# markomih/SplatFields

Hardware: AMD Instinct MI355X
Metric: splats*px rasterized/sec (fwd+bwd) (higher is better)
Workload: dtype f32

## Files before the change

include/splatraster.h:

```cpp
#ifndef SPLATRASTER_H
#define SPLATRASTER_H

#include <stddef.h>

#ifdef __cplusplus
extern "C" {
#endif

#define SR_VERSION 4
#define SR_TILE 16

typedef struct SrView {
    int image_height;
    int image_width;
    float tanfovx;
    float tanfovy;
    float scale_modifier;
    int sh_degree;
    int sh_coeffs;
    int prefiltered;
    int debug;
    const float* viewmatrix;
    const float* projmatrix;
    const float* campos;
    const float* bg;
} SrView;

typedef struct SrSplats {
    int count;
    const float* means3D;
    const float* opacities;
    const float* scales;
    const float* rotations;
    const float* cov3D_precomp;
    const float* shs;
    const float* colors_precomp;
    int raw_params;
    const float* shs_rest;
} SrSplats;

#define SR_RAW_SCALES 1
#define SR_RAW_OPACITY 2
#define SR_RAW_ROTATIONS 4
#define SR_FORWARD_ONLY 8

typedef struct SrGrads {
    float* dL_dmeans3D;
    float* dL_dmeans2D;
    float* dL_dopacity;
    float* dL_dscales;
    float* dL_drotations;
    float* dL_dcov3D;
    float* dL_dshs;
    float* dL_dcolors;
    float* dL_dshs_rest;
} SrGrads;

int sr_version(void);
const char* sr_last_error(void);

size_t sr_geom_bytes(int n_splats, int height, int width);
size_t sr_binning_bytes(long long instances, int height, int width);
size_t sr_image_bytes(int height, int width);
size_t sr_backward_scratch_bytes(long long instances);

int sr_forward_prepare(const SrView* view, const SrSplats* splats, void* geom, int* radii,
                       long long* instances_out, void* hip_stream);

int sr_forward_render(const SrView* view, const SrSplats* splats, void* geom, void* binning,
                      long long instances, void* image, float* out_color, float* out_depth,
                      float* out_alpha, void* hip_stream);

#define SR_NEED_CAPACITY 2
int sr_forward(const SrView* view, const SrSplats* splats, void* geom, int* radii, void* binning,
               long long binning_capacity, void* image, float* out_color, float* out_depth, float* out_alpha,
               long long* instances_out, void* hip_stream);

int sr_forward_async(const SrView* view, const SrSplats* splats, void* geom, int* radii, void* binning,
                     long long binning_capacity, long long longest_list_hint, long long longest_list_expected, void* image,
                     float* out_color, float* out_depth, float* out_alpha, void** ticket_out, void* hip_stream);
int sr_ticket_wait(void* ticket, long long* instances_out, long long* longest_list_out);
long long sr_last_longest_list(void);
int sr_ticket_release(void* ticket);

#define SR_BWD_SLOT_SPEC_BELOW 6
int sr_backward(const SrView* view, const SrSplats* splats, const void* geom, void* binning,
                long long instances, long long instances_rendered, const void* image, const int* radii,
                const float* dL_dcolor, const float* dL_ddepth, const float* dL_dalpha, void* scratch,
                const SrGrads* grads, void* hip_stream);

int sr_backward_blend(const SrView* view, const SrSplats* splats, const void* geom, void* binning,
                      long long instances, long long instances_rendered, const void* image,
                      const float* dL_dcolor, const float* dL_ddepth, const float* dL_dalpha, void* scratch, void* hip_stream);
int sr_backward_splats(const SrView* view, const SrSplats* splats, const void* geom, void* binning,
                       long long instances, long long instances_rendered, const void* image, const int* radii, void* scratch,
                       const SrGrads* grads, int first_splat, int n_splats, void* hip_stream);

int sr_set_backward_kernel(int which);

int sr_mark_visible(int n_splats, const float* means3D, const float* viewmatrix,
                    const float* projmatrix, unsigned char* present, void* hip_stream);

int sr_densification_stats(int n_splats, const float* dL_dmeans2D, const int* radii, float* grad_accum, float* denom,
                           float* max_radii2D, void* hip_stream);

size_t sr_loss_workspace_bytes(int planes, int height, int width);
size_t sr_loss_maps_bytes(int planes, int height, int width);
int sr_photometric_forward(int batch, int channels, int height, int width, const float* image, const float* gt,
                           const float* alpha, const float* gt_mask, float lambda_dssim, float lambda_mask, void* workspace,
                           float* maps, float* loss, float* l1, float* ssim, float* mask_l1, void* hip_stream);
int sr_photometric_backward(int batch, int channels, int height, int width, const float* image, const float* gt,
                            const float* alpha, const float* gt_mask, const float* maps, float w_l1, float w_ssim, float w_mask,
                            const float* upstream, int upstream_per_item, float* dL_dimage, float* dL_dalpha, void* hip_stream);

#define SR_QUANT_NONE 0
#define SR_QUANT_PNG 1
#define SR_QUANT_TO8B 2
size_t sr_metrics_workspace_bytes(int batch, int height, int width);
int sr_image_metrics(int batch, int height, int width, const float* pred, const long long* pred_strides4, const float* gt,
                     const long long* gt_strides4, const float* mask, long long mask_item_stride, int quantize, void* workspace,
                     float* psnr, float* ssim, float* psnr_channels, unsigned char* frames, void* hip_stream);

int sr_sh_forward(int n_splats, int sh_coeffs, int sh_degree, const float* means3D, const float* shs, const float* campos,
                  float* colors, unsigned char* clamped, void* hip_stream);

int sr_sh_forward_views(int n_splats, int sh_coeffs, int sh_degree, int n_views, const float* means3D, const float* shs,
                        const float* campos, float* colors, float* keep, void* hip_stream);

int sr_sh_backward(int n_splats, int sh_coeffs, int sh_degree, int n_views, const float* means3D, const float* shs,
                   const float* campos, const float* dL_dcolors, float scale, float* dL_dshs, float* dL_dmeans3D,
                   int accumulate_means, void* hip_stream);

size_t sr_knn_workspace_bytes(int n_points);
int sr_knn3_mean_dist2(int n_points, const float* points, float* mean_dist2, void* workspace, void* hip_stream);

#define SR_KNN_MAX_K 8
size_t sr_knn_graph_workspace_bytes(int n_points, int k);
int sr_knn_graph(int n_points, int k, const float* points, int* nn_ix, unsigned* order, unsigned* rev_start, unsigned* rev_edges,
                 void* workspace, void* hip_stream);

#define SR_MORAN_MAX_TENSORS 8
size_t sr_moran_workspace_bytes(int n_items, int n_tensors);
size_t sr_moran_edges_bytes(int n_items, int k, int channels);
int sr_moran_forward(int n_items, int k, float eps, const float* points, const float* weight, const int* nn_ix,
                     const unsigned* order, int n_tensors, const float* const* features, const int* widths, void* workspace,
                     float* out, void* hip_stream);
int sr_moran_backward(int n_items, int k, float eps, const float* points, const float* weight, const int* nn_ix,
                      const unsigned* order, const unsigned* rev_start, const unsigned* rev_edges, int n_tensors,
                      const float* const* features, const int* widths, const float* out, const float* upstream, void* edges,
                      float* const* dL_dfeatures, float* dL_dpoints, float* dL_dweight, void* hip_stream);
int sr_moran_weights(int n_points, int k, float eps, const float* points, const int* nn_ix, float* weights, void* hip_stream);
int sr_moran_weights_backward(int n_points, int k, float eps, const float* points, const int* nn_ix, const unsigned* rev_start,
                              const unsigned* rev_edges, const float* dL_dweights, void* edges, float* dL_dpoints,
                              void* hip_stream);

size_t sr_splat_reg_workspace_bytes(int n_splats);
int sr_splat_reg_forward(int n_splats, const float* means3D, const float* opacity, double lambda_norm, double lambda_norm_mean,
                         double lambda_opacity, void* workspace, float* out, void* hip_stream);
int sr_splat_reg_backward(int n_splats, const float* means3D, const float* opacity, double lambda_norm, double lambda_norm_mean,
                          double lambda_opacity, const float* out, const float* upstream, float* dL_dmeans3D, float* dL_dopacity,
                          void* hip_stream);

size_t sr_depth_l1_workspace_bytes(int batch, int height, int width);
int sr_depth_l1_forward(int batch, int height, int width, const float* depth, const float* gt_depth, void* workspace, float* out,
                        void* hip_stream);
int sr_depth_l1_backward(int batch, int height, int width, const float* depth, const float* gt_depth, const float* upstream,
                         int upstream_per_item, float* dL_ddepth, void* hip_stream);

size_t sr_densify_workspace_bytes(int n_splats);
int sr_densify_plan(int n_splats, const float* log_scales, int scale_cols, const float* opacity_logits, const float* grad_accum,
                    const float* denom, const float* max_radii2D, float grad_threshold, float min_opacity, float extent,
                    float percent_dense, float max_screen_size, void* workspace, int* dest, long long* counts5, void* hip_stream);
int sr_densify_gather(int n_splats, int row_floats, const float* src, float* dst, const int* dest, int mode,
                      const float* log_scales, int scale_cols, const float* rotations, const float* unit_normals,
                      void* hip_stream);

#define SR_ADAM_MAX_TENSORS 32
typedef struct SrAdamJob {
    float* param;
    const float* grad;
    float* exp_avg;
    float* exp_avg_sq;
    long long count;
    int row;
    float step_size, bias_correction2_sqrt, one_minus_beta1, one_minus_beta2, eps;
} SrAdamJob;
int sr_adam_step(int n_jobs, const SrAdamJob* jobs, const unsigned char* visible_or_null, long long rows, void* hip_stream);

#define SR_MLP_MAX_OPS 24
#define SR_MLP_NONE 0
#define SR_MLP_LEAKY 1
#define SR_MLP_MASK 2
typedef struct SrMlpOp {
    const float* w_packed;
    const float* bias;
    const float* src;
    const float* mask;
    float* store;
    unsigned int* sign_store;
    const unsigned int* mask_bits;
    int out_tiles;
    int mem_tiles;
    int reg_tiles;
    int src_row;
    int epilogue;
    int mask_row;
    int store_row;
    int store_channels;
    int store_accumulate;
    int keep_state;
} SrMlpOp;
int sr_mlp_chain(int n_points, int hidden_tiles, int n_ops, const SrMlpOp* ops, float negative_slope, void* hip_stream);

#define SR_MLP_MAX_PACK_JOBS 32
typedef struct SrMlpPackJob {
    const float* w;
    const float* bias_src;
    float* dst;
    float* bias_dst;
    int ld;
    int transposed;
    int row0, n_rows;
    int n_mem, mem_pad, mem_col0;
    int n_reg, reg_width, reg_col0;
    int out_tiles;
    int n_bias;
} SrMlpPackJob;
int sr_mlp_pack(int n_jobs, const SrMlpPackJob* jobs, void* hip_stream);

int sr_mlp_pack_bf16(int n_jobs, const SrMlpPackJob* jobs, void* hip_stream);
int sr_mlp_chain_bf16(int n_points, int hidden_tiles, int n_ops, const SrMlpOp* ops, float negative_slope, void* hip_stream);

int sr_mlp_pack_bf16x3(int n_jobs, const SrMlpPackJob* jobs, void* hip_stream);
int sr_mlp_chain_bf16x3(int n_points, int hidden_tiles, int n_ops, const SrMlpOp* ops, float negative_slope, void* hip_stream);

#define SR_MLP_GROUP_MAX_NETS 8
#define SR_MLP_GROUP_MAX_OPS 40
typedef struct SrMlpNet {
    const SrMlpOp* ops;
    int n_ops;
} SrMlpNet;
int sr_mlp_chain_group(int n_points, int hidden_tiles, int n_nets, const SrMlpNet* nets, float negative_slope, void* hip_stream);
int sr_mlp_chain_group_bf16(int n_points, int hidden_tiles, int n_nets, const SrMlpNet* nets, float negative_slope, void* hip_stream);
int sr_mlp_chain_group_bf16x3(int n_points, int hidden_tiles, int n_nets, const SrMlpNet* nets, float negative_slope, void* hip_stream);

#define SR_MLP_MAX_GRAD_JOBS 16
#define SR_MLP_MAX_GRAD_TASKS 128
typedef struct SrMlpGradJob {
    const float* dz;
    const float* x;
    float* dw;
// ... 50 lines not shown
size_t sr_resfield_backward_workspace(int n_jobs, const SrResFieldJob* jobs);
int sr_resfield_backward(int n_jobs, const SrResFieldJob* jobs, const long long* frame, void* workspace, size_t workspace_bytes,
                         void* hip_stream);

size_t sr_triplane_backward_workspace(int n_points, int channels, int height, int width);
int sr_triplane_forward(int n_points, int channels, int height, int width, const float* planes, float* planes_texel_major,
                        const float* points, float* out, void* hip_stream);
int sr_triplane_backward(int n_points, int channels, int height, int width, const float* planes_texel_major, const float* points,
                         const float* dL_dout, float* dL_dplanes, float* dL_dpoints, void* workspace, void* hip_stream);

#define SR_PLANE_MAX_JOBS 8
#define SR_CONV_PROLOGUE 1
#define SR_CONV_UPSAMPLE 2
#define SR_CONV_RESIDUAL 4
#define SR_CONV_SILU_OUT 8
typedef struct SrPlaneJob {
    const float* x;
    const float* weight;
    const float* bias;
    const float* gamma;
    const float* beta;
    float* stats;
    const float* residual;
    float* out;
    float* pre;
    const float* dy;
    float* dx;
    float* dweight;
    float* dbias;
    float* dgamma;
    float* dbeta;
    float* d_residual;
    const float* add;
    float* dx_out;
} SrPlaneJob;

size_t sr_groupnorm_stats_workspace(int n_planes, int channels, int groups, int height, int width);
int sr_groupnorm_stats(int n_planes, const SrPlaneJob* jobs, int channels, int groups, int height, int width, float eps,
                       void* workspace, void* hip_stream);

int sr_conv3x3_forward(int n_planes, const SrPlaneJob* jobs, int cin, int cout, int h_in, int w_in, int groups, int flags,
                       void* hip_stream);

int sr_conv3x3_backward_data(int n_planes, const SrPlaneJob* jobs, int cin, int cout, int h_in, int w_in, int flags, void* hip_stream);

size_t sr_groupnorm_silu_backward_workspace(int n_planes, int channels, int height, int width);
int sr_groupnorm_silu_backward(int n_planes, const SrPlaneJob* jobs, int channels, int groups, int height, int width, float eps,
                               void* workspace, void* hip_stream);

size_t sr_conv3x3_weight_grad_workspace(int n_planes, int cin, int cout, int h_in, int w_in, int flags);
int sr_conv3x3_weight_grad(int n_planes, const SrPlaneJob* jobs, int cin, int cout, int h_in, int w_in, int groups, int flags,
                           void* workspace, void* hip_stream);

typedef struct SrAttentionJob {
    const float* x;
    const float* gamma;
    const float* beta;
    float* stats;
    const float* wq;
    const float* bq;
    const float* wk;
    const float* bk;
    const float* wv;
    const float* bv;
    const float* wo;
    const float* bo;
    float* out;
    void* saved;
    const float* dy;
    float* dx;
    float* dgamma;
    float* dbeta;
    float* dwq;
    float* dbq;
    float* dwk;
    float* dbk;
    float* dwv;
    float* dbv;
    float* dwo;
    float* dbo;
} SrAttentionJob;

size_t sr_attention_saved_bytes(int n_planes, int channels, int groups, int height, int width);
size_t sr_attention_backward_workspace(int n_planes, int channels, int groups, int height, int width);

int sr_attention_forward(int n_planes, const SrAttentionJob* jobs, int channels, int groups, int height, int width, float eps,
                         void* hip_stream);

int sr_attention_backward(int n_planes, const SrAttentionJob* jobs, int channels, int groups, int height, int width, float eps,
                          void* workspace, void* hip_stream);

#define SR_HULL_KRT 0
#define SR_HULL_NDC 1
#define SR_HULL_OUTSIDE_CARVE 0
#define SR_HULL_OUTSIDE_KEEP 1
#define SR_HULL_MAX_VIEWS 1024
typedef struct SrHullView {
    double m[12];
    long long mask_offset;
    int height, width;
    int convention;
    int outside;
} SrHullView;
size_t sr_hull_workspace_bytes(long long n_items);
int sr_hull_carve(int n_views, const SrHullView* views, const unsigned char* masks, long long mask_bytes, const double* grid, int G,
                  const void* points, long long n_points, int point_is_double, void* workspace, int* count_out, void* hip_stream);
int sr_hull_gather(const double* grid, int G, const void* points, long long n_points, int point_is_double, const void* workspace,
                   long long capacity, int* indices_out, float* points_out, void* hip_stream);

#define SR_FLOW_OFFSET 0
#define SR_FLOW_SE3 1
#define SR_FLOW_SE3_AFFINE 2
#define SR_FLOW_SE3_SCALED 3
#define SR_FLOW_AFFINE 4
#define SR_FLOW_DCT 5
#define SR_FLOW_MAX_BRANCHES 4
#define SR_FLOW_MAX_WIDTH 256
#define SR_FLOW_MAX_OUT 32
#define SR_FLOW_MAX_BASIS 10
typedef struct SrFlowBranch {
    const float* weight;
    const float* bias;
    int rows;
} SrFlowBranch;
size_t sr_flow_head_saved_bytes(int model, long long n_points, int width, int n_basis);
size_t sr_flow_head_workspace_bytes(int model, long long n_points, int width, int n_basis);
int sr_flow_head_dz_row(int model, int n_basis);
int sr_flow_head_forward(int model, long long n_points, int width, int n_basis, int n_branches, const SrFlowBranch* branches,
                         const float* hidden, const float* pts, const float* bases, float* means3D, float* flow, void* saved,
                         void* hip_stream);
int sr_flow_head_backward(int model, long long n_points, int width, int n_basis, int n_branches, const SrFlowBranch* branches,
                          const float* pts, const float* bases, const void* saved, const float* dL_dmeans3D, const float* dL_dflow,
                          float* dL_dpts, float* dL_dz, float* dL_dhidden, void* workspace, void* hip_stream);

#define SR_VIEW_FROM_CAMERAS 0
#define SR_VIEW_DIRS_GIVEN 1
#define SR_VIEW_MAX_WIDTH 256
#define SR_VIEW_MAX_VIEWS 16
size_t sr_view_color_saved_bytes(long long n_points, int width, int n_views);
size_t sr_view_color_workspace_bytes(long long n_points, int width, int n_views);
int sr_view_color_forward(int mode, long long n_points, int width, int n_views, const float* feature, const float* means3D,
                          const float* campos_or_dirs, const float* weight, const float* bias, float* colours, void* saved,
                          void* hip_stream);
int sr_view_color_backward(int mode, long long n_points, int width, int n_views, const float* means3D, const float* campos_or_dirs,
                           const float* weight, const void* saved, const float* dL_dcolours, float* dL_dfeature, float* dL_dpos,
                           float* dL_dzsum, void* workspace, void* hip_stream);

int sr_debug_layout(int n_splats, int height, int width, long long instances, size_t* out4);

int sr_debug_backward_stats(unsigned long long* out16, int reset);

int sr_debug_counters(long long* out4, int reset);

int sr_debug_snapshot(const SrView* view, const SrSplats* splats, const float* dL_dcolor, const float* dL_ddepth,
                      const float* dL_dalpha, int backward);

#define SR_PROFILE_STAGES 7
int sr_profile_enable(int on);
int sr_profile_collect(double* ms_sum, long long* launches);
const char* sr_profile_stage_name(int stage);

#ifdef __cplusplus
}
#endif
#endif
```

splatfields_amd/_lib.py:

```python
from __future__ import annotations

import ctypes as C
from pathlib import Path

import os

import torch

LIB_PATH = Path(os.environ.get("SPLATRASTER_LIB") or (Path(__file__).resolve().parent / "libsplatraster.so"))

c_float_p = C.c_void_p


class SrView(C.Structure):
    _fields_ = [("image_height", C.c_int), ("image_width", C.c_int), ("tanfovx", C.c_float), ("tanfovy", C.c_float),
                ("scale_modifier", C.c_float), ("sh_degree", C.c_int), ("sh_coeffs", C.c_int), ("prefiltered", C.c_int),
                ("debug", C.c_int), ("viewmatrix", C.c_void_p), ("projmatrix", C.c_void_p), ("campos", C.c_void_p),
                ("bg", C.c_void_p)]


class SrSplats(C.Structure):
    _fields_ = [("count", C.c_int), ("means3D", C.c_void_p), ("opacities", C.c_void_p), ("scales", C.c_void_p),
                ("rotations", C.c_void_p), ("cov3D_precomp", C.c_void_p), ("shs", C.c_void_p),
                ("colors_precomp", C.c_void_p), ("raw_params", C.c_int), ("shs_rest", C.c_void_p)]


class SrGrads(C.Structure):
    _fields_ = [("dL_dmeans3D", C.c_void_p), ("dL_dmeans2D", C.c_void_p), ("dL_dopacity", C.c_void_p),
                ("dL_dscales", C.c_void_p), ("dL_drotations", C.c_void_p), ("dL_dcov3D", C.c_void_p),
                ("dL_dshs", C.c_void_p), ("dL_dcolors", C.c_void_p), ("dL_dshs_rest", C.c_void_p)]


class SrMlpOp(C.Structure):
    _fields_ = [("w_packed", C.c_void_p), ("bias", C.c_void_p), ("src", C.c_void_p), ("mask", C.c_void_p), ("store", C.c_void_p),
                ("sign_store", C.c_void_p), ("mask_bits", C.c_void_p),
                ("out_tiles", C.c_int), ("mem_tiles", C.c_int), ("reg_tiles", C.c_int), ("src_row", C.c_int), ("epilogue", C.c_int),
                ("mask_row", C.c_int), ("store_row", C.c_int), ("store_channels", C.c_int), ("store_accumulate", C.c_int),
                ("keep_state", C.c_int)]


class SrMlpNet(C.Structure):
    _fields_ = [("ops", C.POINTER(SrMlpOp)), ("n_ops", C.c_int)]


class SrMlpHeadInput(C.Structure):
    _fields_ = [("x0", C.c_void_p), ("dL_dx0", C.c_void_p), ("multires", C.c_int), ("row", C.c_int)]


class SrMlpHeadOutput(C.Structure):
    _fields_ = [("y", C.c_void_p), ("out", C.c_void_p), ("dL_dout", C.c_void_p), ("g", C.c_void_p), ("out_features", C.c_int),
                ("row", C.c_int), ("activation", C.c_int), ("reserved", C.c_int)]


class SrMlpPackJob(C.Structure):
    _fields_ = [("w", C.c_void_p), ("bias_src", C.c_void_p), ("dst", C.c_void_p), ("bias_dst", C.c_void_p), ("ld", C.c_int),
                ("transposed", C.c_int), ("row0", C.c_int), ("n_rows", C.c_int), ("n_mem", C.c_int), ("mem_pad", C.c_int),
                ("mem_col0", C.c_int), ("n_reg", C.c_int), ("reg_width", C.c_int), ("reg_col0", C.c_int), ("out_tiles", C.c_int),
                ("n_bias", C.c_int)]


class SrMlpGradJob(C.Structure):
    _fields_ = [("dz", C.c_void_p), ("x", C.c_void_p), ("dw", C.c_void_p), ("db", C.c_void_p), ("dz_row", C.c_int), ("m", C.c_int),
                ("x_row", C.c_int), ("k", C.c_int), ("dw_row", C.c_int), ("dw_col0", C.c_int)]


class SrResFieldJob(C.Structure):
    _fields_ = [("w", C.c_void_p), ("weights_t", C.c_void_p), ("matrix_t", C.c_void_p), ("out", C.c_void_p), ("d_out", C.c_void_p),
                ("d_matrix_t", C.c_void_p), ("d_weights_t", C.c_void_p), ("count", C.c_int), ("rank", C.c_int), ("capacity", C.c_int)]


class SrAdamJob(C.Structure):
    _fields_ = [("param", C.c_void_p), ("grad", C.c_void_p), ("exp_avg", C.c_void_p), ("exp_avg_sq", C.c_void_p),
                ("count", C.c_longlong), ("row", C.c_int), ("step_size", C.c_float), ("bias_correction2_sqrt", C.c_float),
                ("one_minus_beta1", C.c_float), ("one_minus_beta2", C.c_float), ("eps", C.c_float)]


class SrPlaneJob(C.Structure):
    _fields_ = [(name, C.c_void_p) for name in (
        "x", "weight", "bias", "gamma", "beta", "stats", "residual", "out", "pre", "dy", "dx", "dweight", "dbias", "dgamma", "dbeta",
        "d_residual", "add", "dx_out")]


class SrAttentionJob(C.Structure):
    _fields_ = [(name, C.c_void_p) for name in (
        "x", "gamma", "beta", "stats", "wq", "bq", "wk", "bk", "wv", "bv", "wo", "bo", "out", "saved", "dy", "dx", "dgamma", "dbeta",
        "dwq", "dbq", "dwk", "dbk", "dwv", "dbv", "dwo", "dbo")]


class SrHullView(C.Structure):
    _fields_ = [("m", C.c_double * 12), ("mask_offset", C.c_longlong), ("height", C.c_int), ("width", C.c_int),
                ("convention", C.c_int), ("outside", C.c_int)]


class SrFlowBranch(C.Structure):
    _fields_ = [("weight", C.c_void_p), ("bias", C.c_void_p), ("rows", C.c_int)]


FLOW_OFFSET, FLOW_SE3, FLOW_SE3_AFFINE, FLOW_SE3_SCALED, FLOW_AFFINE, FLOW_DCT = 0, 1, 2, 3, 4, 5
FLOW_MAX_BRANCHES, FLOW_MAX_WIDTH, FLOW_MAX_OUT, FLOW_MAX_BASIS = 4, 256, 32, 10
VIEW_FROM_CAMERAS, VIEW_DIRS_GIVEN, VIEW_MAX_WIDTH, VIEW_MAX_VIEWS = 0, 1, 256, 16
HULL_KRT, HULL_NDC, HULL_OUTSIDE_CARVE, HULL_OUTSIDE_KEEP, HULL_MAX_VIEWS = 0, 1, 0, 1, 1024
RESFIELD_MAX_JOBS, RESFIELD_MAX_RANK = 16, 64
PLANE_MAX_JOBS = 8
CONV_PROLOGUE, CONV_UPSAMPLE, CONV_RESIDUAL, CONV_SILU_OUT = 1, 2, 4, 8
MLP_MAX_GRAD_JOBS, MLP_MAX_GRAD_TASKS = 16, 128
MLP_MAX_PACK_JOBS = 32
MORAN_MAX_TENSORS, KNN_MAX_K = 8, 8
ADAM_MAX_TENSORS = 32
QUANT_NONE, QUANT_PNG, QUANT_TO8B = 0, 1, 2
MLP_MAX_OPS, MLP_NONE, MLP_LEAKY, MLP_MASK = 24, 0, 1, 2
MLP_GROUP_MAX_NETS, MLP_GROUP_MAX_OPS, MLP_GROUP_MAX_HEADS = 8, 40, 8
MLP_OUT_NONE, MLP_OUT_SIGMOID, MLP_OUT_NORMALIZE = 0, 1, 2


SYMBOLS = {
    "sr_version": (C.c_int, []),
    "sr_last_error": (C.c_char_p, []),
    "sr_geom_bytes": (C.c_size_t, [C.c_int, C.c_int, C.c_int]),
    "sr_binning_bytes": (C.c_size_t, [C.c_longlong, C.c_int, C.c_int]),
    "sr_image_bytes": (C.c_size_t, [C.c_int, C.c_int]),
    "sr_backward_scratch_bytes": (C.c_size_t, [C.c_longlong]),
    "sr_forward_prepare": (C.c_int, [C.POINTER(SrView), C.POINTER(SrSplats), C.c_void_p, C.c_void_p,
                                     C.POINTER(C.c_longlong), C.c_void_p]),
    "sr_forward_render": (C.c_int, [C.POINTER(SrView), C.POINTER(SrSplats), C.c_void_p, C.c_void_p, C.c_longlong,
                                    C.c_void_p, C.c_void_p, C.c_void_p, C.c_void_p, C.c_void_p]),
    "sr_forward": (C.c_int, [C.POINTER(SrView), C.POINTER(SrSplats), C.c_void_p, C.c_void_p, C.c_void_p, C.c_longlong,
                             C.c_void_p, C.c_void_p, C.c_void_p, C.c_void_p, C.POINTER(C.c_longlong), C.c_void_p]),
    "sr_forward_async": (C.c_int, [C.POINTER(SrView), C.POINTER(SrSplats), C.c_void_p, C.c_void_p, C.c_void_p, C.c_longlong,
                                   C.c_longlong, C.c_longlong, C.c_void_p, C.c_void_p, C.c_void_p, C.c_void_p, C.POINTER(C.c_void_p),
                                   C.c_void_p]),
    "sr_ticket_wait": (C.c_int, [C.c_void_p, C.POINTER(C.c_longlong), C.POINTER(C.c_longlong)]),
    "sr_ticket_release": (C.c_int, [C.c_void_p]),
    "sr_last_longest_list": (C.c_longlong, []),
    "sr_debug_counters": (C.c_int, [C.POINTER(C.c_longlong), C.c_int]),
    "sr_backward": (C.c_int, [C.POINTER(SrView), C.POINTER(SrSplats), C.c_void_p, C.c_void_p, C.c_longlong, C.c_longlong, C.c_void_p,
                              C.c_void_p, C.c_void_p, C.c_void_p, C.c_void_p, C.c_void_p, C.POINTER(SrGrads),
                              C.c_void_p]),
    "sr_backward_blend": (C.c_int, [C.POINTER(SrView), C.POINTER(SrSplats), C.c_void_p, C.c_void_p, C.c_longlong, C.c_longlong, C.c_void_p,
                                    C.c_void_p, C.c_void_p, C.c_void_p, C.c_void_p, C.c_void_p]),
    "sr_backward_splats": (C.c_int, [C.POINTER(SrView), C.POINTER(SrSplats), C.c_void_p, C.c_void_p, C.c_longlong, C.c_longlong, C.c_void_p, C.c_void_p,
                                     C.c_void_p, C.POINTER(SrGrads), C.c_int, C.c_int, C.c_void_p]),
    "sr_debug_snapshot": (C.c_int, [C.POINTER(SrView), C.POINTER(SrSplats), C.c_void_p, C.c_void_p, C.c_void_p, C.c_int]),
    "sr_set_backward_kernel": (C.c_int, [C.c_int]),
    "sr_sh_forward": (C.c_int, [C.c_int, C.c_int, C.c_int, C.c_void_p, C.c_void_p, C.c_void_p, C.c_void_p, C.c_void_p, C.c_void_p]),
    "sr_sh_forward_views": (C.c_int, [C.c_int, C.c_int, C.c_int, C.c_int, C.c_void_p, C.c_void_p, C.c_void_p, C.c_void_p, C.c_void_p, C.c_void_p]),
    "sr_sh_backward": (C.c_int, [C.c_int, C.c_int, C.c_int, C.c_int, C.c_void_p, C.c_void_p, C.c_void_p, C.c_void_p, C.c_float,
                                 C.c_void_p, C.c_void_p, C.c_int, C.c_void_p]),
    "sr_knn_workspace_bytes": (C.c_size_t, [C.c_int]),
    "sr_knn3_mean_dist2": (C.c_int, [C.c_int, C.c_void_p, C.c_void_p, C.c_void_p, C.c_void_p]),
    "sr_knn_graph_workspace_bytes": (C.c_size_t, [C.c_int, C.c_int]),
    "sr_knn_graph": (C.c_int, [C.c_int, C.c_int, C.c_void_p, C.c_void_p, C.c_void_p, C.c_void_p, C.c_void_p, C.c_void_p, C.c_void_p]),
    "sr_moran_workspace_bytes": (C.c_size_t, [C.c_int, C.c_int]),
    "sr_moran_edges_bytes": (C.c_size_t, [C.c_int, C.c_int, C.c_int]),
    "sr_moran_forward": (C.c_int, [C.c_int, C.c_int, C.c_float, C.c_void_p, C.c_void_p, C.c_void_p, C.c_void_p, C.c_int,
                                   C.POINTER(C.c_void_p), C.POINTER(C.c_int), C.c_void_p, C.c_void_p, C.c_void_p]),
    "sr_moran_backward": (C.c_int, [C.c_int, C.c_int, C.c_float, C.c_void_p, C.c_void_p, C.c_void_p, C.c_void_p, C.c_void_p, C.c_void_p,
                                    C.c_int, C.POINTER(C.c_void_p), C.POINTER(C.c_int), C.c_void_p, C.c_void_p, C.c_void_p,
                                    C.POINTER(C.c_void_p), C.c_void_p, C.c_void_p, C.c_void_p]),
    "sr_moran_weights": (C.c_int, [C.c_int, C.c_int, C.c_float, C.c_void_p, C.c_void_p, C.c_void_p, C.c_void_p]),
    "sr_moran_weights_backward": (C.c_int, [C.c_int, C.c_int, C.c_float, C.c_void_p, C.c_void_p, C.c_void_p, C.c_void_p, C.c_void_p,
                                            C.c_void_p, C.c_void_p, C.c_void_p]),
    "sr_loss_workspace_bytes": (C.c_size_t, [C.c_int, C.c_int, C.c_int]),
    "sr_loss_maps_bytes": (C.c_size_t, [C.c_int, C.c_int, C.c_int]),
    "sr_photometric_forward": (C.c_int, [C.c_int, C.c_int, C.c_int, C.c_int, C.c_void_p, C.c_void_p, C.c_void_p, C.c_void_p, C.c_float,
                                         C.c_float, C.c_void_p, C.c_void_p, C.c_void_p, C.c_void_p, C.c_void_p, C.c_void_p, C.c_void_p]),
    "sr_photometric_backward": (C.c_int, [C.c_int, C.c_int, C.c_int, C.c_int, C.c_void_p, C.c_void_p, C.c_void_p, C.c_void_p, C.c_void_p,
                                          C.c_float, C.c_float, C.c_float, C.c_void_p, C.c_int, C.c_void_p, C.c_void_p, C.c_void_p]),
    "sr_metrics_workspace_bytes": (C.c_size_t, [C.c_int, C.c_int, C.c_int]),
    "sr_image_metrics": (C.c_int, [C.c_int, C.c_int, C.c_int, C.c_void_p, C.POINTER(C.c_longlong), C.c_void_p, C.POINTER(C.c_longlong),
                                   C.c_void_p, C.c_longlong, C.c_int, C.c_void_p, C.c_void_p, C.c_void_p, C.c_void_p, C.c_void_p,
                                   C.c_void_p]),
    "sr_adam_step": (C.c_int, [C.c_int, C.POINTER(SrAdamJob), C.c_void_p, C.c_longlong, C.c_void_p]),
    "sr_splat_reg_workspace_bytes": (C.c_size_t, [C.c_int]),
    "sr_splat_reg_forward": (C.c_int, [C.c_int, C.c_void_p, C.c_void_p, C.c_double, C.c_double, C.c_double, C.c_void_p, C.c_void_p, C.c_void_p]),
    "sr_splat_reg_backward": (C.c_int, [C.c_int, C.c_void_p, C.c_void_p, C.c_double, C.c_double, C.c_double, C.c_void_p, C.c_void_p, C.c_void_p,
                                        C.c_void_p, C.c_void_p]),
    "sr_depth_l1_workspace_bytes": (C.c_size_t, [C.c_int, C.c_int, C.c_int]),
    "sr_depth_l1_forward": (C.c_int, [C.c_int, C.c_int, C.c_int, C.c_void_p, C.c_void_p, C.c_void_p, C.c_void_p, C.c_void_p]),
    "sr_depth_l1_backward": (C.c_int, [C.c_int, C.c_int, C.c_int, C.c_void_p, C.c_void_p, C.c_void_p, C.c_int, C.c_void_p, C.c_void_p]),
    "sr_densify_workspace_bytes": (C.c_size_t, [C.c_int]),
    "sr_densify_plan": (C.c_int, [C.c_int, C.c_void_p, C.c_int, C.c_void_p, C.c_void_p, C.c_void_p, C.c_void_p, C.c_float, C.c_float,
                                  C.c_float, C.c_float, C.c_float, C.c_void_p, C.c_void_p, C.POINTER(C.c_longlong), C.c_void_p]),
    "sr_densify_gather": (C.c_int, [C.c_int, C.c_int, C.c_void_p, C.c_void_p, C.c_void_p, C.c_int, C.c_void_p, C.c_int, C.c_void_p,
                                    C.c_void_p, C.c_void_p]),
    "sr_hull_workspace_bytes": (C.c_size_t, [C.c_longlong]),
    "sr_hull_carve": (C.c_int, [C.c_int, C.POINTER(SrHullView), C.c_void_p, C.c_longlong, C.c_void_p, C.c_int, C.c_void_p, C.c_longlong,
                                C.c_int, C.c_void_p, C.c_void_p, C.c_void_p]),
    "sr_hull_gather": (C.c_int, [C.c_void_p, C.c_int, C.c_void_p, C.c_longlong, C.c_int, C.c_void_p, C.c_longlong, C.c_void_p, C.c_void_p,
                                 C.c_void_p]),
    "sr_mlp_pack": (C.c_int, [C.c_int, C.POINTER(SrMlpPackJob), C.c_void_p]),
    "sr_mlp_weight_grad_workspace": (C.c_size_t, [C.c_int, C.c_int, C.POINTER(SrMlpGradJob)]),
    "sr_mlp_weight_grad": (C.c_int, [C.c_int, C.c_int, C.POINTER(SrMlpGradJob), C.c_void_p, C.c_size_t, C.c_void_p]),
    "sr_mlp_chain": (C.c_int, [C.c_int, C.c_int, C.c_int, C.POINTER(SrMlpOp), C.c_float, C.c_void_p]),
    "sr_mlp_pack_bf16": (C.c_int, [C.c_int, C.POINTER(SrMlpPackJob), C.c_void_p]),
    "sr_mlp_chain_bf16": (C.c_int, [C.c_int, C.c_int, C.c_int, C.POINTER(SrMlpOp), C.c_float, C.c_void_p]),
    "sr_mlp_pack_bf16x3": (C.c_int, [C.c_int, C.POINTER(SrMlpPackJob), C.c_void_p]),
    "sr_mlp_chain_bf16x3": (C.c_int, [C.c_int, C.c_int, C.c_int, C.POINTER(SrMlpOp), C.c_float, C.c_void_p]),
    "sr_mlp_chain_group": (C.c_int, [C.c_int, C.c_int, C.c_int, C.POINTER(SrMlpNet), C.c_float, C.c_void_p]),
    "sr_mlp_chain_group_bf16": (C.c_int, [C.c_int, C.c_int, C.c_int, C.POINTER(SrMlpNet), C.c_float, C.c_void_p]),
    "sr_mlp_chain_group_bf16x3": (C.c_int, [C.c_int, C.c_int, C.c_int, C.POINTER(SrMlpNet), C.c_float, C.c_void_p]),
    "sr_mlp_group_input_forward": (C.c_int, [C.c_int, C.c_int, C.POINTER(SrMlpHeadInput), C.c_int, C.c_int, C.c_void_p, C.c_void_p, C.c_void_p,
                                             C.c_void_p]),
    "sr_mlp_group_input_backward": (C.c_int, [C.c_int, C.c_int, C.POINTER(SrMlpHeadInput), C.c_int, C.c_void_p, C.c_void_p, C.c_void_p, C.c_void_p]),
    "sr_mlp_group_output": (C.c_int, [C.c_int, C.c_int, C.POINTER(SrMlpHeadOutput), C.c_void_p]),
    "sr_mlp_group_top_gradient": (C.c_int, [C.c_int, C.c_int, C.POINTER(SrMlpHeadOutput), C.c_float, C.c_void_p]),
    "sr_mlp_input_forward": (C.c_int, [C.c_int, C.c_int, C.c_int, C.c_int, C.c_int, C.c_void_p, C.c_void_p, C.c_void_p, C.c_void_p, C.c_void_p]),
    "sr_mlp_top_gradient": (C.c_int, [C.c_int, C.c_int, C.c_int, C.c_void_p, C.c_void_p, C.c_float, C.c_void_p, C.c_void_p]),
    "sr_mlp_input_backward": (C.c_int, [C.c_int, C.c_int, C.c_int, C.c_int, C.c_void_p, C.c_void_p, C.c_void_p, C.c_void_p, C.c_void_p]),
    "sr_resfield_compose": (C.c_int, [C.c_int, C.POINTER(SrResFieldJob), C.c_void_p, C.c_void_p]),
    "sr_resfield_backward_workspace": (C.c_size_t, [C.c_int, C.POINTER(SrResFieldJob)]),
    "sr_resfield_backward": (C.c_int, [C.c_int, C.POINTER(SrResFieldJob), C.c_void_p, C.c_void_p, C.c_size_t, C.c_void_p]),
    "sr_triplane_backward_workspace": (C.c_size_t, [C.c_int, C.c_int, C.c_int, C.c_int]),
    "sr_triplane_forward": (C.c_int, [C.c_int, C.c_int, C.c_int, C.c_int, C.c_void_p, C.c_void_p, C.c_void_p, C.c_void_p, C.c_void_p]),
    "sr_triplane_backward": (C.c_int, [C.c_int, C.c_int, C.c_int, C.c_int, C.c_void_p, C.c_void_p, C.c_void_p, C.c_void_p, C.c_void_p,
                                       C.c_void_p, C.c_void_p]),
    "sr_groupnorm_stats_workspace": (C.c_size_t, [C.c_int, C.c_int, C.c_int, C.c_int, C.c_int]),
    "sr_groupnorm_stats": (C.c_int, [C.c_int, C.POINTER(SrPlaneJob), C.c_int, C.c_int, C.c_int, C.c_int, C.c_float, C.c_void_p, C.c_void_p]),
    "sr_conv3x3_forward": (C.c_int, [C.c_int, C.POINTER(SrPlaneJob), C.c_int, C.c_int, C.c_int, C.c_int, C.c_int, C.c_int, C.c_void_p]),
    "sr_conv3x3_backward_data": (C.c_int, [C.c_int, C.POINTER(SrPlaneJob), C.c_int, C.c_int, C.c_int, C.c_int, C.c_int, C.c_void_p]),
    "sr_groupnorm_silu_backward_workspace": (C.c_size_t, [C.c_int, C.c_int, C.c_int, C.c_int]),
    "sr_groupnorm_silu_backward": (C.c_int, [C.c_int, C.POINTER(SrPlaneJob), C.c_int, C.c_int, C.c_int, C.c_int, C.c_float, C.c_void_p,
                                             C.c_void_p]),
    "sr_conv3x3_weight_grad_workspace": (C.c_size_t, [C.c_int, C.c_int, C.c_int, C.c_int, C.c_int, C.c_int]),
    "sr_conv3x3_weight_grad": (C.c_int, [C.c_int, C.POINTER(SrPlaneJob), C.c_int, C.c_int, C.c_int, C.c_int, C.c_int, C.c_int, C.c_void_p,
                                         C.c_void_p]),
    "sr_attention_saved_bytes": (C.c_size_t, [C.c_int, C.c_int, C.c_int, C.c_int, C.c_int]),
    "sr_attention_backward_workspace": (C.c_size_t, [C.c_int, C.c_int, C.c_int, C.c_int, C.c_int]),
    "sr_attention_forward": (C.c_int, [C.c_int, C.POINTER(SrAttentionJob), C.c_int, C.c_int, C.c_int, C.c_int, C.c_float, C.c_void_p]),
    "sr_attention_backward": (C.c_int, [C.c_int, C.POINTER(SrAttentionJob), C.c_int, C.c_int, C.c_int, C.c_int, C.c_float, C.c_void_p,
                                        C.c_void_p]),
    "sr_flow_head_saved_bytes": (C.c_size_t, [C.c_int, C.c_longlong, C.c_int, C.c_int]),
    "sr_flow_head_workspace_bytes": (C.c_size_t, [C.c_int, C.c_longlong, C.c_int, C.c_int]),
    "sr_flow_head_dz_row": (C.c_int, [C.c_int, C.c_int]),
    "sr_flow_head_forward": (C.c_int, [C.c_int, C.c_longlong, C.c_int, C.c_int, C.c_int, C.POINTER(SrFlowBranch), C.c_void_p, C.c_void_p,
                                       C.c_void_p, C.c_void_p, C.c_void_p, C.c_void_p, C.c_void_p]),
    "sr_flow_head_backward": (C.c_int, [C.c_int, C.c_longlong, C.c_int, C.c_int, C.c_int, C.POINTER(SrFlowBranch), C.c_void_p, C.c_void_p,
                                        C.c_void_p, C.c_void_p, C.c_void_p, C.c_void_p, C.c_void_p, C.c_void_p, C.c_void_p, C.c_void_p]),
    "sr_view_color_saved_bytes": (C.c_size_t, [C.c_longlong, C.c_int, C.c_int]),
    "sr_view_color_workspace_bytes": (C.c_size_t, [C.c_longlong, C.c_int, C.c_int]),
    "sr_view_color_forward": (C.c_int, [C.c_int, C.c_longlong, C.c_int, C.c_int, C.c_void_p, C.c_void_p, C.c_void_p, C.c_void_p, C.c_void_p,
                                        C.c_void_p, C.c_void_p, C.c_void_p]),
    "sr_view_color_backward": (C.c_int, [C.c_int, C.c_longlong, C.c_int, C.c_int, C.c_void_p, C.c_void_p, C.c_void_p, C.c_void_p, C.c_void_p,
                                         C.c_void_p, C.c_void_p, C.c_void_p, C.c_void_p, C.c_void_p]),
    "sr_debug_layout": (C.c_int, [C.c_int, C.c_int, C.c_int, C.c_longlong, C.POINTER(C.c_size_t)]),
    "sr_debug_backward_stats": (C.c_int, [C.POINTER(C.c_ulonglong), C.c_int]),
    "sr_profile_enable": (C.c_int, [C.c_int]),
    "sr_profile_collect": (C.c_int, [C.POINTER(C.c_double), C.POINTER(C.c_longlong)]),
    "sr_profile_stage_name": (C.c_char_p, [C.c_int]),
    "sr_mark_visible": (C.c_int, [C.c_int, C.c_void_p, C.c_void_p, C.c_void_p, C.c_void_p, C.c_void_p]),
    "sr_densification_stats": (C.c_int, [C.c_int, C.c_void_p, C.c_void_p, C.c_void_p, C.c_void_p, C.c_void_p, C.c_void_p]),
}

PROFILE_STAGES = 7
SR_VERSION = 4
SR_NEED_CAPACITY = 2
SR_RAW_SCALES, SR_RAW_OPACITY, SR_RAW_ROTATIONS, SR_FORWARD_ONLY = 1, 2, 4, 8
_lib = None


def bind(path) -> C.CDLL:
    lib = C.CDLL(str(path))
    for name, (res, args) in SYMBOLS.items():
        fn = getattr(lib, name)
        fn.restype = res
        fn.argtypes = args
    got = lib.sr_version()
    if got != SR_VERSION:
        raise RuntimeError(f"{path} implements version {got} of the splatraster ABI, this binding expects {SR_VERSION}: "
                           "rebuild it with `python -m splatfields_amd.build`")
    return lib


def load() -> C.CDLL:
    global _lib
    if _lib is None:
        if not LIB_PATH.exists():
            raise RuntimeError(
                f"{LIB_PATH} is missing: build it with `python -m splatfields_amd.build` "
                "(hipcc --offload-arch=gfx950). There is no CPU fallback.")
        _lib = bind(LIB_PATH)
    return _lib


class use_library:

    def __init__(self, path):
        self.handle = bind(path)

    def __enter__(self):
        global _lib
        self.prev, _lib = _lib, self.handle
        return self.handle

    def __exit__(self, *exc):
        global _lib
        _lib = self.prev
# ... 31 lines not shown
```

splatfields_amd/build.py:

```python
from __future__ import annotations

import os
import shutil
import subprocess
from pathlib import Path

PKG_DIR = Path(__file__).resolve().parent
CSRC = PKG_DIR / "csrc"
LIB_PATH = PKG_DIR / "libsplatraster.so"
STATS_LIB_PATH = PKG_DIR / "libsplatraster_stats.so"
SOURCES = ["api.hip", "preprocess.hip", "binning.hip", "render.hip", "blend_bwd.hip", "knn.hip", "sh.hip", "densify.hip", "mlp.hip", "triplane.hip", "loss.hip", "moran.hip", "adam.hip", "metrics.hip", "objective.hip", "planegen.hip", "attention.hip", "hull.hip", "flow_head.hip", "view_color.hip"]
HEADERS = ["common.h", "kernels.h", "host_api.h", "expand.h", "sh_stage.h", "quadmask.h", "reduce.h", "window11.h", "point_tile.h", "mlp_bf16x3.h", "../../include/splatraster.h"]


def _hipcc() -> str:
    exe = shutil.which("hipcc") or "/opt/rocm/bin/hipcc"
    if not os.path.exists(exe):
        raise RuntimeError("hipcc not found; libsplatraster.so cannot be built")
    return exe


def is_stale() -> bool:
    if not LIB_PATH.exists():
        return True
    t = LIB_PATH.stat().st_mtime
    return any((CSRC / f).stat().st_mtime > t for f in SOURCES + HEADERS)


def strip_comments(text: str) -> str:
    out, i, n = [], 0, len(text)
    while i < n:
        c = text[i]
        if c in "\"'":
            j = i + 1
            while j < n and text[j] != c:
                j += 2 if text[j] == "\\" else 1
            out.append(text[i:j + 1])
            i = j + 1
        elif text.startswith("//", i):
            j = text.find("\n", i)
            i = n if j < 0 else j
        elif text.startswith("/*", i):
            j = text.find("*/", i + 2)
            out.append(" ")
            i = n if j < 0 else j + 2
        else:
            out.append(c)
            i += 1
    lines = (" ".join(line.split()) for line in "".join(out).splitlines())
    return "\n".join(line for line in lines if line)


def source_hash() -> str:
    import hashlib
    h = hashlib.sha256()
    for f in sorted(SOURCES + HEADERS):
        h.update(f.encode())
        h.update(strip_comments((CSRC / f).read_text()).encode())
    return h.hexdigest()[:16]


def build_library(force: bool = False, verbose: bool = False, out: Path = None, defines=()) -> Path:
    if out is None and not force and not is_stale():
        return LIB_PATH
    target = Path(out) if out is not None else LIB_PATH
    cmd = [_hipcc(), "--offload-arch=gfx950", "-O3", "-std=c++17", "-shared", "-fPIC", "-Wno-unused-value",
           "-fno-slp-vectorize"] + [f"-D{d}" for d in defines] + [
           "-o", str(target)] + [str(CSRC / f) for f in SOURCES]
    if verbose:
        print(" ".join(cmd))
    subprocess.run(cmd, check=True, cwd=str(CSRC))
    return target


def build_stats_library(force: bool = False, verbose: bool = False) -> Path:
    if not force and STATS_LIB_PATH.exists() and not any(
            (CSRC / f).stat().st_mtime > STATS_LIB_PATH.stat().st_mtime for f in SOURCES + HEADERS):
        return STATS_LIB_PATH
    return build_library(force=True, verbose=verbose, out=STATS_LIB_PATH, defines=["SR_BWD_STATS", "SR_BWD_WAVES_PER_SIMD=3"])


if __name__ == "__main__":
    import sys
    if len(sys.argv) > 1:
        print(build_library(force=True, verbose=True, out=Path(sys.argv[1]).resolve(), defines=sys.argv[2:]))
    else:
        print(build_library(force=True, verbose=True))
```

splatfields_amd/csrc/api.hip:

```cpp
#include <cstdint>
#include <cstdio>
#include <cstdlib>
#include <cstring>
#include <atomic>
#include <chrono>
#include <thread>
#include <mutex>
#include <string>
#include <vector>
#include "host_api.h"
#include "kernels.h"

namespace {

thread_local std::string g_last_error;
thread_local long long g_last_longest = -1;

struct ProfRec { int stage; hipEvent_t a, b; bool ended; unsigned long long serial; };
unsigned long long g_prof_serial = 0;
bool g_prof_on = false;
std::vector<ProfRec> g_prof;
std::mutex g_prof_mutex;
const char* kStageNames[SR_PROFILE_STAGES] = {"preprocess", "scan", "emit", "sort_tiles", "render_forward",
                                              "render_backward", "preprocess_backward"};

}

namespace sr {

int fail(const std::string& msg) { g_last_error = msg; return 1; }

int check_hip(hipError_t e, const char* what) {
    if (e == hipSuccess) return 0;
    return fail(std::string(what) + ": " + hipGetErrorString(e));
}

StageTimer::StageTimer(int stage, hipStream_t s) : st(s) {
    if (!g_prof_on) return;
    ProfRec r; r.stage = stage; r.ended = false;
    if (hipEventCreate(&r.a) != hipSuccess || hipEventCreate(&r.b) != hipSuccess) return;
    hipEventRecord(r.a, st);
    std::lock_guard<std::mutex> lock(g_prof_mutex);
    serial = ++g_prof_serial;
    r.serial = serial;
    g_prof.push_back(r); idx = 0;
    end = r.b;
}
StageTimer::~StageTimer() {
    if (idx < 0) return;
    std::lock_guard<std::mutex> lock(g_prof_mutex);
    for (auto& r : g_prof)
        if (r.serial == serial) { hipEventRecord(end, st); r.ended = true; break; }
}

}

using sr::fail; using sr::check_hip; using sr::StageTimer;

namespace {

struct StatusBlock { uint32_t* pinned = nullptr; uint32_t* pinned_dev = nullptr; uint32_t seq = 0; hipStream_t stream = nullptr; int dev = 0; };
thread_local StatusBlock g_sync[64];
std::mutex g_ticket_mutex;
std::vector<StatusBlock*> g_ticket_free[64];
std::atomic<long long> g_counters[4];

int status_block_init(StatusBlock& b, int dev) {
    if (hipHostMalloc(reinterpret_cast<void**>(&b.pinned), 64, hipHostMallocCoherent) != hipSuccess &&
        hipHostMalloc(reinterpret_cast<void**>(&b.pinned), 64, hipHostMallocDefault) != hipSuccess) return fail("hipHostMalloc failed");
    void* dp = nullptr;
    if (hipHostGetDevicePointer(&dp, b.pinned, 0) != hipSuccess) { hipHostFree(b.pinned); b.pinned = nullptr; return fail("hipHostGetDevicePointer failed"); }
    b.pinned_dev = static_cast<uint32_t*>(dp);
    for (int i = 0; i < 16; ++i) b.pinned[i] = 0u;
    b.dev = dev; b.seq = 0;
    return 0;
}
uint32_t status_block_arm(StatusBlock& b, hipStream_t st) {
    b.seq = b.seq + 1u == 0u ? 1u : b.seq + 1u;
    b.stream = st;
    return b.seq;
}
int status_block_wait(StatusBlock& b, bool* waited) {
    volatile uint32_t* p = b.pinned;
    auto ready = [&] { return p[2] == b.seq && p[3] == b.seq; };
    if (waited) *waited = false;
    if (!ready()) {
        if (waited) *waited = true;
        const auto t0 = std::chrono::steady_clock::now();
        for (unsigned spins = 0; !ready(); ++spins) {
            if (spins > 4096u) std::this_thread::yield();
            if ((spins & 0xfffu) == 0xfffu && std::chrono::steady_clock::now() - t0 > std::chrono::seconds(2)) {
                SR_TRY(check_hip(hipStreamSynchronize(b.stream), "wait for the instance count"));
                if (!ready()) return fail("the instance count of the forward never reached the host (k_scan_small did not run?)");
            }
        }
    }
    std::atomic_thread_fence(std::memory_order_acquire);
    return 0;
}

int current_device(int* dev) {
    if (hipGetDevice(dev) != hipSuccess || *dev < 0 || *dev >= 64) return fail("hipGetDevice failed");
    return 0;
}

int thread_block(StatusBlock** out) {
    int dev = 0;
    SR_TRY(current_device(&dev));
    *out = &g_sync[dev];
    return (*out)->pinned ? 0 : status_block_init(**out, dev);
}

int ticket_acquire(StatusBlock** out) {
    int dev = 0;
    SR_TRY(current_device(&dev));
    {
        std::lock_guard<std::mutex> lock(g_ticket_mutex);
        if (!g_ticket_free[dev].empty()) { *out = g_ticket_free[dev].back(); g_ticket_free[dev].pop_back(); return 0; }
    }
    StatusBlock* t = new StatusBlock;
    if (int rc = status_block_init(*t, dev)) { delete t; return rc; }
    g_counters[3].fetch_add(1, std::memory_order_relaxed);
    *out = t;
    return 0;
}
void ticket_recycle(StatusBlock* t) {
    std::lock_guard<std::mutex> lock(g_ticket_mutex);
    g_ticket_free[t->dev].push_back(t);
}

std::atomic<int> g_bwd_kernel{[] {
    const char* sel = getenv("SPLATRASTER_BWD");
    return !sel ? 0 : (std::string(sel) == "wave" ? 1 : (std::string(sel) == "quads" ? 2 : 0));
}()};


struct CallContext { const SrView* view = nullptr; const SrSplats* splats = nullptr; const char* file = nullptr;
                     const float* dL_dcolor = nullptr; const float* dL_ddepth = nullptr; const float* dL_dalpha = nullptr; };
thread_local CallContext g_call;

void dump_record(FILE* f, const char* name, const void* dev, size_t bytes, bool on_device) {
    char tag[16] = {0};
    std::strncpy(tag, name, 15);
    std::vector<char> host;
    uint64_t n = 0;
    if (dev && bytes) {
        host.resize(bytes);
        if (!on_device) { std::memcpy(host.data(), dev, bytes); n = bytes; }
        else if (hipMemcpy(host.data(), dev, bytes, hipMemcpyDeviceToHost) == hipSuccess) n = bytes;
        else (void)hipGetLastError();
    }
    std::fwrite(tag, 1, 16, f); std::fwrite(&n, 8, 1, f);
    if (n) std::fwrite(host.data(), 1, (size_t)n, f);
}

void dump_snapshot(const char* stage) {
    const CallContext& c = g_call;
    if (!c.view || !c.splats || !c.file) return;
    FILE* f = std::fopen(c.file, "wb");
    if (!f) return;
    char head[8] = {'S', 'R', 'S', 'N', 'A', 'P', '1', 0}, st[32] = {0};
    std::strncpy(st, stage, 31);
    std::fwrite(head, 1, 8, f); std::fwrite(st, 1, 32, f);
    const SrView* v = c.view; const SrSplats* s = c.splats;
    const int32_t vi[4] = {v->image_height, v->image_width, v->sh_degree, v->sh_coeffs};
    const float vf[3] = {v->tanfovx, v->tanfovy, v->scale_modifier};
    char vb[32]; std::memcpy(vb, vi, 16); std::memcpy(vb + 16, vf, 12); const int32_t pf = v->prefiltered; std::memcpy(vb + 28, &pf, 4);
    dump_record(f, "view", vb, 32, false);
    const int32_t n = s->count;
    dump_record(f, "count", &n, 4, false);
    dump_record(f, "viewmatrix", v->viewmatrix, 64, true); dump_record(f, "projmatrix", v->projmatrix, 64, true);
    dump_record(f, "campos", v->campos, 12, true); dump_record(f, "bg", v->bg, 12, true);
    const size_t N = (size_t)(n > 0 ? n : 0);
    dump_record(f, "means3D", s->means3D, N * 12, true); dump_record(f, "opacities", s->opacities, N * 4, true);
    dump_record(f, "scales", s->scales, N * 12, true); dump_record(f, "rotations", s->rotations, N * 16, true);
    dump_record(f, "cov3D_precomp", s->cov3D_precomp, N * 24, true);
    dump_record(f, "shs", s->shs, s->shs ? N * 12 * (size_t)(s->shs_rest ? 1 : v->sh_coeffs) : 0, true);
    dump_record(f, "shs_rest", s->shs_rest, N * 12 * 15, true);
    dump_record(f, "colors_precomp", s->colors_precomp, N * 12, true);
    const size_t px = (size_t)v->image_height * v->image_width;
    dump_record(f, "dL_dcolor", c.dL_dcolor, px * 12, true); dump_record(f, "dL_ddepth", c.dL_ddepth, px * 4, true);
    dump_record(f, "dL_dalpha", c.dL_dalpha, px * 4, true);
    std::fclose(f);
}

int after_launch(const SrView* view, hipStream_t st, const char* what) {
    int rc = check_hip(hipGetLastError(), what);
    if (!rc && view && view->debug) rc = check_hip(hipStreamSynchronize(st), what);
    if (rc && view && view->debug) {
        const std::string keep = g_last_error;
        dump_snapshot(what);
        g_last_error = keep + (g_call.file ? std::string(" (inputs written to ") + g_call.file + ")" : std::string());
    }
    return rc;
}

int validate(const SrView* view, const SrSplats* s) {
    if (!view || !s) return fail("null view/splats");
    if (s->count < 0) return fail("negative splat count");
    if (view->image_height <= 0 || view->image_width <= 0) return fail("image size must be positive");
    if (!view->viewmatrix || !view->projmatrix || !view->campos || !view->bg) return fail("viewmatrix/projmatrix/campos/bg must be device pointers");
    if (s->count > 0) {
        if (!s->means3D || !s->opacities) return fail("means3D/opacities missing");
        const bool has_sr = s->scales && s->rotations;
        if (has_sr == (s->cov3D_precomp != nullptr)) return fail("Please provide exactly one of either scale/rotation pair or precomputed 3D covariance!");
        if ((s->shs != nullptr) == (s->colors_precomp != nullptr)) return fail("Please provide excatly one of either SHs or precomputed colors!");
        if (s->shs) {
            if (view->sh_degree < 0 || view->sh_degree > 3) return fail("sh_degree must be 0..3");
            if (view->sh_coeffs < (view->sh_degree + 1) * (view->sh_degree + 1)) return fail("shs holds fewer coefficients than sh_degree needs");
            if (s->shs_rest) {
                if (view->sh_coeffs != 16) return fail("shs_rest (dc + rest SH tensors) needs sh_coeffs == 16");
                if ((reinterpret_cast<uintptr_t>(s->shs) | reinterpret_cast<uintptr_t>(s->shs_rest)) & 15u) return fail("shs / shs_rest must be 16-byte aligned");
            }
        } else if (s->shs_rest) return fail("shs_rest without shs");
        if (s->raw_params & ~(SR_RAW_SCALES | SR_RAW_OPACITY | SR_RAW_ROTATIONS | SR_FORWARD_ONLY)) return fail("unknown bits in raw_params");
        if (s->cov3D_precomp && (s->raw_params & (SR_RAW_SCALES | SR_RAW_ROTATIONS))) return fail("raw scales/rotations with cov3D_precomp");
    }
    if ((sr::tiles_x(view->image_width) > sr::kMaxTilesPerSide) || (sr::tiles_y(view->image_height) > sr::kMaxTilesPerSide)) return fail("image too large (more than 65520 pixels a side)");
    return 0;
}

sr::ViewK make_view(const SrView* v) {
    sr::ViewK k;
    k.H = v->image_height; k.W = v->image_width;
    k.gx = sr::tiles_x(k.W); k.gy = sr::tiles_y(k.H);
    k.tanfovx = v->tanfovx; k.tanfovy = v->tanfovy;
    k.focal_x = k.W / (2.0f * v->tanfovx); k.focal_y = k.H / (2.0f * v->tanfovy);
    k.scale_modifier = v->scale_modifier;
    k.sh_degree = v->sh_degree; k.sh_coeffs = v->sh_coeffs;
    k.viewmatrix = v->viewmatrix; k.projmatrix = v->projmatrix; k.campos = v->campos; k.bg = v->bg;
    return k;
}

sr::SplatsK make_splats(const SrSplats* s) {
    sr::SplatsK k;
    k.N = s->count; k.means3D = s->means3D; k.opacities = s->opacities; k.scales = s->scales;
    k.rotations = s->rotations; k.cov3D = s->cov3D_precomp; k.shs = s->shs; k.colors = s->colors_precomp;
    k.raw = s->raw_params; k.shs_rest = s->shs_rest;
    return k;
}

long long covered_by_hint(long long hint) { return hint <= 2048 ? 2048 : hint <= 4096 ? 4096 : hint <= 8192 ? 8192 : -1; }

struct Call {
    hipStream_t st = nullptr;
    sr::ViewK v; sr::SplatsK s;
    sr::Geom g; sr::Binning b; sr::Image im;
    void carve(const void* geom, void* binning, long long capacity, const void* image) {
        sr::carve_geom(const_cast<void*>(geom), s.N, v.H, v.W, &g);
        if (binning) sr::carve_binning(binning, capacity, &b);
        if (image) sr::carve_image(const_cast<void*>(image), v.H, v.W, &im);
    }
};

int open_call(Call& c, const CallContext& ctx, void* hip_stream) {
    SR_TRY(validate(ctx.view, ctx.splats));
    g_call = ctx;
    c.st = static_cast<hipStream_t>(hip_stream);
    c.v = make_view(ctx.view);
    c.s = make_splats(ctx.splats);
    return 0;
}

bool capacity_in_range(long long r) { return r >= 0 && r < (1ll << 32); }

}

extern "C" {

int sr_version(void) { return SR_VERSION; }
const char* sr_last_error(void) { return g_last_error.c_str(); }

size_t sr_geom_bytes(int n, int h, int w) { return sr::carve_geom(nullptr, n, h, w, nullptr); }
size_t sr_binning_bytes(long long r, int, int) { return sr::carve_binning(nullptr, r, nullptr); }
size_t sr_image_bytes(int h, int w) { return sr::carve_image(nullptr, h, w, nullptr); }
size_t sr_backward_scratch_bytes(long long r) {
    const size_t n = (size_t)(r > 0 ? r : 1);
    return sr::align_up(n * sr::kSlotFloats * sizeof(float), 256);
}

}

namespace {

int launch_stage1(const SrView* view, const sr::ViewK& v, const sr::SplatsK& s, const sr::Geom& g, int* radii, uint32_t* host_out,
                  uint32_t host_seq, hipStream_t st) {
    { StageTimer t_(0, st); sr::launch_preprocess(v, s, g, radii, st); }
    SR_TRY(after_launch(view, st, "preprocess"));
    { StageTimer t_(1, st); sr::launch_count_tiles(v, s.N, g, st); sr::launch_scan_small(v, s.N, g, host_out, host_seq, st); }
    SR_TRY(after_launch(view, st, "scan"));
    return 0;
}

int launch_stage2(const SrView* view, const sr::ViewK& v, const sr::SplatsK& s, const sr::Geom& g, const sr::Binning& b,
                  const sr::Image& im, float* out_color, float* out_depth, float* out_alpha, StatusBlock* hs, long long max_len,
                  long long expected_len, hipStream_t st) {
    { StageTimer t_(2, st); sr::launch_emit(v, s.N, g, b, st); }
    SR_TRY(after_launch(view, st, "emit"));
    if (hs) {
        g_counters[0].fetch_add(1, std::memory_order_relaxed);
        SR_TRY(status_block_wait(*hs, nullptr));
        max_len = (long long)hs->pinned[1];
        if ((long long)hs->pinned[0] > (long long)b.capacity) return 0;
    }
    { StageTimer t_(3, st); sr::launch_sort_tiles(v, g, b, max_len, expected_len, st); }
    SR_TRY(after_launch(view, st, "sort_tiles"));
    { StageTimer t_(4, st); sr::launch_render_forward(v, g, b, im, out_color, out_depth, out_alpha, st); }
    SR_TRY(after_launch(view, st, "render_forward"));
    return 0;
}

}

extern "C" {

int sr_forward_prepare(const SrView* view, const SrSplats* splats, void* geom, int* radii,
                       long long* instances_out, void* hip_stream) {
    Call c;
    SR_TRY(open_call(c, CallContext{view, splats, "snapshot_fw.dump"}, hip_stream));
    if (!geom || !instances_out || (splats->count > 0 && !radii)) return fail("null geom/radii/instances_out");
    c.carve(geom, nullptr, 0, nullptr);
    StatusBlock* hs = nullptr;
    SR_TRY(thread_block(&hs));
    SR_TRY(launch_stage1(view, c.v, c.s, c.g, radii, hs->pinned_dev, status_block_arm(*hs, c.st), c.st));
    SR_TRY(check_hip(hipStreamSynchronize(c.st), "sync after prepare"));
    *instances_out = (long long)hs->pinned[0];
    return 0;
}

int sr_forward(const SrView* view, const SrSplats* splats, void* geom, int* radii, void* binning,
               long long binning_capacity, void* image, float* out_color, float* out_depth, float* out_alpha,
               long long* instances_out, void* hip_stream) {
    Call c;
    SR_TRY(open_call(c, CallContext{view, splats, "snapshot_fw.dump"}, hip_stream));
    if (!geom || !binning || !image || !out_color || !out_depth || !instances_out || (splats->count > 0 && !radii)) return fail("null buffer");
    if (!capacity_in_range(binning_capacity)) return fail("binning capacity out of range");
    c.carve(geom, binning, binning_capacity, image);
    StatusBlock* hs = nullptr;
    SR_TRY(thread_block(&hs));
    SR_TRY(launch_stage1(view, c.v, c.s, c.g, radii, hs->pinned_dev, status_block_arm(*hs, c.st), c.st));
    SR_TRY(launch_stage2(view, c.v, c.s, c.g, c.b, c.im, out_color, out_depth, out_alpha, hs, -1, -1, c.st));
    const long long total = (long long)hs->pinned[0];
    *instances_out = total;
    g_last_longest = (long long)hs->pinned[1];
    return total > binning_capacity ? SR_NEED_CAPACITY : 0;
}

int sr_forward_render(const SrView* view, const SrSplats* splats, void* geom, void* binning,
                      long long instances, void* image, float* out_color, float* out_depth,
                      float* out_alpha, void* hip_stream) {
    Call c;
    SR_TRY(open_call(c, CallContext{view, splats, "snapshot_fw.dump"}, hip_stream));
    if (!geom || !binning || !image || !out_color || !out_depth) return fail("null buffer");
    if (!capacity_in_range(instances)) return fail("instance count out of range");
    c.carve(geom, binning, instances, image);
    return launch_stage2(view, c.v, c.s, c.g, c.b, c.im, out_color, out_depth, out_alpha, nullptr, -1, -1, c.st);
}

int sr_forward_async(const SrView* view, const SrSplats* splats, void* geom, int* radii, void* binning,
                     long long binning_capacity, long long longest_list_hint, long long longest_list_expected, void* image,
                     float* out_color, float* out_depth, float* out_alpha, void** ticket_out, void* hip_stream) {
    Call c;
    SR_TRY(open_call(c, CallContext{view, splats, "snapshot_fw.dump"}, hip_stream));
    if (!geom || !binning || !image || !out_color || !out_depth || !ticket_out || (splats->count > 0 && !radii)) return fail("null buffer");
    if (!capacity_in_range(binning_capacity)) return fail("binning capacity out of range");
    if (longest_list_hint < 0) return fail("longest_list_hint must be >= 0");
    c.carve(geom, binning, binning_capacity, image);
    const long long covered = covered_by_hint(longest_list_hint);
    c.b.sorted_up_to = covered < 0 ? 0xffffffffu : (uint32_t)covered;
    StatusBlock* t = nullptr;
    SR_TRY(ticket_acquire(&t));
    int rc = launch_stage1(view, c.v, c.s, c.g, radii, t->pinned_dev, status_block_arm(*t, c.st), c.st);
    if (!rc) rc = launch_stage2(view, c.v, c.s, c.g, c.b, c.im, out_color, out_depth, out_alpha, nullptr, covered,
                                longest_list_expected >= 0 && longest_list_expected <= longest_list_hint ? longest_list_expected : -1, c.st);
    if (rc) {
        (void)hipStreamSynchronize(c.st);
        ticket_recycle(t);
        return rc;
    }
    g_counters[1].fetch_add(1, std::memory_order_relaxed);
    *ticket_out = t;
    return 0;
}

int sr_ticket_wait(void* ticket, long long* instances_out, long long* longest_list_out) {
    if (!ticket) return fail("null ticket");
    StatusBlock* t = static_cast<StatusBlock*>(ticket);
    bool waited = false;
    const int rc = status_block_wait(*t, &waited);
    if (waited) g_counters[2].fetch_add(1, std::memory_order_relaxed);
    if (rc) {
        return rc;
    }
    if (instances_out) *instances_out = (long long)t->pinned[0];
    if (longest_list_out) *longest_list_out = (long long)t->pinned[1];
    ticket_recycle(t);
    return 0;
}

long long sr_last_longest_list(void) { return g_last_longest; }

int sr_ticket_release(void* ticket) { return sr_ticket_wait(ticket, nullptr, nullptr); }

int sr_debug_counters(long long* out4, int reset) {
    if (!out4) return fail("null pointer in sr_debug_counters");
    for (int i = 0; i < 4; ++i) out4[i] = reset ? g_counters[i].exchange(0, std::memory_order_relaxed) : g_counters[i].load(std::memory_order_relaxed);
    return 0;
}

namespace {
int backward_impl(int what, const SrView* view, const SrSplats* splats, const void* geom, void* binning,
                  long long instances, long long instances_rendered, const void* image, const int* radii,
                  const float* dL_dcolor, const float* dL_ddepth, const float* dL_dalpha, void* scratch,
                  const SrGrads* grads, int first, int count, void* hip_stream) {
    Call c;
    SR_TRY(open_call(c, CallContext{view, splats, "snapshot_bw.dump", dL_dcolor, dL_ddepth, dL_dalpha}, hip_stream));
    if (!geom || !binning || !image || !scratch) return fail("null buffer");
    if ((what & 1) && !dL_dcolor) return fail("null buffer");
    if ((what & 2) && !grads) return fail("null buffer");
    if (what & 2) {
        if (splats->count > 0 && (!radii || !grads->dL_dmeans3D || !grads->dL_dmeans2D || !grads->dL_dopacity)) return fail("null gradient output");
        if (splats->count > 0 && splats->shs && !grads->dL_dshs && !grads->dL_dcolors) return fail("dL_dshs (or dL_dcolors for the colour-gradient mode) missing");
        if (splats->count > 0 && splats->shs_rest && grads->dL_dshs && !grads->dL_dshs_rest) return fail("dL_dshs_rest missing");
        if (splats->count > 0 && splats->colors_precomp && !grads->dL_dcolors) return fail("dL_dcolors missing");
        if (splats->count > 0 && splats->cov3D_precomp && !grads->dL_dcov3D) return fail("dL_dcov3D missing");
        if (splats->count > 0 && !splats->cov3D_precomp && (!grads->dL_dscales || !grads->dL_drotations)) return fail("dL_dscales/dL_drotations missing");
        if (first < 0 || count < 0 || (first % sr::kBlock) != 0) return fail("splat range must start at a multiple of 256");
    }
    if (splats->raw_params & SR_FORWARD_ONLY) return fail("the forward of these buffers was run with SR_FORWARD_ONLY");
    c.carve(geom, binning, instances, image);
    const hipStream_t st = c.st;
    const sr::SplatsK& s = c.s;
    float* slots = static_cast<float*>(scratch);
    if (what & 1) {
        StageTimer t_(5, st);
        const int pinned = g_bwd_kernel.load(std::memory_order_relaxed);
        const bool wave_kernel = pinned == 1;
        if (wave_kernel) sr::launch_render_backward(c.v, c.g, c.b, c.im, dL_dcolor, dL_ddepth, dL_dalpha, slots, st);
        else sr::launch_render_backward_quads(c.v, c.g, c.b, c.im, dL_dcolor, dL_ddepth, dL_dalpha, slots, st);
    }
    if (what & 1) SR_TRY(after_launch(view, st, "render_backward"));
    if (what & 2) {
        sr::GradsK gr;
        gr.means3D = grads->dL_dmeans3D; gr.means2D = grads->dL_dmeans2D; gr.opacity = grads->dL_dopacity;
        gr.scales = s.cov3D ? nullptr : grads->dL_dscales; gr.rotations = s.cov3D ? nullptr : grads->dL_drotations;
        gr.cov3D = s.cov3D ? grads->dL_dcov3D : nullptr;
        gr.shs = s.shs ? grads->dL_dshs : nullptr;
        gr.shs_rest = (s.shs_rest && gr.shs) ? grads->dL_dshs_rest : nullptr;
        gr.colors = (s.colors || (s.shs && !grads->dL_dshs)) ? grads->dL_dcolors : nullptr;
        const bool small_fp = !(instances_rendered >= 0 && instances_rendered > (long long)SR_BWD_SLOT_SPEC_BELOW * (long long)s.N);
        { StageTimer t_(6, st); sr::launch_preprocess_backward(c.v, s, c.g, radii, slots, c.b.reached, gr, first, count, small_fp, st); }
        SR_TRY(after_launch(view, st, "preprocess_backward"));
    }
    return 0;
}
}

int sr_backward(const SrView* view, const SrSplats* splats, const void* geom, void* binning,
                long long instances, long long instances_rendered, const void* image, const int* radii,
                const float* dL_dcolor, const float* dL_ddepth, const float* dL_dalpha, void* scratch,
                const SrGrads* grads, void* hip_stream) {
    return backward_impl(3, view, splats, geom, binning, instances, instances_rendered, image, radii, dL_dcolor, dL_ddepth, dL_dalpha,
                         scratch, grads, 0, splats ? splats->count : 0, hip_stream);
}

int sr_backward_blend(const SrView* view, const SrSplats* splats, const void* geom, void* binning,
                      long long instances, long long instances_rendered, const void* image,
                      const float* dL_dcolor, const float* dL_ddepth, const float* dL_dalpha, void* scratch, void* hip_stream) {
    return backward_impl(1, view, splats, geom, binning, instances, instances_rendered, image, nullptr, dL_dcolor, dL_ddepth, dL_dalpha,
                         scratch, nullptr, 0, 0, hip_stream);
}

int sr_backward_splats(const SrView* view, const SrSplats* splats, const void* geom, void* binning,
                       long long instances, long long instances_rendered, const void* image, const int* radii, void* scratch,
                       const SrGrads* grads, int first_splat, int n_splats, void* hip_stream) {
    return backward_impl(2, view, splats, geom, binning, instances, instances_rendered, image, radii, nullptr, nullptr, nullptr, scratch,
                         grads, first_splat, n_splats, hip_stream);
}

int sr_set_backward_kernel(int which) {
    if (which < 0 || which > 2) return -1;
    return g_bwd_kernel.exchange(which, std::memory_order_relaxed);
}

int sr_mark_visible(int n, const float* means3D, const float* viewmatrix, const float*, unsigned char* present, void* hip_stream) {
    if (n < 0 || (n > 0 && (!means3D || !viewmatrix || !present))) return fail("bad arguments to sr_mark_visible");
    hipStream_t st = static_cast<hipStream_t>(hip_stream);
    sr::launch_mark_visible(n, means3D, viewmatrix, present, st);
    return check_hip(hipGetLastError(), "mark_visible");
}

int sr_densification_stats(int n, const float* dL_dmeans2D, const int* radii, float* grad_accum, float* denom, float* max_radii2D,
                           void* hip_stream) {
    if (n < 0) return fail("bad arguments to sr_densification_stats");
    if (n > 0 && (!dL_dmeans2D || !radii)) return fail("null pointer in sr_densification_stats");
    sr::launch_densification_stats(n, dL_dmeans2D, radii, grad_accum, denom, max_radii2D, static_cast<hipStream_t>(hip_stream));
    return check_hip(hipGetLastError(), "densification_stats");
}

int sr_debug_layout(int n, int h, int w, long long instances, size_t* out4) {
    if (!out4 || n < 0 || h <= 0 || w <= 0 || instances < 0) return fail("bad arguments to sr_debug_layout");
    sr::Geom g; sr::Binning b;
    char* const origin = reinterpret_cast<char*>(4096);
    sr::carve_geom(origin, n, h, w, &g);
    sr::carve_binning(origin, instances, &b);
    out4[0] = (size_t)(reinterpret_cast<char*>(g.tile_start) - origin);
    out4[1] = (size_t)(reinterpret_cast<char*>(b.sorted_id) - origin);
    out4[2] = (size_t)(reinterpret_cast<char*>(g.total) - origin);
    out4[3] = (size_t)(reinterpret_cast<char*>(g.offsets) - origin);
    return 0;
}

int sr_debug_backward_stats(unsigned long long* out8, int reset) {
    if (!out8) return fail("null pointer in sr_debug_backward_stats");
    if (hipDeviceSynchronize() != hipSuccess) return fail("sr_debug_backward_stats: device synchronisation failed");
    return sr::backward_stats(out8, reset) ? fail("sr_debug_backward_stats: counter copy failed") : 0;
}

int sr_debug_snapshot(const SrView* view, const SrSplats* splats, const float* dL_dcolor, const float* dL_ddepth, const float* dL_dalpha,
                      int backward) {
    if (!view || !splats) return fail("null view/splats");
    g_call = CallContext{view, splats, backward ? "snapshot_bw.dump" : "snapshot_fw.dump", dL_dcolor, dL_ddepth, dL_dalpha};
    dump_snapshot(backward ? "render_backward (test hook)" : "preprocess (test hook)");
    return 0;
}

int sr_profile_enable(int on) { g_prof_on = on != 0; return 0; }

int sr_profile_collect(double* ms_sum, long long* launches) {
    std::lock_guard<std::mutex> lock(g_prof_mutex);
    std::vector<ProfRec> open;
    for (auto& r : g_prof) {
        if (!r.ended) { open.push_back(r); continue; }
        float ms = 0.f;
        if (hipEventSynchronize(r.b) == hipSuccess && hipEventElapsedTime(&ms, r.a, r.b) == hipSuccess) {
            if (ms_sum) ms_sum[r.stage] += ms;
            if (launches) launches[r.stage] += 1;
        }
        hipEventDestroy(r.a); hipEventDestroy(r.b);
    }
    g_prof.swap(open);
    return 0;
}

const char* sr_profile_stage_name(int stage) { return (stage >= 0 && stage < SR_PROFILE_STAGES) ? kStageNames[stage] : ""; }

}
```

splatfields_amd/csrc/binning.hip:

```cpp
#include <atomic>
#include "kernels.h"
#include "expand.h"

namespace sr {

static void allow_dynamic_lds(const void* kernel, int slot, int bytes) {
    static std::atomic<bool> done[8][64];
    int dev = 0;
    if (hipGetDevice(&dev) != hipSuccess) return;
    if (dev >= 0 && dev < 64 && done[slot][dev].load(std::memory_order_acquire)) return;
    if (hipFuncSetAttribute(kernel, hipFuncAttributeMaxDynamicSharedMemorySize, bytes) != hipSuccess) { (void)hipGetLastError(); return; }
    if (dev >= 0 && dev < 64) done[slot][dev].store(true, std::memory_order_release);
}

__global__ void __launch_bounds__(kBlock) k_count_tiles(const ViewK v, int N, const Geom g, const Chunking ch) {
    extern __shared__ __attribute__((aligned(16))) uint32_t s_hist[];
    __shared__ uint32_t s_off[kBlock + 1];
    __shared__ ushort4 s_rect[kBlock];
    __shared__ float4 s_r0[kBlock], s_r1[kBlock];
    __shared__ uint32_t s_scan[8];
    for (int t = 4 * threadIdx.x; t < ch.tiles_padded; t += 4 * kBlock) *reinterpret_cast<uint4*>(&s_hist[t]) = make_uint4(0u, 0u, 0u, 0u);
    __syncthreads();
    const int base_chunk = (int)blockIdx.x / ch.slices, slice = (int)blockIdx.x % ch.slices;
    const int sb0 = base_chunk * ch.sub_per_chunk, sb1 = min(sb0 + ch.sub_per_chunk, ch.n_sub);
    for (int sb = sb0; sb < sb1; ++sb) {
        const int idx = sb * kBlock + threadIdx.x;
        uint32_t touched = 0;
        ushort4 rect = make_ushort4(0, 0, 0, 0);
        float4 r0 = make_float4(0.f, 0.f, -1.f, 0.f), r1 = r0;
        if (idx < N) {
            touched = g.touched[idx]; rect = g.rect[idx];
            if (touched > kMaskTiles) { r0 = g.rec[4 * (size_t)idx]; r1 = g.rec[4 * (size_t)idx + 1]; }
        }
        const uint32_t mask = rect_mask16(rect);
        const ushort4 packed = rect;
        rect = rect_clean(rect);
        const bool direct = ch.slices == 1 && touched <= kDirectTiles;
        if (direct && touched > 0u) {
            uint32_t k = 0;
            for (uint32_t ty = rect.y; ty < rect.w; ++ty)
                for (uint32_t tx = rect.x; tx < rect.z; ++tx, ++k)
                    if ((mask >> k) & 1u) atomicAdd(&s_hist[ty * (uint32_t)v.gx + tx], 1u);
        }
        const uint32_t coop = direct ? 0u : touched;
        if (!__syncthreads_or(coop != 0u)) continue;
        uint32_t total;
        const uint32_t excl = block_exclusive_scan(coop, s_scan, total);
        s_off[threadIdx.x] = excl;
        s_rect[threadIdx.x] = packed;
        tile_test_prepare(r0, r1, s_r0[threadIdx.x], s_r1[threadIdx.x]);
        if (threadIdx.x == 0) s_off[kBlock] = total;
        __syncthreads();
        for_each_block_instance(s_off, s_rect, v.gx, [&](int e, uint32_t k, uint32_t tile, uint32_t, uint32_t tile_x, uint32_t tile_y, uint32_t w) {
            if ((w & kRectMasked) ? (w >> k) & 1u : tile_reached(s_r0[e], s_r1[e], tile_x, tile_y)) atomicAdd(&s_hist[tile], 1u);
        }, (uint32_t)slice, (uint32_t)ch.slices);
    }
    __syncthreads();
    uint32_t* row = g.cnt + (size_t)blockIdx.x * ch.tiles_padded;
    for (int t = 4 * threadIdx.x; t < ch.tiles_padded; t += 4 * kBlock) *reinterpret_cast<uint4*>(&row[t]) = *reinterpret_cast<const uint4*>(&s_hist[t]);
}

#ifndef SR_STRIP_COLS
#define SR_STRIP_COLS 32
#endif
constexpr int kStripCols = SR_STRIP_COLS, kStripGroups = 1024 / kStripCols, kStripRows = (kMaxChunks + kStripGroups - 1) / kStripGroups;
__global__ void __launch_bounds__(1024) k_colscan(const Geom g, const Chunking ch) {
    __shared__ uint32_t s_tot[kStripGroups][kStripCols + 1];
    const int c = threadIdx.x % kStripCols, rg = threadIdx.x / kStripCols;
    const int col = blockIdx.x * kStripCols + c, row0 = rg * kStripRows;
    uint32_t* p = g.cnt + (size_t)row0 * ch.tiles_padded + col;
    uint32_t x[kStripRows];
#pragma unroll
    for (int r = 0; r < kStripRows; ++r) x[r] = row0 + r < ch.chunks ? p[(size_t)r * ch.tiles_padded] : 0u;
    uint32_t run = 0;
#pragma unroll
    for (int r = 0; r < kStripRows; ++r) { const uint32_t t = x[r]; x[r] = run; run += t; }
    s_tot[rg][c] = run;
    __syncthreads();
    uint32_t base = 0, all = 0;
#pragma unroll 8
    for (int k = 0; k < kStripGroups; ++k) { const uint32_t t = s_tot[k][c]; base += k < rg ? t : 0u; all += t; }
    if (rg == 0) g.segtot[col] = all;
#pragma unroll
    for (int r = 0; r < kStripRows; ++r) if (row0 + r < ch.chunks) p[(size_t)r * ch.tiles_padded] = x[r] + base;
}

void launch_count_tiles(const ViewK& v, int N, const Geom& g, hipStream_t st) {
    if (!use_count_matrix(v) || N <= 0) return;
    const Chunking ch = make_chunking(N, v.gx * v.gy);
    allow_dynamic_lds(reinterpret_cast<const void*>(&k_count_tiles), 0, (int)(sizeof(uint32_t) * kMaxMatrixTiles));
    hipLaunchKernelGGL(k_count_tiles, dim3(ch.chunks), dim3(kBlock), sizeof(uint32_t) * ch.tiles_padded, st, v, N, g, ch);
    hipLaunchKernelGGL(k_colscan, dim3(ch.tiles_padded / kStripCols), dim3(1024), 0, st, g, ch);
}

__global__ void __launch_bounds__(1024) k_scan_small(const Geom g, int n_sub, int n_tiles, const Chunking ch, int use_matrix,
                                                      uint32_t* __restrict__ host_out, uint32_t host_seq) {
    __shared__ uint32_t s_wave[16];
    const bool tiles = blockIdx.x == 1;
    uint32_t* dst = tiles ? g.tile_start : g.block_offsets;
    const int n = tiles ? n_tiles : n_sub;
    const int tid = threadIdx.x, lane = tid & 63, w = tid >> 6;
    constexpr int kPer = 4;
    uint32_t carry = 0, vmax = 0;
    uint32_t v[kPer];
    for (int base = 0; base < n; base += 1024 * kPer) {
        const int i0 = base + tid * kPer;
        uint32_t sum = 0;
#pragma unroll
        for (int k = 0; k < kPer; ++k) {
            const int i = i0 + k;
            v[k] = 0;
            if (i < n) {
                if (!tiles) v[k] = g.block_sums[i];
                else if (!use_matrix) v[k] = g.tile_count[i];
                else v[k] = g.segtot[i];
            }
            vmax = max(vmax, v[k]);
            sum += v[k];
        }
        const uint32_t inc = wave_inclusive_scan(sum);
        if (lane == 63) s_wave[w] = inc;
        __syncthreads();
        uint32_t wave_base = 0, all = 0;
#pragma unroll
        for (int k = 0; k < 16; ++k) { const uint32_t t = s_wave[k]; if (k < w) wave_base += t; all += t; }
        uint32_t run = carry + wave_base + inc - sum;
#pragma unroll
        for (int k = 0; k < kPer; ++k) {
            const int i = i0 + k;
            if (i < n) { dst[i] = run; if (tiles) g.tile_cursor[i] = 0u; }
            run += v[k];
        }
        carry += all;
        __syncthreads();
    }
    const bool in_regs = n <= 1024 * kPer;
    if (tid == 0) {
        if (tiles) dst[n] = carry;
        else {
            g.total[0] = carry;
            if (host_out) { host_out[0] = carry; __hip_atomic_store(host_out + 2, host_seq, __ATOMIC_RELEASE, __HIP_MEMORY_SCOPE_SYSTEM); }
        }
    }
    if (tiles) {
#pragma unroll
        for (int d = 32; d > 0; d >>= 1) vmax = max(vmax, (uint32_t)__shfl_xor((int)vmax, d, 64));
        __syncthreads();
        if (lane == 0) s_wave[w] = vmax;
        __syncthreads();
        if (tid == 0) {
            uint32_t m = 0;
            for (int k = 0; k < 16; ++k) m = max(m, s_wave[k]);
            g.total[1] = m; s_wave[0] = m;
            if (host_out) { host_out[1] = m; __hip_atomic_store(host_out + 3, host_seq, __ATOMIC_RELEASE, __HIP_MEMORY_SCOPE_SYSTEM); }
        }
        __syncthreads();
        __shared__ uint32_t s_hist[256];
        const uint32_t longest = max(s_wave[0], 1u);
        const float to_class = 255.0f / (float)longest;
        if (tid < 256) s_hist[tid] = 0u;
        __syncthreads();
        if (in_regs) {
#pragma unroll
            for (int k = 0; k < kPer; ++k)
                if (tid * kPer + k < n) atomicAdd(&s_hist[255u - min(255u, (uint32_t)((float)v[k] * to_class))], 1u);
        } else {
            for (int i = tid; i < n; i += 1024) {
                const uint32_t len = dst[i + 1] - dst[i];
                atomicAdd(&s_hist[255u - min(255u, (uint32_t)((float)len * to_class))], 1u);
            }
        }
        __syncthreads();
        if (w == 0) {
            uint32_t c0 = s_hist[4 * lane], c1 = s_hist[4 * lane + 1], c2 = s_hist[4 * lane + 2], c3 = s_hist[4 * lane + 3];
            const uint32_t sum = c0 + c1 + c2 + c3;
            const uint32_t excl = wave_inclusive_scan(sum) - sum;
            s_hist[4 * lane] = excl; s_hist[4 * lane + 1] = excl + c0; s_hist[4 * lane + 2] = excl + c0 + c1;
            s_hist[4 * lane + 3] = excl + c0 + c1 + c2;
        }
        __syncthreads();
        if (tid < 3) {
            const uint32_t lo = 2048u << tid;
            uint32_t cand = 0u;
            if (longest > lo) {
                const uint32_t cls = 255u - min(255u, (uint32_t)((float)(lo + 1u) * to_class));
                cand = cls >= 255u ? (uint32_t)n : s_hist[cls + 1u];
            }
            g.total[4 + tid] = cand;
        }
        __syncthreads();
        if (in_regs) {
#pragma unroll
            for (int k = 0; k < kPer; ++k)
                if (tid * kPer + k < n)
                    g.tile_order[atomicAdd(&s_hist[255u - min(255u, (uint32_t)((float)v[k] * to_class))], 1u)] = (uint32_t)(tid * kPer + k);
        } else {
            for (int i = tid; i < n; i += 1024) {
                const uint32_t len = dst[i + 1] - dst[i];
                g.tile_order[atomicAdd(&s_hist[255u - min(255u, (uint32_t)((float)len * to_class))], 1u)] = (uint32_t)i;
            }
        }
    }
}

void launch_scan_small(const ViewK& v, int N, const Geom& g, uint32_t* host_out, uint32_t host_seq, hipStream_t st) {
    const Chunking ch = make_chunking(N, v.gx * v.gy);
    hipLaunchKernelGGL(k_scan_small, dim3(2), dim3(1024), 0, st, g, (N + kBlock - 1) / kBlock, v.gx * v.gy, ch,
                       use_count_matrix(v) ? 1 : 0, host_out, host_seq);
}

template <bool MATRIX>
__global__ void __launch_bounds__(kBlock) k_emit(const ViewK v, int N, const Geom g, const Binning b, const Chunking ch) {
    extern __shared__ __attribute__((aligned(16))) uint32_t s_cur[];
    __shared__ uint32_t s_off[kBlock + 1];
    __shared__ ushort4 s_rect[kBlock];
    __shared__ uint32_t s_depth[kBlock];
    __shared__ float4 s_r0[kBlock], s_r1[kBlock];
    __shared__ uint32_t s_scan[8];
    if (g.total[0] > b.capacity) return;
    int sb0 = blockIdx.x, sb1 = blockIdx.x + 1;
    uint32_t slice = 0, slices = 1;
    if constexpr (MATRIX) {
        const int per = (ch.chunks + 7) >> 3;
        const int chunk = (int)(blockIdx.x & 7u) * per + (int)(blockIdx.x >> 3);
        if ((int)(blockIdx.x >> 3) >= per || chunk >= ch.chunks) return;
        slice = (uint32_t)(chunk % ch.slices); slices = (uint32_t)ch.slices;
        sb0 = (chunk / ch.slices) * ch.sub_per_chunk; sb1 = min(sb0 + ch.sub_per_chunk, ch.n_sub);
        const uint32_t* row = g.cnt + (size_t)chunk * ch.tiles_padded;
        const int n_tiles = v.gx * v.gy;
        for (int t = 4 * threadIdx.x; t < n_tiles; t += 4 * kBlock) {
            const uint4 a = *reinterpret_cast<const uint4*>(&g.tile_start[t]), r = *reinterpret_cast<const uint4*>(&row[t]);
            *reinterpret_cast<uint4*>(&s_cur[t]) = make_uint4(a.x + r.x, a.y + r.y, a.z + r.z, a.w + r.w);
        }
    }
    constexpr int kAhead = 4;
    for (int sbg = sb0; sbg < sb1; sbg += kAhead) {
        uint32_t touched_a[kAhead], word_a[kAhead], dbits_a[kAhead], base_a[kAhead];
        ushort4 rect_a[kAhead];
        float4 r0_a[kAhead], r1_a[kAhead];
#pragma unroll
        for (int u = 0; u < kAhead; ++u) {
            const int idx = (sbg + u) * kBlock + threadIdx.x;
            touched_a[u] = 0; dbits_a[u] = 0; base_a[u] = 0; rect_a[u] = make_ushort4(0, 0, 0, 0);
            if (sbg + u < sb1) {
                base_a[u] = g.block_offsets[sbg + u];
                if (idx < N) {
                    touched_a[u] = g.touched[idx];
                    rect_a[u] = g.rect[idx];
                    dbits_a[u] = g.depth_bits[idx];
                }
            }
        }
#pragma unroll
        for (int u = 0; u < kAhead; ++u) {
            const int idx = (sbg + u) * kBlock + threadIdx.x;
            r0_a[u] = make_float4(0.f, 0.f, -1.f, 0.f); r1_a[u] = r0_a[u];
            if (touched_a[u] > kMaskTiles) { r0_a[u] = g.rec[4 * (size_t)idx]; r1_a[u] = g.rec[4 * (size_t)idx + 1]; }
            word_a[u] = rect_mask16(rect_a[u]);
        }
#pragma unroll
        for (int u = 0; u < kAhead; ++u) {
            const int sb = sbg + u;
            if (sb >= sb1) break;
            const int idx = sb * kBlock + threadIdx.x;
            const uint32_t touched = touched_a[u], mask = word_a[u];
            const bool direct = slices == 1u && touched <= kDirectTiles;
            const uint32_t coop = direct ? 0u : touched;
            uint32_t total, coop_total;
            uint32_t coop_excl;
            const uint32_t excl = block_exclusive_scan2(touched, coop, s_scan, total, coop_excl, coop_total);
            const uint32_t base = base_a[u];
            if (idx < N) g.offsets[idx] = base + excl;
            if (slice == 0u)
                for (uint32_t i = threadIdx.x; i < total; i += kBlock) b.reached[base + i] = 0;
            const uint32_t first_splat = (uint32_t)sb * kBlock;
            if (direct && touched > 0u) {
                const uint64_t entry = ((uint64_t)dbits_a[u] << 32) | (uint64_t)(first_splat + threadIdx.x);
                uint32_t k = 0;
                const ushort4 rc = rect_clean(rect_a[u]);
                for (uint32_t ty = rc.y; ty < rc.w; ++ty)
                    for (uint32_t tx = rc.x; tx < rc.z; ++tx, ++k) {
                        if (!((mask >> k) & 1u)) continue;
                        const uint32_t tile = ty * (uint32_t)v.gx + tx;
                        uint32_t slot;
                        if constexpr (MATRIX) slot = atomicAdd(&s_cur[tile], 1u);
                        else slot = g.tile_start[tile] + atomicAdd(&g.tile_cursor[tile], 1u);
                        b.ent[slot] = entry;
                    }
            }
            if (coop_total == 0u) continue;
            s_off[threadIdx.x] = coop_excl;
            s_rect[threadIdx.x] = rect_a[u];
            s_depth[threadIdx.x] = dbits_a[u];
            tile_test_prepare(r0_a[u], r1_a[u], s_r0[threadIdx.x], s_r1[threadIdx.x]);
            if (threadIdx.x == 0) s_off[kBlock] = coop_total;
            __syncthreads();
            for_each_block_instance(s_off, s_rect, v.gx, [&](int e, uint32_t k, uint32_t tile, uint32_t, uint32_t tile_x, uint32_t tile_y, uint32_t w) {
                if (!((w & kRectMasked) ? (w >> k) & 1u : tile_reached(s_r0[e], s_r1[e], tile_x, tile_y))) return;
                uint32_t slot;
                if constexpr (MATRIX) slot = atomicAdd(&s_cur[tile], 1u);
                else slot = g.tile_start[tile] + atomicAdd(&g.tile_cursor[tile], 1u);
                b.ent[slot] = ((uint64_t)s_depth[e] << 32) | (uint64_t)(first_splat + (uint32_t)e);
            }, slice, slices);
        }
    }
}

void launch_emit(const ViewK& v, int N, const Geom& g, const Binning& b, hipStream_t st) {
    if (N <= 0) return;
    const Chunking ch = make_chunking(N, v.gx * v.gy);
    allow_dynamic_lds(reinterpret_cast<const void*>(&k_emit<true>), 1, (int)(sizeof(uint32_t) * kMaxMatrixTiles));
    if (use_count_matrix(v))
        hipLaunchKernelGGL(k_emit<true>, dim3((ch.chunks + 7) / 8 * 8), dim3(kBlock), sizeof(uint32_t) * ch.tiles_padded, st, v, N, g, b, ch);
    else
        hipLaunchKernelGGL(k_emit<false>, dim3(ch.n_sub), dim3(kBlock), 0, st, v, N, g, b, ch);
}

template <int D>
__device__ __forceinline__ uint32_t lane_xor(uint32_t x) {
    if constexpr (D == 1) return (uint32_t)__builtin_amdgcn_update_dpp(0, (int)x, 0xB1, 0xf, 0xf, false);
    else if constexpr (D == 2) return (uint32_t)__builtin_amdgcn_update_dpp(0, (int)x, 0x4E, 0xf, 0xf, false);
    else if constexpr (D == 8) return (uint32_t)__builtin_amdgcn_update_dpp(0, (int)x, 0x128, 0xf, 0xf, false);
    else if constexpr (D == 4) {
        const uint32_t a = (uint32_t)__builtin_amdgcn_update_dpp(0, (int)x, 0x124, 0xf, 0xf, false);
        const uint32_t b = (uint32_t)__builtin_amdgcn_update_dpp(0, (int)x, 0x12C, 0xf, 0xf, false);
        return (threadIdx.x & 4u) ? a : b;
    } else if constexpr (D == 16) {
        typedef unsigned int u2 __attribute__((ext_vector_type(2)));
        const u2 r = __builtin_amdgcn_permlane16_swap(x, x, false, false);
        return (threadIdx.x & 16u) ? r.x : r.y;
    } else {
        typedef unsigned int u2 __attribute__((ext_vector_type(2)));
        const u2 r = __builtin_amdgcn_permlane32_swap(x, x, false, false);
        return (threadIdx.x & 32u) ? r.x : r.y;
    }
}

__device__ __forceinline__ uint32_t lane_xor_d(uint32_t x, int d) {
    switch (d) {
        case 1: return lane_xor<1>(x);
        case 2: return lane_xor<2>(x);
        case 4: return lane_xor<4>(x);
        case 8: return lane_xor<8>(x);
        case 16: return lane_xor<16>(x);
        default: return lane_xor<32>(x);
    }
}

__device__ __forceinline__ void exchange_select(uint64_t& k, uint64_t pk, bool keep_min) {
    const bool take = (pk < k) == keep_min;
    k = take ? pk : k;
}

template <int N, int E>
__device__ __forceinline__ void bitonic_regs(uint64_t (&k)[E], uint64_t* skey, uint32_t tid) {
#pragma unroll
    for (int kk = 2; kk <= N; kk <<= 1) {
#pragma unroll
        for (int j = kk >> 1; j > 0; j >>= 1) {
            if (j < E) {
#pragma unroll
                for (int e = 0; e < E; ++e) {
                    if ((e & j) == 0) {
                        const uint32_t i = tid * E + e;
                        const bool asc = (i & kk) == 0;
                        const bool swap = (k[e] > k[e | j]) == asc;
                        const uint64_t ka = k[e], kb = k[e | j];
                        k[e] = swap ? kb : ka; k[e | j] = swap ? ka : kb;
                    }
                }
            } else if (j < 64 * E) {
                const int d = j / E;
                const bool lower = (tid & d) == 0;
                const bool keep_min = lower == (((tid * E) & kk) == 0);
                uint32_t plo[E], phi[E];
#pragma unroll
                for (int e = 0; e < E; ++e) {
                    plo[e] = lane_xor_d((uint32_t)k[e], d);
                    phi[e] = lane_xor_d((uint32_t)(k[e] >> 32), d);
                }
#pragma unroll
                for (int e = 0; e < E; ++e) exchange_select(k[e], ((uint64_t)phi[e] << 32) | plo[e], keep_min);
            } else {
                __syncthreads();
#pragma unroll
                for (int e = 0; e < E; ++e) skey[tid * E + e] = k[e];
                __syncthreads();
#pragma unroll
                for (int e = 0; e < E; ++e) {
                    const uint32_t i = tid * E + e;
                    const bool asc = (i & kk) == 0;
                    const bool lower = (i & j) == 0;
                    exchange_select(k[e], skey[i ^ j], lower == asc);
                }
            }
        }
    }
}

template <int N, int E>
__device__ __forceinline__ void load_sort_chunk(const Binning& b, uint32_t first, uint32_t m, uint64_t (&k)[E], uint64_t* scratch_key, uint32_t tid) {
#pragma unroll
    for (int e = 0; e < E; ++e) {
        const uint32_t i = tid * E + e;
        k[e] = i < m ? b.ent[first + i] : ~0ull;
    }
    bitonic_regs<N, E>(k, scratch_key, tid);
}

template <int N, int E>
__device__ __forceinline__ void sort_tile_regs(const Binning& b, uint32_t start, uint32_t n, uint64_t* skey) {
    uint64_t k[E];
    load_sort_chunk<N, E>(b, start, n, k, skey, threadIdx.x);
#pragma unroll
    for (int e = 0; e < E; ++e) {
        const uint32_t i = threadIdx.x * E + e;
        if (i < n) b.sorted_id[start + i] = (uint32_t)k[e];
    }
}

template <int CAP, int THREADS, typename Emit>
__device__ __forceinline__ void sort_block_lds(const Binning& b, uint32_t first, uint32_t n, uint64_t* run_key, Emit&& emit);

__global__ void __launch_bounds__(256) k_sort_tiles_regs(const Geom g, const Binning b) {
    __shared__ uint64_t skey[2048];
    const uint32_t total_instances = g.total[0];
    const uint32_t tile = g.tile_order[blockIdx.x];
    asm volatile("" :: "s"(tile));
    if (total_instances > b.capacity) return;
    const uint32_t start = g.tile_start[tile];
    const uint32_t n = g.tile_start[tile + 1] - start;
    if (n == 0u || n > 2048u) return;
    if (n <= 256u) sort_tile_regs<256, 1>(b, start, n, skey);
    else if (n <= 512u) sort_tile_regs<512, 2>(b, start, n, skey);
    else if (n <= 1024u) sort_tile_regs<1024, 4>(b, start, n, skey);
    else sort_block_lds<2048, 256>(b, start, n, skey, [&](uint32_t rank, uint64_t key) { b.sorted_id[start + rank] = (uint32_t)key; });
}

template <int E, typename Out>
__device__ __forceinline__ void merge_run_pairs(const uint64_t* src, uint32_t n, uint32_t width, Out&& out) {
    const uint32_t o = threadIdx.x * (uint32_t)E;
    if (o >= n) return;
    const uint32_t base = o & ~(2u * width - 1u);
    const uint64_t* A = src + base;
    const uint32_t a = min(width, n - base);
    const uint32_t b = n - base - a < width ? n - base - a : width;
    const uint32_t d = o - base;
    uint32_t lo = d > b ? d - b : 0u, hi = min(d, a);
    while (lo < hi) {
        const uint32_t mid = (lo + hi) >> 1;
        if (A[mid] < A[width + d - 1u - mid]) lo = mid + 1u; else hi = mid;
    }
    uint32_t ai = lo, bi = d - lo;
    constexpr uint64_t kInf = ~0ull;
    uint64_t ka = ai < a ? A[ai] : kInf;
    uint64_t kb = bi < b ? A[width + bi] : kInf;
#pragma unroll
    for (int e = 0; e < E; ++e) {
        const bool take_a = ka < kb;
        const uint64_t key = take_a ? ka : kb;
        if (d + (uint32_t)e < a + b) out(o + (uint32_t)e, key);
        ai += take_a ? 1u : 0u;
        bi += take_a ? 0u : 1u;
        const bool more = take_a ? ai < a : bi < b;
        const uint64_t nxt = A[take_a ? min(ai, a - 1u) : width + min(bi, max(b, 1u) - 1u)];
        if (take_a) ka = more ? nxt : kInf; else kb = more ? nxt : kInf;
    }
}

template <int CAP, int THREADS, typename Emit>
__device__ __forceinline__ void sort_block_lds(const Binning& b, uint32_t first, uint32_t n, uint64_t* run_key, Emit&& emit) {
    constexpr int GROUPS = THREADS / 256;
    const uint32_t group = threadIdx.x >> 8, tid = threadIdx.x & 255u;
    const uint32_t n_runs = (n + 1023u) / 1024u;
    for (uint32_t r0 = 0; r0 < n_runs; r0 += GROUPS) {
        const uint32_t r = r0 + group;
        const uint32_t m = r < n_runs ? min(1024u, n - r * 1024u) : 0u;
        __syncthreads();
        uint64_t* rk = run_key + r * 1024u;
        uint64_t k[4];
        if (m <= 256u) {
            uint64_t k1[1];
            load_sort_chunk<256, 1>(b, first + r * 1024u, m, k1, rk, tid);
            k[0] = k1[0];
        } else if (m <= 512u) {
            uint64_t k2[2];
            load_sort_chunk<512, 2>(b, first + r * 1024u, m, k2, rk, tid);
            k[0] = k2[0]; k[1] = k2[1];
        } else {
            load_sort_chunk<1024, 4>(b, first + r * 1024u, m, k, rk, tid);
        }
        __syncthreads();
        const uint32_t per = m <= 256u ? 1u : (m <= 512u ? 2u : 4u);
#pragma unroll
        for (int e = 0; e < 4; ++e) {
            const uint32_t i = tid * per + e;
            if ((uint32_t)e < per && i < m) rk[i] = k[e];
        }
    }
    __syncthreads();
    uint64_t* src = run_key;
    uint64_t* dst = run_key + CAP;
    for (uint32_t width = 1024u;; width <<= 1) {
        if (2u * width >= n) {
            merge_run_pairs<CAP / THREADS>(src, n, width, emit);
            break;
        }
        merge_run_pairs<CAP / THREADS>(src, n, width, [&](uint32_t pos, uint64_t key) { dst[pos] = key; });
        __syncthreads();
        uint64_t* t = src; src = dst; dst = t;
    }
    __syncthreads();
}

template <int LO, int CAP, int THREADS>
__global__ void __launch_bounds__(THREADS) k_sort_tiles_merge(const Geom g, const Binning b, int n_tiles) {
    extern __shared__ __attribute__((aligned(16))) unsigned char s_dyn[];
    uint64_t* run_key = reinterpret_cast<uint64_t*>(s_dyn);
    if (g.total[0] > b.capacity) return;
    const uint32_t limit = min((uint32_t)n_tiles, g.total[LO == 2048 ? 4 : 5]);
    for (uint32_t slot = blockIdx.x; slot < limit; slot += gridDim.x) {
        const uint32_t tile = g.tile_order[slot];
        const uint32_t start = g.tile_start[tile];
        const uint32_t n = g.tile_start[tile + 1] - start;
        if (n <= (uint32_t)LO || n > (uint32_t)CAP) continue;
        sort_block_lds<CAP, THREADS>(b, start, n, run_key, [&](uint32_t rank, uint64_t key) { b.sorted_id[start + rank] = (uint32_t)key; });
    }
}

template <typename T>
__device__ __forceinline__ T ld_agent(const T* p) { return __hip_atomic_load(p, __ATOMIC_RELAXED, __HIP_MEMORY_SCOPE_AGENT); }

template <int CAP, int THREADS>
__global__ void __launch_bounds__(THREADS) k_sort_tiles_long(const Geom g, const Binning b, int n_tiles) {
    extern __shared__ __attribute__((aligned(16))) unsigned char s_dyn[];
    uint64_t* run_key = reinterpret_cast<uint64_t*>(s_dyn);
    if (g.total[0] > b.capacity) return;
    const uint32_t limit = min((uint32_t)n_tiles, g.total[6]);
    for (uint32_t slot = blockIdx.x; slot < limit; slot += gridDim.x) {
        const uint32_t tile = g.tile_order[slot];
        const uint32_t start = g.tile_start[tile];
        const uint32_t n = g.tile_start[tile + 1] - start;
        if (n <= (uint32_t)CAP) continue;
        uint64_t* k0 = b.keys + start;
        uint64_t* k1 = b.keys_tmp + start;
        for (uint32_t c0 = 0; c0 < n; c0 += CAP) {
            const uint32_t m = min((uint32_t)CAP, n - c0);
            sort_block_lds<CAP, THREADS>(b, start + c0, m, run_key, [&](uint32_t rank, uint64_t key) { k0[c0 + rank] = key; });
        }
        for (uint32_t width = CAP; width < n; width <<= 1) {
            __threadfence();
            __syncthreads();
            for (uint32_t i = threadIdx.x; i < n; i += THREADS) {
                const uint32_t pair_base = (i / (2 * width)) * (2 * width);
                const uint32_t mid = min(pair_base + width, n), end = min(pair_base + 2 * width, n);
                const bool left = i < mid;
                const uint64_t key = ld_agent(k0 + i);
                uint32_t lo = left ? mid : pair_base, hi = left ? end : mid;
                while (lo < hi) {
                    const uint32_t mm = (lo + hi) >> 1;
                    if (ld_agent(k0 + mm) < key) lo = mm + 1; else hi = mm;
                }
                const uint32_t rank = lo - (left ? mid : pair_base);
                const uint32_t pos = pair_base + (i - (left ? pair_base : mid)) + rank;
                k1[pos] = key;
            }
            uint64_t* tk = k0; k0 = k1; k1 = tk;
        }
        __threadfence();
        __syncthreads();
        for (uint32_t i = threadIdx.x; i < n; i += THREADS) b.sorted_id[start + i] = (uint32_t)ld_agent(k0 + i);
        __syncthreads();
    }
}

void launch_sort_tiles(const ViewK& v, const Geom& g, const Binning& b, long long max_len, long long expected_len, hipStream_t st) {
    const int tiles = v.gx * v.gy;
    if (tiles <= 0) return;
    auto lds = [](int cap, int) { return (size_t)cap * 16; };
    hipLaunchKernelGGL(k_sort_tiles_regs, dim3(tiles), dim3(256), 0, st, g, b);
    if (max_len >= 0 && max_len <= 2048) return;
    allow_dynamic_lds(reinterpret_cast<const void*>(&k_sort_tiles_merge<2048, 4096, 1024>), 2, (int)lds(4096, 1024));
    allow_dynamic_lds(reinterpret_cast<const void*>(&k_sort_tiles_merge<4096, 8192, 1024>), 3, (int)lds(8192, 1024));
    allow_dynamic_lds(reinterpret_cast<const void*>(&k_sort_tiles_long<8192, 1024>), 4, (int)lds(8192, 1024));
    const int long_grid = tiles < 512 ? tiles : 512;
    auto grid_for = [&](long long lo) { return (expected_len >= 0 && expected_len <= lo) ? (long_grid < 8 ? long_grid : 8) : long_grid; };
    hipLaunchKernelGGL((k_sort_tiles_merge<2048, 4096, 1024>), dim3(grid_for(2048)), dim3(1024), lds(4096, 1024), st, g, b, tiles);
    if (max_len >= 0 && max_len <= 4096) return;
    hipLaunchKernelGGL((k_sort_tiles_merge<4096, 8192, 1024>), dim3(grid_for(4096)), dim3(1024), lds(8192, 1024), st, g, b, tiles);
    if (max_len >= 0 && max_len <= 8192) return;
    hipLaunchKernelGGL((k_sort_tiles_long<8192, 1024>), dim3(grid_for(8192)), dim3(1024), lds(8192, 1024), st, g, b, tiles);
}

}
```

splatfields_amd/csrc/common.h:

```cpp
#pragma once
#include <hip/hip_runtime.h>
#include <stdint.h>
#include "../../include/splatraster.h"

namespace sr {

constexpr int kTile = SR_TILE;
constexpr int kSub = 8;
constexpr float kNearCullZ = 0.2f;
constexpr float kDilation = 0.3f;
constexpr float kClampFov = 1.3f;
constexpr float kAlphaMax = 0.99f;
constexpr float kAlphaMin = 1.0f / 255.0f;
constexpr float kTStop = 0.0001f;
constexpr float kWEps = 0.0000001f;

constexpr float SH_C0 = 0.28209479177387814f;
constexpr float SH_C1 = 0.4886025119029199f;
constexpr float SH_C2_0 = 1.0925484305920792f, SH_C2_1 = -1.0925484305920792f, SH_C2_2 = 0.31539156525252005f,
                SH_C2_3 = -1.0925484305920792f, SH_C2_4 = 0.5462742152960396f;
constexpr float SH_C3_0 = -0.5900435899266435f, SH_C3_1 = 2.890611442640554f, SH_C3_2 = -0.4570457994644658f,
                SH_C3_3 = 0.3731763325901154f, SH_C3_4 = -0.4570457994644658f, SH_C3_5 = 1.445305721320277f,
                SH_C3_6 = -0.5900435899266435f;

constexpr int kBlock = 256;
constexpr int kWave = 64;

constexpr uint8_t kFlagClampR = 1, kFlagClampG = 2, kFlagClampB = 4, kFlagClampTx = 8, kFlagClampTy = 16;

struct Geom {
    float4* rec;
    ushort4* rect;
    uint32_t* touched;
    uint32_t* offsets;
    float* dcol_ddir;
    uint32_t* depth_bits;
    uint8_t* flags;
    uint32_t* block_sums;
    uint32_t* block_offsets;
    uint32_t* tile_count;
    uint32_t* tile_start;
    uint32_t* tile_cursor;
    uint32_t* tile_order;
    uint32_t* total;
    uint32_t* tile_qlast;
    uint32_t* cnt;
    uint32_t* segtot;
    uint32_t* segbase;
};

constexpr int kMaxChunks = 1024;
constexpr int kSegRows = 128;
constexpr int kMaxMatrixTiles = 16384;

struct Chunking { int n_sub, chunks, sub_per_chunk, slices, segments, tiles_padded; };
inline Chunking make_chunking(int N, int tiles) {
    Chunking c;
    c.n_sub = (N + 255) / 256; if (c.n_sub < 1) c.n_sub = 1;
    const int b = c.n_sub < kMaxChunks ? c.n_sub : kMaxChunks;
    c.sub_per_chunk = (c.n_sub + b - 1) / b;
    c.chunks = (c.n_sub + c.sub_per_chunk - 1) / c.sub_per_chunk;
    c.slices = 1;
    if (c.sub_per_chunk == 1) { c.slices = kMaxChunks / c.chunks; if (c.slices > 8) c.slices = 8; if (c.slices < 1) c.slices = 1; }
    c.chunks *= c.slices;
    c.segments = (c.chunks + kSegRows - 1) / kSegRows;
    c.tiles_padded = (tiles + 63) / 64 * 64;
    return c;
}

struct Binning {
    uint64_t* ent;
    uint64_t* keys;
    uint64_t* keys_tmp;
    uint32_t* sorted_id;
    uint32_t* qmask;
    uint8_t* reached;
    uint32_t capacity;
    uint32_t sorted_up_to;
};

struct Image {
    float* final_T;
    uint32_t* n_contrib;
};

__host__ __device__ inline size_t align_up(size_t x, size_t a) { return (x + a - 1) / a * a; }
inline bool aligned16(const void* p) { return (reinterpret_cast<uintptr_t>(p) & 15u) == 0; }

struct Carver {
    char* base; size_t off;
    template <typename T> __host__ T* take(size_t n) {
        off = align_up(off, 256);
        T* p = base ? reinterpret_cast<T*>(base + off) : nullptr;
        off += n * sizeof(T);
        return p;
    }
};

inline int tiles_x(int W) { return (W + kTile - 1) / kTile; }
inline int tiles_y(int H) { return (H + kTile - 1) / kTile; }

inline size_t carve_geom(void* base, int N, int H, int W, Geom* g) {
    Carver c{static_cast<char*>(base), 0};
    const size_t n = (size_t)(N > 0 ? N : 1);
    const size_t nb = (n + kBlock - 1) / kBlock;
    const size_t tiles = (size_t)tiles_x(W) * tiles_y(H);
    Geom t;
    t.rec = c.take<float4>(4 * n);
    t.rect = c.take<ushort4>(n);
    t.touched = c.take<uint32_t>(n); t.offsets = c.take<uint32_t>(n); t.depth_bits = c.take<uint32_t>(n);
    t.dcol_ddir = c.take<float>(9 * n);
    t.flags = c.take<uint8_t>(n);
    t.block_sums = c.take<uint32_t>(nb); t.block_offsets = c.take<uint32_t>(nb);
    t.tile_count = c.take<uint32_t>(tiles); t.tile_start = c.take<uint32_t>(tiles + 1);
    t.tile_cursor = c.take<uint32_t>(tiles); t.tile_order = c.take<uint32_t>(tiles); t.total = c.take<uint32_t>(8);
    t.tile_qlast = c.take<uint32_t>(16 * tiles);
    t.cnt = t.segtot = t.segbase = nullptr;
    if (tiles <= (size_t)kMaxMatrixTiles) {
        const Chunking ch = make_chunking(N, (int)tiles);
        t.cnt = c.take<uint32_t>((size_t)ch.chunks * ch.tiles_padded);
        t.segtot = c.take<uint32_t>((size_t)ch.segments * ch.tiles_padded);
        t.segbase = c.take<uint32_t>((size_t)ch.segments * ch.tiles_padded);
    }
    if (g) *g = t;
    return align_up(c.off, 256);
}

inline size_t carve_binning(void* base, long long R, Binning* b) {
    Carver c{static_cast<char*>(base), 0};
    const size_t r = (size_t)(R > 0 ? R : 1);
    Binning t;
    t.ent = c.take<uint64_t>(r);
    t.keys = c.take<uint64_t>(r);
    t.keys_tmp = c.take<uint64_t>(r);
    t.sorted_id = c.take<uint32_t>(r);
    t.qmask = c.take<uint32_t>(r);
    t.reached = c.take<uint8_t>(r);
    t.capacity = (uint32_t)(R > 0 ? R : 0);
    t.sorted_up_to = 0xffffffffu;
    if (b) *b = t;
    return align_up(c.off, 256);
}

inline size_t carve_image(void* base, int H, int W, Image* im) {
    Carver c{static_cast<char*>(base), 0};
    const size_t px = (size_t)H * W;
    Image t;
    t.final_T = c.take<float>(px); t.n_contrib = c.take<uint32_t>(px);
    if (im) *im = t;
    return align_up(c.off, 256);
}

constexpr int kSlotF4 = 3;
constexpr int kSlotFloats = 4 * kSlotF4;


struct ViewK {
    int H, W, gx, gy;
    float tanfovx, tanfovy, focal_x, focal_y, scale_modifier;
    int sh_degree, sh_coeffs;
    const float* viewmatrix; const float* projmatrix; const float* campos; const float* bg;
};

#ifdef __HIPCC__

__device__ __forceinline__ int lane_id() { return threadIdx.x & 63; }
__device__ __forceinline__ int wave_id() { return threadIdx.x >> 6; }

__device__ __forceinline__ float4 load_stream(const float4* p) {
    typedef float v4f_nt __attribute__((ext_vector_type(4)));
    const v4f_nt x = __builtin_nontemporal_load(reinterpret_cast<const v4f_nt*>(p));
    return make_float4(x.x, x.y, x.z, x.w);
}

__device__ __forceinline__ void store_stream(float4* p, const float4 v) {
    typedef float v4f_nt __attribute__((ext_vector_type(4)));
    const v4f_nt x = {v.x, v.y, v.z, v.w};
    __builtin_nontemporal_store(x, reinterpret_cast<v4f_nt*>(p));
}

__device__ __forceinline__ void lds_copy16_async(const void* src, uint32_t lds_base) {
    unsigned keep;
    asm volatile("s_mov_b32 %0, m0\n\ts_mov_b32 m0, %2\n\ts_nop 0\n\tglobal_load_lds_dwordx4 %1, off\n\ts_mov_b32 m0, %0"
                 : "=&s"(keep) : "v"(src), "s"(lds_base) : "memory");
}
__device__ __forceinline__ void lds_copy4_async(const void* src, uint32_t lds_base) {
    unsigned keep;
    asm volatile("s_mov_b32 %0, m0\n\ts_mov_b32 m0, %2\n\ts_nop 0\n\tglobal_load_lds_dword %1, off\n\ts_mov_b32 m0, %0"
                 : "=&s"(keep) : "v"(src), "s"(lds_base) : "memory");
}
__device__ __forceinline__ void lds_copy_wait() { asm volatile("s_waitcnt vmcnt(0)" ::: "memory"); }
__device__ __forceinline__ void lds_barrier() { asm volatile("s_waitcnt lgkmcnt(0)\n\ts_barrier" ::: "memory"); }
__device__ __forceinline__ uint32_t lds_address(const void* p) { return (uint32_t)(uintptr_t)p; }

template <int CTRL, int ROW_MASK = 0xf>
__device__ __forceinline__ float dpp_add(float v) {
    const int moved = __builtin_amdgcn_update_dpp(0, __float_as_int(v), CTRL, ROW_MASK, 0xf, false);
    return v + __int_as_float(moved);
}

__device__ __forceinline__ float wave_sum_to_lane63(float v) {
    v = dpp_add<0xB1>(v);
    v = dpp_add<0x4E>(v);
    v = dpp_add<0x124>(v);
    v = dpp_add<0x128>(v);
    v = dpp_add<0x142, 0xA>(v);
    v = dpp_add<0x143, 0xC>(v);
    return v;
}

__device__ __forceinline__ uint32_t wave_inclusive_scan(uint32_t v) {
    const int lane = lane_id();
#pragma unroll
    for (int d = 1; d < 64; d <<= 1) {
        const uint32_t n = __shfl_up(v, d, 64);
        if (lane >= d) v += n;
    }
    return v;
}

__device__ __forceinline__ uint32_t block_exclusive_scan(uint32_t v, uint32_t* scratch, uint32_t& total) {
    const uint32_t inc = wave_inclusive_scan(v);
    const int w = wave_id();
    __syncthreads();
    if (lane_id() == 63) scratch[w] = inc;
    __syncthreads();
    const uint32_t s0 = scratch[0], s1 = scratch[1], s2 = scratch[2], s3 = scratch[3];
    total = s0 + s1 + s2 + s3;
    const uint32_t wave_base = (w > 0 ? s0 : 0) + (w > 1 ? s1 : 0) + (w > 2 ? s2 : 0);
    return wave_base + inc - v;
}


__device__ __forceinline__ uint32_t block_exclusive_scan2(uint32_t a, uint32_t b, uint32_t* scratch, uint32_t& a_total, uint32_t& b_excl, uint32_t& b_total) {
    const uint32_t ia = wave_inclusive_scan(a), ib = wave_inclusive_scan(b);
    const int w = wave_id();
    __syncthreads();
    if (lane_id() == 63) { scratch[w] = ia; scratch[4 + w] = ib; }
    __syncthreads();
    const uint32_t s0 = scratch[0], s1 = scratch[1], s2 = scratch[2], s3 = scratch[3];
    const uint32_t t0 = scratch[4], t1 = scratch[5], t2 = scratch[6], t3 = scratch[7];
    a_total = s0 + s1 + s2 + s3;
    b_total = t0 + t1 + t2 + t3;
    b_excl = (w > 0 ? t0 : 0) + (w > 1 ? t1 : 0) + (w > 2 ? t2 : 0) + ib - b;
    return (w > 0 ? s0 : 0) + (w > 1 ? s1 : 0) + (w > 2 ? s2 : 0) + ia - a;
}

constexpr float kLog2e = 1.4426950408889634f;
__device__ __forceinline__ float pair_alpha_unclamped(float dx, float dy, const float4 f) {
    const float t = f.x * fmaf(f.y, dy, dx), u = f.z * dy;
    const float w = fmaf(u, u, fmaf(t, t, f.w));
    return __builtin_amdgcn_exp2f(-w);
}
__device__ __forceinline__ void exponent_terms(float cx, float cy, const float4 f, float tx0f, float ty0f, float& E0, float& F0, float& ps) {
    const float cxr = cx - tx0f, cyr = cy - ty0f;
    E0 = f.x * fmaf(f.y, cyr, cxr);
    F0 = f.z * cyr;
    ps = f.x * f.y;
}
__device__ __forceinline__ void pair_alpha_row(float Y, float E0, float F0, float ps, float q, float nlo, float& G0, float& K) {
    G0 = fmaf(-ps, Y, E0);
    const float L2 = fmaf(-q, Y, F0);
    K = fmaf(L2, L2, nlo);
}
__device__ __forceinline__ float pair_alpha_px(float X, float p, float G0, float K) {
    const float L1 = fmaf(-p, X, G0);
    return __builtin_amdgcn_exp2f(-fmaf(L1, L1, K));
}
__device__ __forceinline__ void conic_from_factors(const float4 f, float& A, float& B, float& C) {
#pragma clang fp contract(off)
    A = 2.0f * f.x * f.x;
    B = f.y * A;
    C = fmaf(2.0f * f.z, f.z, f.y * B);
}

__device__ __forceinline__ float edge_min(float a, float b2, float c, float inv_c, float fixed, float lo, float hi) {
#pragma clang fp contract(off)
    const float t = fminf(hi, fmaxf(lo, -0.5f * b2 * fixed * inv_c));
    return a * fixed * fixed + (b2 * fixed + c * t) * t;
}
__device__ __forceinline__ bool box_overlap(const float4 r0, const float4 r1, float sx, float sy, float extent) {
    const float tau = r0.z;
    if (!(tau > 0.0f)) return false;
    const float x0 = sx - r0.x, x1 = x0 + extent, y0 = sy - r0.y, y1 = y0 + extent;
    const bool in_x = x0 <= 0.0f && x1 >= 0.0f, in_y = y0 <= 0.0f && y1 >= 0.0f;
    if (in_x && in_y) return true;
    float A, B, C;
    conic_from_factors(r1, A, B, C);
    const float B2 = 2.0f * B;
    const float inv_a = __builtin_amdgcn_rcpf(A), inv_c = __builtin_amdgcn_rcpf(C);
    float fmin_ = edge_min(A, B2, C, inv_c, x0, y0, y1);
    fmin_ = fminf(fmin_, edge_min(A, B2, C, inv_c, x1, y0, y1));
// ... 49 lines not shown
```

splatfields_amd/csrc/kernels.h:

```cpp
#pragma once
#include "common.h"

namespace sr {

struct SplatsK {
    int N;
    const float* means3D; const float* opacities; const float* scales; const float* rotations;
    const float* cov3D; const float* shs; const float* colors;
    int raw;
    const float* shs_rest;
};

struct GradsK {
    float* means3D; float* means2D; float* opacity; float* scales; float* rotations; float* cov3D;
    float* shs; float* colors; float* shs_rest;
};

void launch_preprocess(const ViewK& v, const SplatsK& s, const Geom& g, int* radii, hipStream_t st);
void launch_mark_visible(int N, const float* means3D, const float* viewmatrix, unsigned char* present, hipStream_t st);
void launch_densification_stats(int N, const float* dL_dmeans2D, const int* radii, float* grad_accum, float* denom, float* max_radii2D,
                                hipStream_t st);
void launch_preprocess_backward(const ViewK& v, const SplatsK& s, const Geom& g, const int* radii,
                                const float* slots, const uint8_t* reached, const GradsK& gr, int first, int count, bool small_footprint,
                                hipStream_t st);
inline bool use_count_matrix(const ViewK& v) { return v.gx * v.gy <= kMaxMatrixTiles; }
void launch_count_tiles(const ViewK& v, int N, const Geom& g, hipStream_t st);
void launch_scan_small(const ViewK& v, int N, const Geom& g, uint32_t* host_out, uint32_t host_seq, hipStream_t st);
void launch_emit(const ViewK& v, int N, const Geom& g, const Binning& b, hipStream_t st);
void launch_sort_tiles(const ViewK& v, const Geom& g, const Binning& b, long long max_len, long long expected_len, hipStream_t st);
void launch_render_forward(const ViewK& v, const Geom& g, const Binning& b, const Image& im,
                           float* out_color, float* out_depth, float* out_alpha, hipStream_t st);
void launch_render_backward(const ViewK& v, const Geom& g, const Binning& b, const Image& im,
                            const float* dL_dcolor, const float* dL_ddepth, const float* dL_dalpha,
                            float* slots, hipStream_t st);
void launch_render_backward_quads(const ViewK& v, const Geom& g, const Binning& b, const Image& im,
                                 const float* dL_dcolor, const float* dL_ddepth, const float* dL_dalpha,
                                 float* slots, hipStream_t st);

int backward_stats(unsigned long long* out8, int reset);

}
```

splatfields_amd/csrc/render.hip:

```cpp
#include "kernels.h"
#define SR_QM_DEVICE 1
#include "quadmask.h"

namespace sr {

constexpr int kBwdBatch = 128;

__device__ __forceinline__ void wave_lds_fence() {
    __builtin_amdgcn_fence(__ATOMIC_RELEASE, "wavefront");
    __builtin_amdgcn_wave_barrier();
    __builtin_amdgcn_fence(__ATOMIC_ACQUIRE, "wavefront");
}

typedef unsigned int uint2v __attribute__((ext_vector_type(2)));

__device__ __forceinline__ float mask_select(uint64_t mask, float a, float b) {
    float r;
    asm("v_cndmask_b32_e64 %0, %1, %2, %3" : "=v"(r) : "v"(b), "v"(a), "s"(mask));
    return r;
}
__device__ __forceinline__ uint32_t mask_select(uint64_t mask, uint32_t a, uint32_t b) {
    uint32_t r;
    asm("v_cndmask_b32_e64 %0, %1, %2, %3" : "=v"(r) : "v"(b), "v"(a), "s"(mask));
    return r;
}

__device__ __forceinline__ float swap32_add(float x, float y) {
    const uint2v r = __builtin_amdgcn_permlane32_swap(__float_as_uint(x), __float_as_uint(y), false, false);
    return __uint_as_float(r.x) + __uint_as_float(r.y);
}
__device__ __forceinline__ float swap16_add(float x, float y) {
    const uint2v r = __builtin_amdgcn_permlane16_swap(__float_as_uint(x), __float_as_uint(y), false, false);
    return __uint_as_float(r.x) + __uint_as_float(r.y);
}

__device__ __forceinline__ void publish_tile_reach(const Geom& g, int tile, uint32_t last, int qx, int qy, int D1, int D2, int D3, int D4,
                                                   bool writer) {
    uint32_t ql = last;
    ql = max(ql, (uint32_t)__shfl_xor((int)ql, D1, 64));
    ql = max(ql, (uint32_t)__shfl_xor((int)ql, D2, 64));
    ql = max(ql, (uint32_t)__shfl_xor((int)ql, D3, 64));
    ql = max(ql, (uint32_t)__shfl_xor((int)ql, D4, 64));
    if (writer) g.tile_qlast[16 * (size_t)tile + 4 * qy + qx] = ql;
}

__global__ void __launch_bounds__(kBlock) k_render_forward(const ViewK v, const Geom g, const Binning b, const Image im,
                                                           float* __restrict__ out_color, float* __restrict__ out_depth,
                                                           float* __restrict__ out_alpha) {
    constexpr int kB = 256;
    static_assert(kB == 256 || kB == 128, "a batch is staged by four or by two wavefronts");
    constexpr int kStagers = kB / kWave;
    constexpr uint32_t kStep = 4 / kStagers;
    __shared__ float4 s_r0[1][kB];
    __shared__ float4 s_r1[1][kB];
    __shared__ float4 s_r2[1][kB];
    __shared__ uint16_t s_qm[1][kB];
    __shared__ uint32_t s_live[2][4];
    __shared__ uint8_t s_idx[4][4][kB + 4];
    static_assert(kB == 256, "the pipelined walk indexes the staging area with unmasked bytes: 256 slots");

    const uint32_t total_instances = g.total[0], longest_list = g.total[1];
    const int tile = (int)g.tile_order[blockIdx.x];
    asm volatile("" :: "s"(tile));
    if ((total_instances > b.capacity) | (longest_list > b.sorted_up_to)) {
        const int t = (int)blockIdx.x, lx = (int)threadIdx.x & 15, ly = (int)threadIdx.x >> 4;
        const int qx = (t % v.gx) * kTile + lx, qy = (t / v.gx) * kTile + ly;
        if (qx < v.W && qy < v.H) {
            const size_t hw = (size_t)v.H * v.W, pix = (size_t)qy * v.W + qx;
            const float nan = __builtin_nanf("");
            out_color[pix] = nan; out_color[hw + pix] = nan; out_color[2 * hw + pix] = nan;
            out_depth[pix] = nan;
            if (out_alpha) out_alpha[pix] = nan;
        }
        return;
    }
    const int tx = tile % v.gx, ty = tile / v.gx;
    const int wave = __builtin_amdgcn_readfirstlane(wave_id()), lane = lane_id();
    const int sx = tx * kTile + (wave & 1) * kSub, sy = ty * kTile + (wave >> 1) * kSub;
    const int qrow = lane >> 4;
    const int px = sx + 4 * (qrow & 1) + (lane & 3), py = sy + 4 * (qrow >> 1) + ((lane >> 2) & 3);
    const bool inside = px < v.W && py < v.H;
    const float tx0f = (float)(tx * kTile), ty0f = (float)(ty * kTile);
    const float Xf = (float)(px - tx * kTile), Yf = (float)(py - ty * kTile);
    const uint32_t start = g.tile_start[tile], end = g.tile_start[tile + 1];
    const uint32_t my_quads = 0x33u << (2 * (wave & 1) + 8 * (wave >> 1));

    float T = 1.0f, Cr = 0.f, Cg = 0.f, Cb = 0.f, D = 0.f;
    uint64_t livem = __builtin_amdgcn_ballot_w64(inside);
    uint32_t last = inside ? end - start : 0u;
    if (start == end) {
        goto done;
    }
    {
    auto stages = [&](uint32_t k) { return kStagers == 4 || (uint32_t)(wave >> 1) == (k & 1u); };
    const int slot = kStagers == 4 ? (int)threadIdx.x : (int)(threadIdx.x & 127u);
    const int wslot = kStagers == 4 ? wave : (wave & 1);
    const uint32_t l0 = lds_address(&s_r0[0][wslot * kWave]), l1 = lds_address(&s_r1[0][wslot * kWave]), l2 = lds_address(&s_r2[0][wslot * kWave]);
    constexpr uint32_t kCopyStride = kB * sizeof(float4);
    auto request = [&](int buf, uint32_t id) {
        const float4* rec = g.rec + 4 * (size_t)id;
        lds_copy16_async(rec, l0 + buf * kCopyStride);
        lds_copy16_async(rec + 1, l1 + buf * kCopyStride);
        lds_copy16_async(rec + 2, l2 + buf * kCopyStride);
    };
    auto publish_mask = [&](int buf, uint32_t i) {
        uint32_t qm = 0u;
        if (i < end) {
            const float4 r0 = s_r0[buf][slot], r1 = s_r1[buf][slot];
            qm = sr_quad_mask(r0.x, r0.y, r0.z, r1.x, r1.y, r1.z, tx0f, ty0f);
            b.qmask[i] = qm;
            float E0, F0, ps;
            exponent_terms(r0.x, r0.y, r1, tx0f, ty0f, E0, F0, ps);
            *reinterpret_cast<float2*>(&s_r0[buf][slot]) = make_float2(E0, F0);
            s_r1[buf][slot].y = ps;
        }
        s_qm[buf][slot] = (uint16_t)qm;
    };
    const uint32_t lastpos = end - 1u;
    const uint32_t i0 = start + (uint32_t)slot;
    const uint32_t k_first = kStagers == 4 ? 1u : ((wave >> 1) == 1 ? 1u : 2u);
    uint32_t id_nxt = b.sorted_id[min(i0 + k_first * kB, lastpos)];
    if (stages(0u)) {
        const uint32_t id0 = b.sorted_id[min(i0, lastpos)];
        request(0, id0);
        lds_copy_wait();
        publish_mask(0, i0);
    }
    asm volatile("" :: "v"(id_nxt));
    lds_barrier();

    uint32_t k = 0;
    for (uint32_t base = start; base < end; base += kB, ++k) {
        const bool more = base + kB < end;
        constexpr int buf = 0, nbuf = 0;
        asm volatile("" :: "v"(id_nxt));
        const int cnt = (int)min((uint32_t)kB, end - base);
        if (livem != 0ull) {
            uint32_t qlen[4] = {0u, 0u, 0u, 0u};
            const int qbit0 = 4 * (2 * (wave >> 1)) + 2 * (wave & 1);
            for (int c = 0; c < cnt; c += kWave) {
                const int el = c + lane;
                const uint32_t qm = el < cnt ? (uint32_t)s_qm[buf][el] : 0u;
#pragma unroll
                for (int j = 0; j < 4; ++j) {
                    const bool ok = ((qm >> (qbit0 + (j & 1) + 4 * (j >> 1))) & 1u) != 0u;
                    const uint64_t m = __builtin_amdgcn_ballot_w64(ok);
                    const uint32_t rank = __builtin_amdgcn_mbcnt_hi((uint32_t)(m >> 32), __builtin_amdgcn_mbcnt_lo((uint32_t)m, 0u));
                    if (ok) s_idx[wave][j][qlen[j] + rank] = (uint8_t)el;
                    qlen[j] += (uint32_t)__popcll(m);
                }
            }
            wave_lds_fence();
            const uint32_t my_len = qrow == 0 ? qlen[0] : qrow == 1 ? qlen[1] : qrow == 2 ? qlen[2] : qlen[3];
            const uint32_t n_trip = (uint32_t)__builtin_amdgcn_readfirstlane((int)max(max(qlen[0], qlen[1]), max(qlen[2], qlen[3])));
            const uint8_t* my_idx = &s_idx[wave][qrow][0];
            const uint32_t posb = base - start;
            struct Rec { float2 ef; float4 r1, r2; };
            auto fetch = [&](uint32_t e) { Rec r; r.ef = *reinterpret_cast<const float2*>(&s_r0[buf][e]); r.r1 = s_r1[buf][e]; r.r2 = s_r2[buf][e]; return r; };
            auto trip = [&](uint32_t i, uint32_t e, const Rec& rc) -> bool {
                float G0, K;
                pair_alpha_row(Yf, rc.ef.x, rc.ef.y, rc.r1.y, rc.r1.z, rc.r1.w, G0, K);
                const float alpha = fminf(kAlphaMax, pair_alpha_px(Xf, rc.r1.x, G0, K));
                const float test_T = T * (1.0f - alpha);
                const uint64_t hitm = __builtin_amdgcn_ballot_w64(alpha >= kAlphaMin) & __builtin_amdgcn_ballot_w64(i < my_len) & livem;
                const uint64_t stopm = __builtin_amdgcn_ballot_w64(test_T < kTStop) & hitm;
                const uint64_t blendm = hitm ^ stopm;
                livem &= ~stopm;
                const float w = mask_select(blendm, alpha * T, 0.0f);
                Cr = fmaf(rc.r2.x, w, Cr); Cg = fmaf(rc.r2.y, w, Cg); Cb = fmaf(rc.r2.z, w, Cb); D = fmaf(rc.r2.w, w, D);
                T = mask_select(blendm, test_T, T);
                if (stopm != 0ull) {
                    last = mask_select(stopm, posb + e, last);
                    return livem == 0ull;
                }
                return false;
            };
            if (n_trip != 0u) {
                uint32_t ea = my_idx[0], eb = my_idx[1];
                Rec ra = fetch(ea);
#pragma unroll 1
                for (uint32_t i = 0;;) {
                    const Rec rb = fetch(eb);
                    const uint32_t ea_n = my_idx[i + 2];
                    if (trip(i, ea, ra)) break;
                    if (++i >= n_trip) break;
                    ra = fetch(ea_n);
                    const uint32_t eb_n = my_idx[i + 2];
                    if (trip(i, eb, rb)) break;
                    if (++i >= n_trip) break;
                    ea = ea_n; eb = eb_n;
                }
            }
        }
        if (!more) break;
        if (lane == 0) s_live[k & 1u][wave] = livem != 0ull ? 1u : 0u;
        lds_barrier();
        if ((s_live[k & 1u][0] | s_live[k & 1u][1] | s_live[k & 1u][2] | s_live[k & 1u][3]) == 0u) break;
        if (stages(k + 1u)) request(0, id_nxt);
        if (stages(k + 1u)) {
            lds_copy_wait();
            id_nxt = b.sorted_id[min(base + (1u + kStep) * kB + (uint32_t)slot, lastpos)];
            publish_mask(nbuf, base + kB + (uint32_t)slot);
        }
        lds_barrier();
    }
    }
done:
    if (inside) {
        const size_t hw = (size_t)v.H * v.W, pix = (size_t)py * v.W + px;
        out_color[pix] = Cr + T * v.bg[0];
        out_color[hw + pix] = Cg + T * v.bg[1];
        out_color[2 * hw + pix] = Cb + T * v.bg[2];
        out_depth[pix] = D;
        if (out_alpha) out_alpha[pix] = 1.0f - T;
        im.final_T[pix] = T;
        im.n_contrib[pix] = last;
    }
    publish_tile_reach(g, tile, last,  2 * (wave & 1) + (qrow & 1), 2 * (wave >> 1) + (qrow >> 1),
                        1, 2, 4, 8, (lane & 15) == 0);
}

void launch_render_forward(const ViewK& v, const Geom& g, const Binning& b, const Image& im,
                           float* out_color, float* out_depth, float* out_alpha, hipStream_t st) {
    const int tiles = v.gx * v.gy;
    if (tiles > 0) hipLaunchKernelGGL(k_render_forward, dim3(tiles), dim3(kBlock), 0, st, v, g, b, im, out_color, out_depth, out_alpha);
}

template <bool HAS_D, bool HAS_A>
__global__ void __launch_bounds__(kBlock) k_render_backward(const ViewK v, const Geom g, const Binning b, const Image im,
                                                            const float* __restrict__ dL_dcolor,
                                                            const float* __restrict__ dL_ddepth,
                                                            const float* __restrict__ dL_dalpha,
                                                            float* __restrict__ slots) {
    __shared__ float4 s_r0[kBwdBatch + 1];
    __shared__ float4 s_r1[kBwdBatch + 1];
    __shared__ float4 s_r2[kBwdBatch + 1];
    __shared__ float4 s_acc[4][kBwdBatch][3];
    __shared__ float2 s_ef[kBwdBatch + 1];
    __shared__ uint32_t s_max[4];

    const int tile = (int)g.tile_order[blockIdx.x];
    const int tx = tile % v.gx, ty = tile / v.gx;
    const int wave = wave_id(), lane = lane_id();
    const int sx = tx * kTile + (wave & 1) * kSub, sy = ty * kTile + (wave >> 1) * kSub;
    const int px = sx + (lane & 7), py = sy + (lane >> 3);
    const bool inside = px < v.W && py < v.H;
    const float pxf = (float)px, pyf = (float)py, sxf = (float)sx, syf = (float)sy;
    const float tx0f = (float)(tx * kTile), ty0f = (float)(ty * kTile);
// ... 149 lines not shown
```

splatfields_amd/rasterizer.py:

```python
from __future__ import annotations

import contextlib
import ctypes as C
import math
import os
import threading
import weakref
from typing import NamedTuple, Optional

import torch
from torch import nn

from . import _lib


class GaussianRasterizationSettings(NamedTuple):
    image_height: int
    image_width: int
    tanfovx: float
    tanfovy: float
    bg: torch.Tensor
    scale_modifier: float
    viewmatrix: torch.Tensor
    projmatrix: torch.Tensor
    sh_degree: int
    campos: torch.Tensor
    prefiltered: bool
    debug: bool


def settings_from_camera(cam, bg, sh_degree, scale_modifier=1.0, debug=False) -> GaussianRasterizationSettings:
    return GaussianRasterizationSettings(
        image_height=int(cam.image_height), image_width=int(cam.image_width), tanfovx=math.tan(cam.FoVx * 0.5),
        tanfovy=math.tan(cam.FoVy * 0.5), bg=bg, scale_modifier=scale_modifier, viewmatrix=cam.world_view_transform,
        projmatrix=cam.full_proj_transform, sh_degree=sh_degree, campos=cam.camera_center, prefiltered=False, debug=bool(debug))


LAST_INSTANCES = 0

_DEPTH_GRADIENT = os.environ.get("SPLATRASTER_DEPTH_GRAD", "1") not in ("0", "false", "False", "off")


def set_depth_gradient(enabled: bool) -> bool:
    global _DEPTH_GRADIENT
    prev, _DEPTH_GRADIENT = _DEPTH_GRADIENT, bool(enabled)
    return prev


def depth_gradient_enabled() -> bool:
    return _DEPTH_GRADIENT

_ASYNC = {"1": True, "true": True, "True": True, "on": True, "0": False, "false": False, "False": False, "off": False}.get(
    os.environ.get("SPLATRASTER_ASYNC", ""), None)
_HEADROOM = 1.25


class RasterizerOverflow(RuntimeError):
    """An asynchronously launched forward (sr_forward_async) met more tile-splat instances, or a longer tile list, than the
    last render of that view had promised: it has no result (its outputs are NaN).  The estimates have been corrected; render
    again."""


def set_async_forward(enabled) -> "Optional[bool]":
    global _ASYNC
    prev, _ASYNC = _ASYNC, (None if enabled is None else bool(enabled))
    return prev


class async_forward:

    def __init__(self, enabled: bool = True):
        self.enabled = bool(enabled)

    def __enter__(self):
        self.prev = getattr(_TLS, "async_scope", None)
        _TLS.async_scope = self.enabled
        return self

    def __exit__(self, *exc):
        _TLS.async_scope = self.prev
        return False


def async_forward_enabled() -> bool:
    if _ASYNC is not None:
        return _ASYNC
    return bool(getattr(_TLS, "async_scope", None))


def host_sync_counters(reset: bool = False) -> dict:
    out = (C.c_longlong * 4)()
    _lib.check(_lib.load().sr_debug_counters(out, 1 if reset else 0))
    return {"forward_host_waits": int(out[0]), "async_forwards": int(out[1]), "tickets_waited_for": int(out[2]),
            "tickets_created": int(out[3])}


_BWD_KERNELS = {None: 0, "auto": 0, "wave": 1, "quads": 2}


def set_backward_kernel(which) -> str:
    prev = _lib.load().sr_set_backward_kernel(_BWD_KERNELS[which])
    return {0: "auto", 1: "wave", 2: "quads"}[prev]


def _round_capacity(instances: int) -> int:
    c = max(int(instances * _HEADROOM) + 1024, 1 << 16)
    step = 1 << (c.bit_length() - 4)
    return (c + step - 1) // step * step


def _covered_by_hint(hint: int) -> int:
    return 2048 if hint <= 2048 else 4096 if hint <= 4096 else 8192 if hint <= 8192 else 1 << 62


class _Promise(NamedTuple):
    key: tuple
    capacity: int
    hint: Optional[int] = None
    expected: int = -1
    covered: int = 0


class _Estimates:

    CAPACITY_ROWS = 4096
    SEEN_ROWS = 64

    def __init__(self):
        self.capacity = {}
        self.per_splat = {}
        self.lock = threading.Lock()

    def plan(self, device_index: int, n: int, H: int, W: int, view, may_async: bool) -> _Promise:
        key = (device_index, n, H, W)
        with self.lock:
            ratio = self.per_splat.get((device_index, H, W))
            capacity = self.capacity.get(key) or (max(4 * n, 1 << 16) if ratio is None else _round_capacity(int(ratio * n)))
            before = view.seen.get(n) if may_async else None
        if before is None or _round_capacity(before[0]) > capacity:
            return _Promise(key, capacity)
        hint = int(before[1] * _HEADROOM) + 1
        return _Promise(key, capacity, hint, int(before[1]), _covered_by_hint(hint))

    def record(self, promise: _Promise, view, instances: int, longest: int) -> None:
        global LAST_INSTANCES
        dev, n, H, W = key = promise.key
        rkey = (dev, H, W)
        with self.lock:
            self.capacity[key] = max(self.capacity.get(key, 0), _round_capacity(instances))
            if len(self.capacity) > self.CAPACITY_ROWS:
                self.capacity.clear()
            self.per_splat[rkey] = max(self.per_splat.get(rkey, 0.0), instances / max(n, 1))
            if longest >= 0:
                if len(view.seen) > self.SEEN_ROWS:
                    view.seen.clear()
                view.seen[n] = (int(instances), int(longest))
            LAST_INSTANCES = instances


_ESTIMATES = _Estimates()
_TLS = threading.local()
_PENDING_LOCK = threading.Lock()


class _Pending:

    def __init__(self, lib, ticket, promise: _Promise, view):
        self.lib, self.ticket, self.promise, self.view = lib, ticket, promise, view
        self.outcome = None
        lst = getattr(_TLS, "pending", None)
        if lst is None:
            lst = _TLS.pending = []
        with _PENDING_LOCK:
            if len(lst) > 64:
                lst[:] = [r for r in lst if r() is not None]
            lst.append(weakref.ref(self))
        self._list = lst

    def resolve(self) -> int:
        if self.ticket is not None:
            ticket, self.ticket = self.ticket, None
            try:
                self.outcome = self._redeem(ticket)
            except Exception as e:
                self.outcome = e
        if isinstance(self.outcome, Exception):
            raise self.outcome
        return self.outcome

    def _redeem(self, ticket):
        inst, longest = C.c_longlong(0), C.c_longlong(0)
        rc = self.lib.sr_ticket_wait(ticket, C.byref(inst), C.byref(longest))
        with _PENDING_LOCK:
            self._list[:] = [r for r in self._list if r() is not None and r() is not self]
        _lib.check(rc)
        instances, longest, promise = int(inst.value), int(longest.value), self.promise
        _ESTIMATES.record(promise, self.view, instances, longest)
        covered = max(promise.covered, 2048)
        if instances > promise.capacity or longest > covered:
            return RasterizerOverflow(
                f"the forward of this view was launched without waiting for its instance count (sr_forward_async) for at most "
                f"{promise.capacity} tile-splat instances and tile lists of up to {covered} entries, but the view has "
                f"{instances} instances and a list of {longest}: it has no result (its outputs are NaN).  Nothing has been applied "
                f"and the estimates are corrected: re-run the step (or splatfields_amd.rasterizer.set_async_forward(False))")
        return instances

    def __del__(self):
        t, self.ticket = getattr(self, "ticket", None), None
        if t is not None:
            try:
                self.lib.sr_ticket_release(t)
            except Exception:
                pass


def resolve_pending() -> None:
    err = None
    with _PENDING_LOCK:
        refs = list(getattr(_TLS, "pending", None) or [])
    for ref in refs:
        p = ref()
        if p is None:
            continue
        try:
            p.resolve()
        except RasterizerOverflow as e:
            err = err or e
    if err is not None:
        raise err


def redeemed(render_fn, scope: bool = False):
    with async_forward() if scope else contextlib.nullcontext():
        out = render_fn()
        try:
            resolve_pending()
        except RasterizerOverflow:
            out = render_fn()
            resolve_pending()
    return out


def _ptr(t: Optional[torch.Tensor]) -> Optional[int]:
    return None if t is None else t.data_ptr()


def _f32c(t: Optional[torch.Tensor], device) -> Optional[torch.Tensor]:
    if t is None:
        return None
    if t.dtype is torch.float32 and t.device == device and t.is_contiguous():
        return t
    return t.detach().to(device=device, dtype=torch.float32).contiguous()


def _opt(t: Optional[torch.Tensor]) -> Optional[torch.Tensor]:
    return None if (t is None or t.numel() == 0) else t


class _ViewPack:

    _cache: "dict" = {}
    _CACHE_MAX = 256

    @classmethod
    def get(cls, rs: GaussianRasterizationSettings, device, sh_coeffs: int) -> "_ViewPack":
        src = (rs.viewmatrix, rs.projmatrix, rs.campos)
        key = (id(src[0]), id(src[1]), id(src[2]), int(rs.image_height), int(rs.image_width), float(rs.tanfovx),
               float(rs.tanfovy), float(rs.scale_modifier), int(rs.sh_degree), int(sh_coeffs), bool(rs.prefiltered),
               bool(rs.debug), device)
        versions = (src[0]._version, src[1]._version, src[2]._version)
        hit = cls._cache.get(key)
        if hit is not None and hit[1] == versions and all(a is b for a, b in zip(hit[2], src)):
            pack = hit[0]
            if pack.bg_src is rs.bg and pack.bg_version == rs.bg._version:
                return pack
            return pack.with_bg(rs.bg, device)
        pack = cls(rs, device, sh_coeffs)
        while len(cls._cache) >= cls._CACHE_MAX:
            cls._cache.pop(next(iter(cls._cache)))
        cls._cache[key] = (pack, versions, src)
        return pack

    def __init__(self, rs: GaussianRasterizationSettings, device, sh_coeffs: int):
        self.viewmatrix = _f32c(rs.viewmatrix, device).reshape(-1)
        self.projmatrix = _f32c(rs.projmatrix, device).reshape(-1)
        self.campos = _f32c(rs.campos, device).reshape(-1)
        if self.viewmatrix.numel() != 16 or self.projmatrix.numel() != 16:
            raise RuntimeError("viewmatrix and projmatrix must hold 16 elements ([4,4] or [1,4,4])")
        if self.campos.numel() != 3:
            raise RuntimeError("campos and bg must hold 3 elements")
        self.seen = {}
        self._fields = (int(rs.image_height), int(rs.image_width), float(rs.tanfovx), float(rs.tanfovy),
                        float(rs.scale_modifier), int(rs.sh_degree), int(sh_coeffs), int(bool(rs.prefiltered)),
                        int(bool(rs.debug)))
        self._set_bg(rs.bg, device)

    def _set_bg(self, bg: torch.Tensor, device) -> None:
        self.bg_src, self.bg_version = bg, bg._version
        self.bg = _f32c(bg, device).reshape(-1)
        if self.bg.numel() != 3:
            raise RuntimeError("campos and bg must hold 3 elements")
        self.struct = _lib.SrView(*self._fields, self.viewmatrix.data_ptr(), self.projmatrix.data_ptr(),
                                  self.campos.data_ptr(), self.bg.data_ptr())

    def with_bg(self, bg: torch.Tensor, device) -> "_ViewPack":
        other = object.__new__(_ViewPack)
        other.viewmatrix, other.projmatrix, other.campos = self.viewmatrix, self.projmatrix, self.campos
        other.seen, other._fields = self.seen, self._fields
        other._set_bg(bg, device)
        return other


def _splats_struct(n, means3D, opacities, scales, rotations, cov3D, shs, colors, raw_params: int = 0, shs_rest=None) -> _lib.SrSplats:
    return _lib.SrSplats(int(n), *map(_ptr, (means3D, opacities, scales, rotations, cov3D, shs, colors)), int(raw_params), _ptr(shs_rest))


def _aligned16(t: Optional[torch.Tensor]) -> Optional[torch.Tensor]:
    return t if (t is None or t.data_ptr() % 16 == 0) else t.clone()


def _check_inputs(means3D, sh, colors_precomp, opacities, scales, rotations, cov3Ds_precomp, sh_rest, slice_hook, color_grad_sink):
    if not means3D.is_cuda:
        raise RuntimeError("splatfields_amd rasterizer has no CPU path: tensors must be on a HIP ('cuda') device")
    dev = means3D.device
    if means3D.dim() != 2 or means3D.shape[1] != 3:
        raise RuntimeError("means3D must have dimensions (num_points, 3)")
    n = means3D.shape[0]
    f = lambda t: _f32c(t, dev)
    means3D_c, opac_c = f(means3D), f(opacities).reshape(-1)
    sh_c, col_c, sc_c, rot_c, cov_c = f(_opt(sh)), f(_opt(colors_precomp)), f(_opt(scales)), f(_opt(rotations)), f(_opt(cov3Ds_precomp))
    if opac_c.numel() != n:
        raise RuntimeError("opacities must have dimensions (num_points, 1)")
    for name, t, last in (("shs", sh_c, None), ("colors_precomp", col_c, 3), ("scales", sc_c, 3),
                          ("rotations", rot_c, 4), ("cov3D_precomp", cov_c, 6)):
        if t is not None and (t.shape[0] != n or (last is not None and t.shape[-1] != last)):
            raise RuntimeError(f"{name} has an unexpected shape {tuple(t.shape)} for {n} points")
    if sh_c is not None and (sh_c.dim() != 3 or sh_c.shape[2] != 3):
        raise RuntimeError("shs must have dimensions (num_points, K, 3)")
    sh_coeffs = 0 if sh_c is None else int(sh_c.shape[1])
    rest_c = None
    if _opt(sh_rest) is not None:
        rest_c = _aligned16(f(sh_rest))
        sh_c = _aligned16(sh_c)
        if sh_c is None or sh_c.shape[1] != 1 or rest_c.dim() != 3 or tuple(rest_c.shape) != (n, 15, 3):
            raise RuntimeError("with shs_rest, shs must be [N,1,3] (dc) and shs_rest [N,15,3]")
        sh_coeffs = 16

    if slice_hook is not None:
        if cov_c is not None:
            raise ValueError("slice_hook requires scales / rotations inputs (cov3D_precomp is not supported in the sliced backward)")
        if rest_c is not None:
            raise ValueError("slice_hook requires the concatenated shs tensor (shs_rest is not supported in the sliced backward)")
        if sh_c is not None and color_grad_sink is None:
            raise ValueError("slice_hook requires color_grad_sink on the SH path (the sliced backward hands over colour gradients)")
    return means3D_c, opac_c, sc_c, rot_c, cov_c, sh_c, col_c, rest_c, sh_coeffs


def _launch_forward(lib, view, splats, n: int, H: int, W: int, dev, may_async: bool, radii, color, depth, alpha):
    with torch.cuda.device(dev):
        stream = _lib.stream(dev)
        geom = torch.empty(lib.sr_geom_bytes(n, H, W), dtype=torch.uint8, device=dev)
        image = torch.empty(lib.sr_image_bytes(H, W), dtype=torch.uint8, device=dev)
        promise = _ESTIMATES.plan(dev.index, n, H, W, view, may_async)
        capacity = promise.capacity
        binning = torch.empty(lib.sr_binning_bytes(capacity, H, W), dtype=torch.uint8, device=dev)
        state, outs = (C.byref(view.struct), C.byref(splats), _ptr(geom)), (_ptr(image), _ptr(color), _ptr(depth), _ptr(alpha))
        if promise.hint is not None:
            ticket = C.c_void_p()
            _lib.check(lib.sr_forward_async(*state, _ptr(radii), _ptr(binning), capacity, promise.hint, promise.expected, *outs,
                                            C.byref(ticket), stream))
            return geom, binning, image, capacity, None, _Pending(lib, ticket, promise, view)
        inst = C.c_longlong(0)
        status = lib.sr_forward(*state, _ptr(radii), _ptr(binning), capacity, *outs, C.byref(inst), stream)
        if status != _lib.SR_NEED_CAPACITY:
            _lib.check(status)
        instances = int(inst.value)
        _ESTIMATES.record(promise, view, instances, int(lib.sr_last_longest_list()))
        if status == _lib.SR_NEED_CAPACITY:
            capacity = _round_capacity(instances)
            binning = torch.empty(lib.sr_binning_bytes(capacity, H, W), dtype=torch.uint8, device=dev)
            _lib.check(lib.sr_forward_render(*state, _ptr(binning), capacity, *outs, stream))
    return geom, binning, image, capacity, instances, None


class _RasterizeGaussians(torch.autograd.Function):

    @staticmethod
    def forward(ctx, means3D, means2D, sh, colors_precomp, opacities, scales, rotations, cov3Ds_precomp,
                raster_settings: GaussianRasterizationSettings, color_grad_sink=None, raw_params: int = 0, sh_rest=None,
                slice_hook=None, grad_mode: bool = True):
        lib = _lib.load()
        means3D_c, opac_c, sc_c, rot_c, cov_c, sh_c, col_c, rest_c, sh_coeffs = _check_inputs(
            means3D, sh, colors_precomp, opacities, scales, rotations, cov3Ds_precomp, sh_rest, slice_hook, color_grad_sink)
        dev, n = means3D.device, means3D.shape[0]
        H, W = int(raster_settings.image_height), int(raster_settings.image_width)
        view = _ViewPack.get(raster_settings, dev, sh_coeffs)
        color, depth, alpha = (torch.empty(c, H, W, dtype=torch.float32, device=dev) for c in (3, 1, 1))
        radii = torch.empty(n, dtype=torch.int32, device=dev)
        ctx.raster_settings, ctx.color_grad_sink, ctx.slice_hook = raster_settings, color_grad_sink, slice_hook
        if not grad_mode or (not any(ctx.needs_input_grad[:8]) and not (len(ctx.needs_input_grad) > 11 and ctx.needs_input_grad[11])):
            raw_params = int(raw_params) | _lib.SR_FORWARD_ONLY
        ctx.raw_params = int(raw_params)
        ctx.n = n
        ctx.opac_shape = tuple(opacities.shape)
        ctx.in_dtypes = [None if t is None else t.dtype for t in (means3D, means2D, sh, colors_precomp, opacities, scales, rotations, cov3Ds_precomp)]
        ctx.rest_dtype = None if rest_c is None else sh_rest.dtype
        ctx.set_materialize_grads(False)
        ctx.mark_non_differentiable(radii)
        if n == 0:
            color[:] = view.bg.reshape(3, 1, 1)
            depth.zero_()
            alpha.zero_()
            ctx.instances = 0
            ctx.pending = None
            ctx.save_for_backward()
            return color, radii, depth, alpha

        splats = _splats_struct(n, means3D_c, opac_c, sc_c, rot_c, cov_c, sh_c, col_c, raw_params, rest_c)
        may_async = async_forward_enabled() and not (ctx.raw_params & _lib.SR_FORWARD_ONLY)
        geom, binning, image, ctx.capacity, ctx.instances, ctx.pending = _launch_forward(
            lib, view, splats, n, H, W, dev, may_async, radii, color, depth, alpha)
        ctx.view_pack = view
        ctx.save_for_backward(means3D_c, opac_c, sc_c, rot_c, cov_c, sh_c, col_c, radii, geom, binning, image, rest_c)
        return color, radii, depth, alpha

    @staticmethod
    def backward(ctx, grad_color, grad_radii, grad_depth, grad_alpha):
        rs = ctx.raster_settings
        n = ctx.n
        if n == 0:
            return (None,) * 14
        lib = _lib.load()
        if ctx.pending is not None:
            ctx.instances = ctx.pending.resolve()
        means3D, opac, sc, rot, cov, sh, col, radii, geom, binning, image, sh_rest = ctx.saved_tensors
        dev = means3D.device
        H, W = int(rs.image_height), int(rs.image_width)
        g = lambda t: _f32c(t, dev)
        grad_color = g(grad_color)
        if grad_color is None:
            grad_color = torch.zeros(3, H, W, dtype=torch.float32, device=dev)
        grad_depth, grad_alpha = g(grad_depth if _DEPTH_GRADIENT else None), g(grad_alpha)
        view = ctx.view_pack
        new = lambda *shape: torch.empty(*shape, dtype=torch.float32, device=dev)
        hook = ctx.slice_hook
        sink = ctx.color_grad_sink if sh is not None else None
        if hook is not None:
            assert cov is None and sh_rest is None and (sh is None or sink is not None)
            hb = hook.buffers(n)
            d_means3D, d_sc, d_rot, d_opac, d_col = hb["means3D"], hb["scales"], hb["rotations"], hb["opacities"], hb["colors"]
            d_means2D, d_cov, d_sh, d_rest = new(n, 3), None, None, None
        else:
            d_means3D, d_means2D, d_opac = new(n, 3), new(n, 3), new(n, 1)
            d_sc = new(n, 3) if sc is not None else None
            d_rot = new(n, 4) if rot is not None else None
            d_cov = new(n, 6) if cov is not None else None
            d_sh = new(*sh.shape) if (sh is not None and sink is None) else None
            d_col = new(n, 3) if (col is not None or sink is not None) else None
            d_rest = new(*sh_rest.shape) if (sh_rest is not None and d_sh is not None) else None
        with torch.cuda.device(dev):
            stream = _lib.stream(dev)
            splats = _splats_struct(n, means3D, opac, sc, rot, cov, sh, col, ctx.raw_params, sh_rest)
            scratch = torch.empty(lib.sr_backward_scratch_bytes(ctx.capacity), dtype=torch.uint8, device=dev)
            grads = _lib.SrGrads(*map(_ptr, (d_means3D, d_means2D, d_opac, d_sc, d_rot, d_cov, d_sh, d_col, d_rest)))
            if hook is None:
                _lib.check(lib.sr_backward(C.byref(view.struct), C.byref(splats), _ptr(geom), _ptr(binning), ctx.capacity, ctx.instances,
                                           _ptr(image), _ptr(radii), _ptr(grad_color), _ptr(grad_depth), _ptr(grad_alpha),
                                           _ptr(scratch), C.byref(grads), stream))
            else:
                _lib.check(lib.sr_backward_blend(C.byref(view.struct), C.byref(splats), _ptr(geom), _ptr(binning), ctx.capacity,
                                                 ctx.instances, _ptr(image), _ptr(grad_color), _ptr(grad_depth), _ptr(grad_alpha),
                                                 _ptr(scratch), stream))
                for j, (lo, hi) in enumerate(slice_ranges(n, hook.slices)):
                    _lib.check(lib.sr_backward_splats(C.byref(view.struct), C.byref(splats), _ptr(geom), _ptr(binning), ctx.capacity,
                                                      ctx.instances, _ptr(image), _ptr(radii), _ptr(scratch), C.byref(grads), lo, hi - lo, stream))
                    hook.on_slice(j, lo, hi)
        if hook is not None:
            return (None, d_means2D) + (None,) * 12
        if sink is not None:
            sink.append(d_col)
            d_col = None
        grads = [d_means3D, d_means2D, d_sh, d_col, d_opac.reshape(ctx.opac_shape), d_sc, d_rot, d_cov]
        grads = [g_ if (g_ is None or dt is None or g_.dtype == dt) else g_.to(dt) for g_, dt in zip(grads, ctx.in_dtypes)]
        if d_rest is not None and ctx.rest_dtype is not None and d_rest.dtype != ctx.rest_dtype:
            d_rest = d_rest.to(ctx.rest_dtype)
        return (*grads, None, None, None, d_rest, None, None)


def slice_ranges(n: int, slices: int) -> list:
    per = -(-n // max(int(slices), 1))
    per = max(256, -(-per // 256) * 256)
    return [(lo, min(lo + per, n)) for lo in range(0, n, per)]


def rasterize_gaussians(means3D, means2D, sh, colors_precomp, opacities, scales, rotations, cov3Ds_precomp,
                        raster_settings, color_grad_sink=None, raw_params: int = 0, sh_rest=None, slice_hook=None):
    return _RasterizeGaussians.apply(means3D, means2D, sh, colors_precomp, opacities, scales, rotations,
                                     cov3Ds_precomp, raster_settings, color_grad_sink, raw_params, sh_rest, slice_hook,
                                     torch.is_grad_enabled())


class GaussianRasterizer(nn.Module):
    def __init__(self, raster_settings: GaussianRasterizationSettings):
        super().__init__()
        self.raster_settings = raster_settings

    def markVisible(self, positions: torch.Tensor) -> torch.Tensor:
        lib = _lib.load()
        if not positions.is_cuda:
            raise RuntimeError("splatfields_amd rasterizer has no CPU path: tensors must be on a HIP ('cuda') device")
        with torch.no_grad():
            rs = self.raster_settings
            dev = positions.device
            pos = positions.detach().to(torch.float32).contiguous()
            vm, pj = _f32c(rs.viewmatrix, dev), _f32c(rs.projmatrix, dev)
            present = torch.zeros(pos.shape[0], dtype=torch.uint8, device=dev)
            with torch.cuda.device(dev):
                _lib.check(lib.sr_mark_visible(pos.shape[0], _ptr(pos), _ptr(vm), _ptr(pj), _ptr(present), _lib.stream(dev)))
        return present.bool()

    def _check(self, shs, colors_precomp, scales, rotations, cov3D_precomp):
        if (shs is None and colors_precomp is None) or (shs is not None and colors_precomp is not None):
            raise Exception('Please provide excatly one of either SHs or precomputed colors!')
        if ((scales is None or rotations is None) and cov3D_precomp is None) or \
                ((scales is not None or rotations is not None) and cov3D_precomp is not None):
            raise Exception('Please provide exactly one of either scale/rotation pair or precomputed 3D covariance!')

    def forward_ex(self, means3D, means2D, opacities, shs=None, colors_precomp=None, scales=None, rotations=None,
                   cov3D_precomp=None, color_grad_sink=None, shs_rest=None, slice_hook=None):
        self._check(shs, colors_precomp, scales, rotations, cov3D_precomp)
# ... 103 lines not shown
```

Measured before the change: 1303000 billion.

## Sort long tiles inside blend kernel when few exist, skipping standalone sort launch

Moves the bitonic/merge tile-sort helpers into a shared header and lets the forward render kernel sort tiles of up to 4096 entries inline when only a handful of long tiles exist. The emit stage now publishes a long-tile count to the host status block, and the host carries it as a per-view hint so the async path can choose a sort class without waiting. The aim is to drop or shrink the separate long-tile sort launch and its serialization. In exchange there is extra status-block synchronization, more host bookkeeping, and heavier blend blocks on tiles that are sorted inline.

```diff
diff --git a/include/splatraster.h b/include/splatraster.h
--- a/include/splatraster.h
+++ b/include/splatraster.h
@@ -81,6 +81,8 @@
                      float* out_color, float* out_depth, float* out_alpha, void** ticket_out, void* hip_stream);
 int sr_ticket_wait(void* ticket, long long* instances_out, long long* longest_list_out);
 long long sr_last_longest_list(void);
+long long sr_last_long_tiles(void);
+int sr_expect_long_tiles(long long tiles);
 int sr_ticket_release(void* ticket);
 
 #define SR_BWD_SLOT_SPEC_BELOW 6
@@ -97,6 +99,8 @@
                        const SrGrads* grads, int first_splat, int n_splats, void* hip_stream);
 
 int sr_set_backward_kernel(int which);
+
+int sr_set_sort_kernel(int which);
 
 int sr_mark_visible(int n_splats, const float* means3D, const float* viewmatrix,
                     const float* projmatrix, unsigned char* present, void* hip_stream);
@@ -453,6 +457,8 @@
 
 int sr_debug_counters(long long* out4, int reset);
 
+int sr_debug_sort_counters(long long* out4, int reset);
+
 int sr_debug_snapshot(const SrView* view, const SrSplats* splats, const float* dL_dcolor, const float* dL_ddepth,
                       const float* dL_dalpha, int backward);
 
diff --git a/splatfields_amd/_lib.py b/splatfields_amd/_lib.py
--- a/splatfields_amd/_lib.py
+++ b/splatfields_amd/_lib.py
@@ -132,7 +132,10 @@
     "sr_ticket_wait": (C.c_int, [C.c_void_p, C.POINTER(C.c_longlong), C.POINTER(C.c_longlong)]),
     "sr_ticket_release": (C.c_int, [C.c_void_p]),
     "sr_last_longest_list": (C.c_longlong, []),
+    "sr_last_long_tiles": (C.c_longlong, []),
+    "sr_expect_long_tiles": (C.c_int, [C.c_longlong]),
     "sr_debug_counters": (C.c_int, [C.POINTER(C.c_longlong), C.c_int]),
+    "sr_debug_sort_counters": (C.c_int, [C.POINTER(C.c_longlong), C.c_int]),
     "sr_backward": (C.c_int, [C.POINTER(SrView), C.POINTER(SrSplats), C.c_void_p, C.c_void_p, C.c_longlong, C.c_longlong, C.c_void_p,
                               C.c_void_p, C.c_void_p, C.c_void_p, C.c_void_p, C.c_void_p, C.POINTER(SrGrads),
                               C.c_void_p]),
@@ -142,6 +145,7 @@
                                      C.c_void_p, C.POINTER(SrGrads), C.c_int, C.c_int, C.c_void_p]),
     "sr_debug_snapshot": (C.c_int, [C.POINTER(SrView), C.POINTER(SrSplats), C.c_void_p, C.c_void_p, C.c_void_p, C.c_int]),
     "sr_set_backward_kernel": (C.c_int, [C.c_int]),
+    "sr_set_sort_kernel": (C.c_int, [C.c_int]),
     "sr_sh_forward": (C.c_int, [C.c_int, C.c_int, C.c_int, C.c_void_p, C.c_void_p, C.c_void_p, C.c_void_p, C.c_void_p, C.c_void_p]),
     "sr_sh_forward_views": (C.c_int, [C.c_int, C.c_int, C.c_int, C.c_int, C.c_void_p, C.c_void_p, C.c_void_p, C.c_void_p, C.c_void_p, C.c_void_p]),
     "sr_sh_backward": (C.c_int, [C.c_int, C.c_int, C.c_int, C.c_int, C.c_void_p, C.c_void_p, C.c_void_p, C.c_void_p, C.c_float,
diff --git a/splatfields_amd/build.py b/splatfields_amd/build.py
--- a/splatfields_amd/build.py
+++ b/splatfields_amd/build.py
@@ -10,7 +10,7 @@
 LIB_PATH = PKG_DIR / "libsplatraster.so"
 STATS_LIB_PATH = PKG_DIR / "libsplatraster_stats.so"
 SOURCES = ["api.hip", "preprocess.hip", "binning.hip", "render.hip", "blend_bwd.hip", "knn.hip", "sh.hip", "densify.hip", "mlp.hip", "triplane.hip", "loss.hip", "moran.hip", "adam.hip", "metrics.hip", "objective.hip", "planegen.hip", "attention.hip", "hull.hip", "flow_head.hip", "view_color.hip"]
-HEADERS = ["common.h", "kernels.h", "host_api.h", "expand.h", "sh_stage.h", "quadmask.h", "reduce.h", "window11.h", "point_tile.h", "mlp_bf16x3.h", "../../include/splatraster.h"]
+HEADERS = ["common.h", "kernels.h", "host_api.h", "expand.h", "sh_stage.h", "quadmask.h", "reduce.h", "window11.h", "point_tile.h", "mlp_bf16x3.h", "sort_tile.h", "../../include/splatraster.h"]
 
 
 def _hipcc() -> str:
diff --git a/splatfields_amd/csrc/api.hip b/splatfields_amd/csrc/api.hip
--- a/splatfields_amd/csrc/api.hip
+++ b/splatfields_amd/csrc/api.hip
@@ -64,6 +64,7 @@
 std::mutex g_ticket_mutex;
 std::vector<StatusBlock*> g_ticket_free[64];
 std::atomic<long long> g_counters[4];
+std::atomic<long long> g_sort_counters[4];
 
 int status_block_init(StatusBlock& b, int dev) {
     if (hipHostMalloc(reinterpret_cast<void**>(&b.pinned), 64, hipHostMallocCoherent) != hipSuccess &&
@@ -82,7 +83,7 @@
 }
 int status_block_wait(StatusBlock& b, bool* waited) {
     volatile uint32_t* p = b.pinned;
-    auto ready = [&] { return p[2] == b.seq && p[3] == b.seq; };
+    auto ready = [&] { return p[2] == b.seq && p[3] == b.seq && p[5] == b.seq; };
     if (waited) *waited = false;
     if (!ready()) {
         if (waited) *waited = true;
@@ -134,6 +135,12 @@
     return !sel ? 0 : (std::string(sel) == "wave" ? 1 : (std::string(sel) == "quads" ? 2 : 0));
 }()};
 
+std::atomic<int> g_sort_kernel{[] {
+    const char* sel = getenv("SPLATRASTER_SORT");
+    return !sel ? 0 : (std::string(sel) == "standalone" ? 1 : (std::string(sel) == "short" ? 2 : 0));
+}()};
+thread_local long long g_last_long_tiles = -1;
+thread_local long long g_expect_long_tiles = -1;
 
 struct CallContext { const SrView* view = nullptr; const SrSplats* splats = nullptr; const char* file = nullptr;
                      const float* dL_dcolor = nullptr; const float* dL_ddepth = nullptr; const float* dL_dalpha = nullptr; };
@@ -292,18 +299,25 @@
     return 0;
 }
 
-int launch_stage2(const SrView* view, const sr::ViewK& v, const sr::SplatsK& s, const sr::Geom& g, const sr::Binning& b,
+int launch_stage2(const SrView* view, const sr::ViewK& v, const sr::SplatsK& s, const sr::Geom& g, const sr::Binning& b_in,
                   const sr::Image& im, float* out_color, float* out_depth, float* out_alpha, StatusBlock* hs, long long max_len,
-                  long long expected_len, hipStream_t st) {
+                  long long expected_len, long long long_tiles, hipStream_t st) {
+    sr::Binning b = b_in;
+    const int who = g_sort_kernel.load(std::memory_order_relaxed);
+    b.sort_in_blend = who == 1 ? 0u : (who == 2 ? 2048u : 4096u);
     { StageTimer t_(2, st); sr::launch_emit(v, s.N, g, b, st); }
     SR_TRY(after_launch(view, st, "emit"));
     if (hs) {
         g_counters[0].fetch_add(1, std::memory_order_relaxed);
         SR_TRY(status_block_wait(*hs, nullptr));
         max_len = (long long)hs->pinned[1];
+        long_tiles = (long long)hs->pinned[4];
         if ((long long)hs->pinned[0] > (long long)b.capacity) return 0;
     }
-    { StageTimer t_(3, st); sr::launch_sort_tiles(v, g, b, max_len, expected_len, st); }
+    int classes = 0;
+    { StageTimer t_(3, st); classes = sr::launch_sort_tiles(v, g, b, max_len, expected_len, long_tiles, st); }
+    b.long_class_launched = (classes & 2) ? 1u : 0u;
+    for (int k = 0; k < 4; ++k) if (classes & (1 << k)) g_sort_counters[k].fetch_add(1, std::memory_order_relaxed);
     SR_TRY(after_launch(view, st, "sort_tiles"));
     { StageTimer t_(4, st); sr::launch_render_forward(v, g, b, im, out_color, out_depth, out_alpha, st); }
     SR_TRY(after_launch(view, st, "render_forward"));
@@ -339,10 +353,11 @@
     StatusBlock* hs = nullptr;
     SR_TRY(thread_block(&hs));
     SR_TRY(launch_stage1(view, c.v, c.s, c.g, radii, hs->pinned_dev, status_block_arm(*hs, c.st), c.st));
-    SR_TRY(launch_stage2(view, c.v, c.s, c.g, c.b, c.im, out_color, out_depth, out_alpha, hs, -1, -1, c.st));
+    SR_TRY(launch_stage2(view, c.v, c.s, c.g, c.b, c.im, out_color, out_depth, out_alpha, hs, -1, -1, -1, c.st));
     const long long total = (long long)hs->pinned[0];
     *instances_out = total;
     g_last_longest = (long long)hs->pinned[1];
+    g_last_long_tiles = (long long)hs->pinned[4];
     return total > binning_capacity ? SR_NEED_CAPACITY : 0;
 }
 
@@ -354,7 +369,7 @@
     if (!geom || !binning || !image || !out_color || !out_depth) return fail("null buffer");
     if (!capacity_in_range(instances)) return fail("instance count out of range");
     c.carve(geom, binning, instances, image);
-    return launch_stage2(view, c.v, c.s, c.g, c.b, c.im, out_color, out_depth, out_alpha, nullptr, -1, -1, c.st);
+    return launch_stage2(view, c.v, c.s, c.g, c.b, c.im, out_color, out_depth, out_alpha, nullptr, -1, -1, -1, c.st);
 }
 
 int sr_forward_async(const SrView* view, const SrSplats* splats, void* geom, int* radii, void* binning,
@@ -368,11 +383,14 @@
     c.carve(geom, binning, binning_capacity, image);
     const long long covered = covered_by_hint(longest_list_hint);
     c.b.sorted_up_to = covered < 0 ? 0xffffffffu : (uint32_t)covered;
+    const long long long_tiles = g_expect_long_tiles;
+    g_expect_long_tiles = -1;
     StatusBlock* t = nullptr;
     SR_TRY(ticket_acquire(&t));
     int rc = launch_stage1(view, c.v, c.s, c.g, radii, t->pinned_dev, status_block_arm(*t, c.st), c.st);
     if (!rc) rc = launch_stage2(view, c.v, c.s, c.g, c.b, c.im, out_color, out_depth, out_alpha, nullptr, covered,
-                                longest_list_expected >= 0 && longest_list_expected <= longest_list_hint ? longest_list_expected : -1, c.st);
+                                longest_list_expected >= 0 && longest_list_expected <= longest_list_hint ? longest_list_expected : -1,
+                                long_tiles, c.st);
     if (rc) {
         (void)hipStreamSynchronize(c.st);
         ticket_recycle(t);
@@ -394,17 +412,26 @@
     }
     if (instances_out) *instances_out = (long long)t->pinned[0];
     if (longest_list_out) *longest_list_out = (long long)t->pinned[1];
+    g_last_long_tiles = (long long)t->pinned[4];
     ticket_recycle(t);
     return 0;
 }
 
 long long sr_last_longest_list(void) { return g_last_longest; }
+long long sr_last_long_tiles(void) { return g_last_long_tiles; }
+int sr_expect_long_tiles(long long tiles) { g_expect_long_tiles = tiles < 0 ? -1 : tiles; return 0; }
 
 int sr_ticket_release(void* ticket) { return sr_ticket_wait(ticket, nullptr, nullptr); }
 
 int sr_debug_counters(long long* out4, int reset) {
     if (!out4) return fail("null pointer in sr_debug_counters");
     for (int i = 0; i < 4; ++i) out4[i] = reset ? g_counters[i].exchange(0, std::memory_order_relaxed) : g_counters[i].load(std::memory_order_relaxed);
+    return 0;
+}
+
+int sr_debug_sort_counters(long long* out4, int reset) {
+    if (!out4) return fail("null pointer in sr_debug_sort_counters");
+    for (int i = 0; i < 4; ++i) out4[i] = reset ? g_sort_counters[i].exchange(0, std::memory_order_relaxed) : g_sort_counters[i].load(std::memory_order_relaxed);
     return 0;
 }
 
@@ -483,6 +510,11 @@
     return g_bwd_kernel.exchange(which, std::memory_order_relaxed);
 }
 
+int sr_set_sort_kernel(int which) {
+    if (which < 0 || which > 2) return -1;
+    return g_sort_kernel.exchange(which, std::memory_order_relaxed);
+}
+
 int sr_mark_visible(int n, const float* means3D, const float* viewmatrix, const float*, unsigned char* present, void* hip_stream) {
     if (n < 0 || (n > 0 && (!means3D || !viewmatrix || !present))) return fail("bad arguments to sr_mark_visible");
     hipStream_t st = static_cast<hipStream_t>(hip_stream);
diff --git a/splatfields_amd/csrc/binning.hip b/splatfields_amd/csrc/binning.hip
--- a/splatfields_amd/csrc/binning.hip
+++ b/splatfields_amd/csrc/binning.hip
@@ -1,6 +1,7 @@
 #include <atomic>
 #include "kernels.h"
 #include "expand.h"
+#include "sort_tile.h"
 
 namespace sr {
 
@@ -187,6 +188,7 @@
                 cand = cls >= 255u ? (uint32_t)n : s_hist[cls + 1u];
             }
             g.total[4 + tid] = cand;
+            if (tid == 0 && host_out) { host_out[4] = cand; __hip_atomic_store(host_out + 5, host_seq, __ATOMIC_RELEASE, __HIP_MEMORY_SCOPE_SYSTEM); }
         }
         __syncthreads();
         if (in_regs) {
@@ -316,201 +318,16 @@
         hipLaunchKernelGGL(k_emit<false>, dim3(ch.n_sub), dim3(kBlock), 0, st, v, N, g, b, ch);
 }
 
-template <int D>
-__device__ __forceinline__ uint32_t lane_xor(uint32_t x) {
-    if constexpr (D == 1) return (uint32_t)__builtin_amdgcn_update_dpp(0, (int)x, 0xB1, 0xf, 0xf, false);
-    else if constexpr (D == 2) return (uint32_t)__builtin_amdgcn_update_dpp(0, (int)x, 0x4E, 0xf, 0xf, false);
-    else if constexpr (D == 8) return (uint32_t)__builtin_amdgcn_update_dpp(0, (int)x, 0x128, 0xf, 0xf, false);
-    else if constexpr (D == 4) {
-        const uint32_t a = (uint32_t)__builtin_amdgcn_update_dpp(0, (int)x, 0x124, 0xf, 0xf, false);
-        const uint32_t b = (uint32_t)__builtin_amdgcn_update_dpp(0, (int)x, 0x12C, 0xf, 0xf, false);
-        return (threadIdx.x & 4u) ? a : b;
-    } else if constexpr (D == 16) {
-        typedef unsigned int u2 __attribute__((ext_vector_type(2)));
-        const u2 r = __builtin_amdgcn_permlane16_swap(x, x, false, false);
-        return (threadIdx.x & 16u) ? r.x : r.y;
-    } else {
-        typedef unsigned int u2 __attribute__((ext_vector_type(2)));
-        const u2 r = __builtin_amdgcn_permlane32_swap(x, x, false, false);
-        return (threadIdx.x & 32u) ? r.x : r.y;
-    }
-}
-
-__device__ __forceinline__ uint32_t lane_xor_d(uint32_t x, int d) {
-    switch (d) {
-        case 1: return lane_xor<1>(x);
-        case 2: return lane_xor<2>(x);
-        case 4: return lane_xor<4>(x);
-        case 8: return lane_xor<8>(x);
-        case 16: return lane_xor<16>(x);
-        default: return lane_xor<32>(x);
-    }
-}
-
-__device__ __forceinline__ void exchange_select(uint64_t& k, uint64_t pk, bool keep_min) {
-    const bool take = (pk < k) == keep_min;
-    k = take ? pk : k;
-}
-
-template <int N, int E>
-__device__ __forceinline__ void bitonic_regs(uint64_t (&k)[E], uint64_t* skey, uint32_t tid) {
-#pragma unroll
-    for (int kk = 2; kk <= N; kk <<= 1) {
-#pragma unroll
-        for (int j = kk >> 1; j > 0; j >>= 1) {
-            if (j < E) {
-#pragma unroll
-                for (int e = 0; e < E; ++e) {
-                    if ((e & j) == 0) {
-                        const uint32_t i = tid * E + e;
-                        const bool asc = (i & kk) == 0;
-                        const bool swap = (k[e] > k[e | j]) == asc;
-                        const uint64_t ka = k[e], kb = k[e | j];
-                        k[e] = swap ? kb : ka; k[e | j] = swap ? ka : kb;
-                    }
-                }
-            } else if (j < 64 * E) {
-                const int d = j / E;
-                const bool lower = (tid & d) == 0;
-                const bool keep_min = lower == (((tid * E) & kk) == 0);
-                uint32_t plo[E], phi[E];
-#pragma unroll
-                for (int e = 0; e < E; ++e) {
-                    plo[e] = lane_xor_d((uint32_t)k[e], d);
-                    phi[e] = lane_xor_d((uint32_t)(k[e] >> 32), d);
-                }
-#pragma unroll
-                for (int e = 0; e < E; ++e) exchange_select(k[e], ((uint64_t)phi[e] << 32) | plo[e], keep_min);
-            } else {
-                __syncthreads();
-#pragma unroll
-                for (int e = 0; e < E; ++e) skey[tid * E + e] = k[e];
-                __syncthreads();
-#pragma unroll
-                for (int e = 0; e < E; ++e) {
-                    const uint32_t i = tid * E + e;
-                    const bool asc = (i & kk) == 0;
-                    const bool lower = (i & j) == 0;
-                    exchange_select(k[e], skey[i ^ j], lower == asc);
-                }
-            }
-        }
-    }
-}
-
-template <int N, int E>
-__device__ __forceinline__ void load_sort_chunk(const Binning& b, uint32_t first, uint32_t m, uint64_t (&k)[E], uint64_t* scratch_key, uint32_t tid) {
-#pragma unroll
-    for (int e = 0; e < E; ++e) {
-        const uint32_t i = tid * E + e;
-        k[e] = i < m ? b.ent[first + i] : ~0ull;
-    }
-    bitonic_regs<N, E>(k, scratch_key, tid);
-}
-
-template <int N, int E>
-__device__ __forceinline__ void sort_tile_regs(const Binning& b, uint32_t start, uint32_t n, uint64_t* skey) {
-    uint64_t k[E];
-    load_sort_chunk<N, E>(b, start, n, k, skey, threadIdx.x);
-#pragma unroll
-    for (int e = 0; e < E; ++e) {
-        const uint32_t i = threadIdx.x * E + e;
-        if (i < n) b.sorted_id[start + i] = (uint32_t)k[e];
-    }
-}
-
-template <int CAP, int THREADS, typename Emit>
-__device__ __forceinline__ void sort_block_lds(const Binning& b, uint32_t first, uint32_t n, uint64_t* run_key, Emit&& emit);
-
 __global__ void __launch_bounds__(256) k_sort_tiles_regs(const Geom g, const Binning b) {
-    __shared__ uint64_t skey[2048];
+    __shared__ uint64_t skey[kSortSmallMax];
     const uint32_t total_instances = g.total[0];
     const uint32_t tile = g.tile_order[blockIdx.x];
     asm volatile("" :: "s"(tile));
     if (total_instances > b.capacity) return;
     const uint32_t start = g.tile_start[tile];
     const uint32_t n = g.tile_start[tile + 1] - start;
-    if (n == 0u || n > 2048u) return;
-    if (n <= 256u) sort_tile_regs<256, 1>(b, start, n, skey);
-    else if (n <= 512u) sort_tile_regs<512, 2>(b, start, n, skey);
-    else if (n <= 1024u) sort_tile_regs<1024, 4>(b, start, n, skey);
-    else sort_block_lds<2048, 256>(b, start, n, skey, [&](uint32_t rank, uint64_t key) { b.sorted_id[start + rank] = (uint32_t)key; });
-}
-
-template <int E, typename Out>
-__device__ __forceinline__ void merge_run_pairs(const uint64_t* src, uint32_t n, uint32_t width, Out&& out) {
-    const uint32_t o = threadIdx.x * (uint32_t)E;
-    if (o >= n) return;
-    const uint32_t base = o & ~(2u * width - 1u);
-    const uint64_t* A = src + base;
-    const uint32_t a = min(width, n - base);
-    const uint32_t b = n - base - a < width ? n - base - a : width;
-    const uint32_t d = o - base;
-    uint32_t lo = d > b ? d - b : 0u, hi = min(d, a);
-    while (lo < hi) {
-        const uint32_t mid = (lo + hi) >> 1;
-        if (A[mid] < A[width + d - 1u - mid]) lo = mid + 1u; else hi = mid;
-    }
-    uint32_t ai = lo, bi = d - lo;
-    constexpr uint64_t kInf = ~0ull;
-    uint64_t ka = ai < a ? A[ai] : kInf;
-    uint64_t kb = bi < b ? A[width + bi] : kInf;
-#pragma unroll
-    for (int e = 0; e < E; ++e) {
-        const bool take_a = ka < kb;
-        const uint64_t key = take_a ? ka : kb;
-        if (d + (uint32_t)e < a + b) out(o + (uint32_t)e, key);
-        ai += take_a ? 1u : 0u;
-        bi += take_a ? 0u : 1u;
-        const bool more = take_a ? ai < a : bi < b;
-        const uint64_t nxt = A[take_a ? min(ai, a - 1u) : width + min(bi, max(b, 1u) - 1u)];
-        if (take_a) ka = more ? nxt : kInf; else kb = more ? nxt : kInf;
-    }
-}
-
-template <int CAP, int THREADS, typename Emit>
-__device__ __forceinline__ void sort_block_lds(const Binning& b, uint32_t first, uint32_t n, uint64_t* run_key, Emit&& emit) {
-    constexpr int GROUPS = THREADS / 256;
-    const uint32_t group = threadIdx.x >> 8, tid = threadIdx.x & 255u;
-    const uint32_t n_runs = (n + 1023u) / 1024u;
-    for (uint32_t r0 = 0; r0 < n_runs; r0 += GROUPS) {
-        const uint32_t r = r0 + group;
-        const uint32_t m = r < n_runs ? min(1024u, n - r * 1024u) : 0u;
-        __syncthreads();
-        uint64_t* rk = run_key + r * 1024u;
-        uint64_t k[4];
-        if (m <= 256u) {
-            uint64_t k1[1];
-            load_sort_chunk<256, 1>(b, first + r * 1024u, m, k1, rk, tid);
-            k[0] = k1[0];
-        } else if (m <= 512u) {
-            uint64_t k2[2];
-            load_sort_chunk<512, 2>(b, first + r * 1024u, m, k2, rk, tid);
-            k[0] = k2[0]; k[1] = k2[1];
-        } else {
-            load_sort_chunk<1024, 4>(b, first + r * 1024u, m, k, rk, tid);
-        }
-        __syncthreads();
-        const uint32_t per = m <= 256u ? 1u : (m <= 512u ? 2u : 4u);
-#pragma unroll
-        for (int e = 0; e < 4; ++e) {
-            const uint32_t i = tid * per + e;
-            if ((uint32_t)e < per && i < m) rk[i] = k[e];
-        }
-    }
-    __syncthreads();
-    uint64_t* src = run_key;
-    uint64_t* dst = run_key + CAP;
-    for (uint32_t width = 1024u;; width <<= 1) {
-        if (2u * width >= n) {
-            merge_run_pairs<CAP / THREADS>(src, n, width, emit);
-            break;
-        }
-        merge_run_pairs<CAP / THREADS>(src, n, width, [&](uint32_t pos, uint64_t key) { dst[pos] = key; });
-        __syncthreads();
-        uint64_t* t = src; src = dst; dst = t;
-    }
-    __syncthreads();
+    if (n == 0u || n > kSortSmallMax) return;
+    sort_tile_small(b, start, n, skey);
 }
 
 template <int LO, int CAP, int THREADS>
@@ -519,6 +336,7 @@
     uint64_t* run_key = reinterpret_cast<uint64_t*>(s_dyn);
     if (g.total[0] > b.capacity) return;
     const uint32_t limit = min((uint32_t)n_tiles, g.total[LO == 2048 ? 4 : 5]);
+    if (LO == 2048 && b.sort_in_blend >= kSortInlineMax && few_long_tiles(g.total[4], g.total[1])) return;
     for (uint32_t slot = blockIdx.x; slot < limit; slot += gridDim.x) {
         const uint32_t tile = g.tile_order[slot];
         const uint32_t start = g.tile_start[tile];
@@ -574,22 +392,32 @@
     }
 }
 
-void launch_sort_tiles(const ViewK& v, const Geom& g, const Binning& b, long long max_len, long long expected_len, hipStream_t st) {
+int launch_sort_tiles(const ViewK& v, const Geom& g, const Binning& b, long long max_len, long long expected_len, long long long_tiles,
+                      hipStream_t st) {
     const int tiles = v.gx * v.gy;
-    if (tiles <= 0) return;
+    if (tiles <= 0) return 0;
+    int launched = 0;
     auto lds = [](int cap, int) { return (size_t)cap * 16; };
-    hipLaunchKernelGGL(k_sort_tiles_regs, dim3(tiles), dim3(256), 0, st, g, b);
-    if (max_len >= 0 && max_len <= 2048) return;
+    if (b.sort_in_blend < kSortSmallMax) { hipLaunchKernelGGL(k_sort_tiles_regs, dim3(tiles), dim3(256), 0, st, g, b); launched |= 1; }
+    if (max_len >= 0 && max_len <= 2048) return launched;
     allow_dynamic_lds(reinterpret_cast<const void*>(&k_sort_tiles_merge<2048, 4096, 1024>), 2, (int)lds(4096, 1024));
     allow_dynamic_lds(reinterpret_cast<const void*>(&k_sort_tiles_merge<4096, 8192, 1024>), 3, (int)lds(8192, 1024));
     allow_dynamic_lds(reinterpret_cast<const void*>(&k_sort_tiles_long<8192, 1024>), 4, (int)lds(8192, 1024));
     const int long_grid = tiles < 512 ? tiles : 512;
     auto grid_for = [&](long long lo) { return (expected_len >= 0 && expected_len <= lo) ? (long_grid < 8 ? long_grid : 8) : long_grid; };
-    hipLaunchKernelGGL((k_sort_tiles_merge<2048, 4096, 1024>), dim3(grid_for(2048)), dim3(1024), lds(4096, 1024), st, g, b, tiles);
-    if (max_len >= 0 && max_len <= 4096) return;
+    const long long longest = expected_len >= 0 ? expected_len : max_len;
+    const bool leave_to_blend = b.sort_in_blend >= kSortInlineMax && long_tiles >= 0 && long_tiles <= (long long)kInlineLongTiles &&
+                                longest >= 0 && longest <= (long long)kSortInlineMax;
+    if (!leave_to_blend) {
+        hipLaunchKernelGGL((k_sort_tiles_merge<2048, 4096, 1024>), dim3(grid_for(2048)), dim3(1024), lds(4096, 1024), st, g, b, tiles);
+        launched |= 2;
+    }
+    if (max_len >= 0 && max_len <= 4096) return launched;
     hipLaunchKernelGGL((k_sort_tiles_merge<4096, 8192, 1024>), dim3(grid_for(4096)), dim3(1024), lds(8192, 1024), st, g, b, tiles);
-    if (max_len >= 0 && max_len <= 8192) return;
+    launched |= 4;
+    if (max_len >= 0 && max_len <= 8192) return launched;
     hipLaunchKernelGGL((k_sort_tiles_long<8192, 1024>), dim3(grid_for(8192)), dim3(1024), lds(8192, 1024), st, g, b, tiles);
-}
-
-}
+    return launched | 8;
+}
+
+}
diff --git a/splatfields_amd/csrc/common.h b/splatfields_amd/csrc/common.h
--- a/splatfields_amd/csrc/common.h
+++ b/splatfields_amd/csrc/common.h
@@ -77,6 +77,8 @@
     uint8_t* reached;
     uint32_t capacity;
     uint32_t sorted_up_to;
+    uint32_t sort_in_blend;
+    uint32_t long_class_launched;
 };
 
 struct Image {
@@ -138,6 +140,8 @@
     t.reached = c.take<uint8_t>(r);
     t.capacity = (uint32_t)(R > 0 ? R : 0);
     t.sorted_up_to = 0xffffffffu;
+    t.sort_in_blend = 0u;
+    t.long_class_launched = 1u;
     if (b) *b = t;
     return align_up(c.off, 256);
 }
diff --git a/splatfields_amd/csrc/kernels.h b/splatfields_amd/csrc/kernels.h
--- a/splatfields_amd/csrc/kernels.h
+++ b/splatfields_amd/csrc/kernels.h
@@ -27,7 +27,8 @@
 void launch_count_tiles(const ViewK& v, int N, const Geom& g, hipStream_t st);
 void launch_scan_small(const ViewK& v, int N, const Geom& g, uint32_t* host_out, uint32_t host_seq, hipStream_t st);
 void launch_emit(const ViewK& v, int N, const Geom& g, const Binning& b, hipStream_t st);
-void launch_sort_tiles(const ViewK& v, const Geom& g, const Binning& b, long long max_len, long long expected_len, hipStream_t st);
+int launch_sort_tiles(const ViewK& v, const Geom& g, const Binning& b, long long max_len, long long expected_len, long long long_tiles,
+                      hipStream_t st);
 void launch_render_forward(const ViewK& v, const Geom& g, const Binning& b, const Image& im,
                            float* out_color, float* out_depth, float* out_alpha, hipStream_t st);
 void launch_render_backward(const ViewK& v, const Geom& g, const Binning& b, const Image& im,
diff --git a/splatfields_amd/csrc/render.hip b/splatfields_amd/csrc/render.hip
--- a/splatfields_amd/csrc/render.hip
+++ b/splatfields_amd/csrc/render.hip
@@ -1,4 +1,5 @@
 #include "kernels.h"
+#include "sort_tile.h"
 #define SR_QM_DEVICE 1
 #include "quadmask.h"
 
@@ -44,22 +45,27 @@
     if (writer) g.tile_qlast[16 * (size_t)tile + 4 * qy + qx] = ql;
 }
 
-__global__ void __launch_bounds__(kBlock) k_render_forward(const ViewK v, const Geom g, const Binning b, const Image im,
+__global__ void __launch_bounds__(kBlock) __attribute__((amdgpu_waves_per_eu(8, 8))) k_render_forward(const ViewK v, const Geom g, const Binning b, const Image im,
                                                            float* __restrict__ out_color, float* __restrict__ out_depth,
                                                            float* __restrict__ out_alpha) {
     constexpr int kB = 256;
     static_assert(kB == 256 || kB == 128, "a batch is staged by four or by two wavefronts");
     constexpr int kStagers = kB / kWave;
     constexpr uint32_t kStep = 4 / kStagers;
-    __shared__ float4 s_r0[1][kB];
-    __shared__ float4 s_r1[1][kB];
-    __shared__ float4 s_r2[1][kB];
-    __shared__ uint16_t s_qm[1][kB];
+    typedef float4 Quarter[1][kB];
+    typedef uint16_t QuadMasks[1][kB];
+    typedef uint8_t QuadIndex[4][4][kB + 4];
+    constexpr size_t kStageBytes = 3 * sizeof(Quarter) + sizeof(QuadMasks) + sizeof(QuadIndex), kSortBytes = kSortSmallMax * sizeof(uint64_t);
+    __shared__ __attribute__((aligned(16))) unsigned char s_blk[kStageBytes > kSortBytes ? kStageBytes : kSortBytes];
+    Quarter& s_r0 = *reinterpret_cast<Quarter*>(s_blk);
+    Quarter& s_r1 = *reinterpret_cast<Quarter*>(s_blk + sizeof(Quarter));
+    Quarter& s_r2 = *reinterpret_cast<Quarter*>(s_blk + 2 * sizeof(Quarter));
+    QuadMasks& s_qm = *reinterpret_cast<QuadMasks*>(s_blk + 3 * sizeof(Quarter));
+    QuadIndex& s_idx = *reinterpret_cast<QuadIndex*>(s_blk + 3 * sizeof(Quarter) + sizeof(QuadMasks));
     __shared__ uint32_t s_live[2][4];
-    __shared__ uint8_t s_idx[4][4][kB + 4];
     static_assert(kB == 256, "the pipelined walk indexes the staging area with unmasked bytes: 256 slots");
 
-    const uint32_t total_instances = g.total[0], longest_list = g.total[1];
+    const uint32_t total_instances = g.total[0], longest_list = g.total[1], long_slots = g.total[4];
     const int tile = (int)g.tile_order[blockIdx.x];
     asm volatile("" :: "s"(tile));
     if ((total_instances > b.capacity) | (longest_list > b.sorted_up_to)) {
@@ -74,15 +80,27 @@
         }
         return;
     }
+    const uint32_t start = g.tile_start[tile], end = g.tile_start[tile + 1];
+    const uint32_t n_list = end - start;
+    const bool short_list = n_list <= min(b.sort_in_blend, kSortSmallMax);
+    const bool long_list = !short_list && n_list <= kSortInlineMax && b.sort_in_blend >= kSortInlineMax &&
+                           (b.long_class_launched == 0u || few_long_tiles(long_slots, longest_list));
+    if ((n_list != 0u) & (short_list | long_list)) {
+        sort_tile_inline(b, start, n_list, reinterpret_cast<uint64_t*>(s_blk));
+        __builtin_amdgcn_fence(__ATOMIC_RELEASE, "workgroup");
+        __syncthreads();
+        __builtin_amdgcn_fence(__ATOMIC_ACQUIRE, "workgroup");
+    }
+    uint32_t tid = threadIdx.x;
+    asm volatile("" : "+v"(tid));
     const int tx = tile % v.gx, ty = tile / v.gx;
-    const int wave = __builtin_amdgcn_readfirstlane(wave_id()), lane = lane_id();
+    const int wave = __builtin_amdgcn_readfirstlane((int)(tid >> 6)), lane = (int)(tid & 63u);
     const int sx = tx * kTile + (wave & 1) * kSub, sy = ty * kTile + (wave >> 1) * kSub;
     const int qrow = lane >> 4;
     const int px = sx + 4 * (qrow & 1) + (lane & 3), py = sy + 4 * (qrow >> 1) + ((lane >> 2) & 3);
     const bool inside = px < v.W && py < v.H;
     const float tx0f = (float)(tx * kTile), ty0f = (float)(ty * kTile);
     const float Xf = (float)(px - tx * kTile), Yf = (float)(py - ty * kTile);
-    const uint32_t start = g.tile_start[tile], end = g.tile_start[tile + 1];
     const uint32_t my_quads = 0x33u << (2 * (wave & 1) + 8 * (wave >> 1));
 
     float T = 1.0f, Cr = 0.f, Cg = 0.f, Cb = 0.f, D = 0.f;
@@ -93,7 +111,7 @@
     }
     {
     auto stages = [&](uint32_t k) { return kStagers == 4 || (uint32_t)(wave >> 1) == (k & 1u); };
-    const int slot = kStagers == 4 ? (int)threadIdx.x : (int)(threadIdx.x & 127u);
+    const int slot = kStagers == 4 ? (int)tid : (int)(tid & 127u);
     const int wslot = kStagers == 4 ? wave : (wave & 1);
     const uint32_t l0 = lds_address(&s_r0[0][wslot * kWave]), l1 = lds_address(&s_r1[0][wslot * kWave]), l2 = lds_address(&s_r2[0][wslot * kWave]);
     constexpr uint32_t kCopyStride = kB * sizeof(float4);
diff --git a/splatfields_amd/csrc/sort_tile.h b/splatfields_amd/csrc/sort_tile.h
--- /dev/null
+++ b/splatfields_amd/csrc/sort_tile.h
@@ -0,0 +1,227 @@
+#pragma once
+#include "common.h"
+
+namespace sr {
+
+template <int D>
+__device__ __forceinline__ uint32_t lane_xor(uint32_t x) {
+    if constexpr (D == 1) return (uint32_t)__builtin_amdgcn_update_dpp(0, (int)x, 0xB1, 0xf, 0xf, false);
+    else if constexpr (D == 2) return (uint32_t)__builtin_amdgcn_update_dpp(0, (int)x, 0x4E, 0xf, 0xf, false);
+    else if constexpr (D == 8) return (uint32_t)__builtin_amdgcn_update_dpp(0, (int)x, 0x128, 0xf, 0xf, false);
+    else if constexpr (D == 4) {
+        const uint32_t a = (uint32_t)__builtin_amdgcn_update_dpp(0, (int)x, 0x124, 0xf, 0xf, false);
+        const uint32_t b = (uint32_t)__builtin_amdgcn_update_dpp(0, (int)x, 0x12C, 0xf, 0xf, false);
+        return (threadIdx.x & 4u) ? a : b;
+    } else if constexpr (D == 16) {
+        typedef unsigned int u2 __attribute__((ext_vector_type(2)));
+        const u2 r = __builtin_amdgcn_permlane16_swap(x, x, false, false);
+        return (threadIdx.x & 16u) ? r.x : r.y;
+    } else {
+        typedef unsigned int u2 __attribute__((ext_vector_type(2)));
+        const u2 r = __builtin_amdgcn_permlane32_swap(x, x, false, false);
+        return (threadIdx.x & 32u) ? r.x : r.y;
+    }
+}
+
+__device__ __forceinline__ uint32_t lane_xor_d(uint32_t x, int d) {
+    switch (d) {
+        case 1: return lane_xor<1>(x);
+        case 2: return lane_xor<2>(x);
+        case 4: return lane_xor<4>(x);
+        case 8: return lane_xor<8>(x);
+        case 16: return lane_xor<16>(x);
+        default: return lane_xor<32>(x);
+    }
+}
+
+__device__ __forceinline__ void exchange_select(uint64_t& k, uint64_t pk, bool keep_min) {
+    const bool take = (pk < k) == keep_min;
+    k = take ? pk : k;
+}
+
+template <int N, int E>
+__device__ __forceinline__ void bitonic_regs(uint64_t (&k)[E], uint64_t* skey, uint32_t tid) {
+#pragma unroll
+    for (int kk = 2; kk <= N; kk <<= 1) {
+#pragma unroll
+        for (int j = kk >> 1; j > 0; j >>= 1) {
+            if (j < E) {
+#pragma unroll
+                for (int e = 0; e < E; ++e) {
+                    if ((e & j) == 0) {
+                        const uint32_t i = tid * E + e;
+                        const bool asc = (i & kk) == 0;
+                        const bool swap = (k[e] > k[e | j]) == asc;
+                        const uint64_t ka = k[e], kb = k[e | j];
+                        k[e] = swap ? kb : ka; k[e | j] = swap ? ka : kb;
+                    }
+                }
+            } else if (j < 64 * E) {
+                const int d = j / E;
+                const bool lower = (tid & d) == 0;
+                const bool keep_min = lower == (((tid * E) & kk) == 0);
+                uint32_t plo[E], phi[E];
+#pragma unroll
+                for (int e = 0; e < E; ++e) {
+                    plo[e] = lane_xor_d((uint32_t)k[e], d);
+                    phi[e] = lane_xor_d((uint32_t)(k[e] >> 32), d);
+                }
+#pragma unroll
+                for (int e = 0; e < E; ++e) exchange_select(k[e], ((uint64_t)phi[e] << 32) | plo[e], keep_min);
+            } else {
+                __syncthreads();
+#pragma unroll
+                for (int e = 0; e < E; ++e) skey[tid * E + e] = k[e];
+                __syncthreads();
+#pragma unroll
+                for (int e = 0; e < E; ++e) {
+                    const uint32_t i = tid * E + e;
+                    const bool asc = (i & kk) == 0;
+                    const bool lower = (i & j) == 0;
+                    exchange_select(k[e], skey[i ^ j], lower == asc);
+                }
+            }
+        }
+    }
+}
+
+template <int N, int E>
+__device__ __forceinline__ void load_sort_chunk(const Binning& b, uint32_t first, uint32_t m, uint64_t (&k)[E], uint64_t* scratch_key, uint32_t tid) {
+#pragma unroll
+    for (int e = 0; e < E; ++e) {
+        const uint32_t i = tid * E + e;
+        k[e] = i < m ? b.ent[first + i] : ~0ull;
+    }
+    bitonic_regs<N, E>(k, scratch_key, tid);
+}
+
+template <int N, int E>
+__device__ __forceinline__ void sort_tile_regs(const Binning& b, uint32_t start, uint32_t n, uint64_t* skey) {
+    uint64_t k[E];
+    load_sort_chunk<N, E>(b, start, n, k, skey, threadIdx.x);
+#pragma unroll
+    for (int e = 0; e < E; ++e) {
+        const uint32_t i = threadIdx.x * E + e;
+        if (i < n) b.sorted_id[start + i] = (uint32_t)k[e];
+    }
+}
+
+template <int E, typename Out>
+__device__ __forceinline__ void merge_run_pairs_at(const uint64_t* src, uint32_t n, uint32_t width, uint32_t o, Out&& out) {
+    if (o >= n) return;
+    const uint32_t base = o & ~(2u * width - 1u);
+    const uint64_t* A = src + base;
+    const uint32_t a = min(width, n - base);
+    const uint32_t b = n - base - a < width ? n - base - a : width;
+    const uint32_t d = o - base;
+    uint32_t lo = d > b ? d - b : 0u, hi = min(d, a);
+    while (lo < hi) {
+        const uint32_t mid = (lo + hi) >> 1;
+        if (A[mid] < A[width + d - 1u - mid]) lo = mid + 1u; else hi = mid;
+    }
+    uint32_t ai = lo, bi = d - lo;
+    constexpr uint64_t kInf = ~0ull;
+    uint64_t ka = ai < a ? A[ai] : kInf;
+    uint64_t kb = bi < b ? A[width + bi] : kInf;
+#pragma unroll
+    for (int e = 0; e < E; ++e) {
+        const bool take_a = ka < kb;
+        const uint64_t key = take_a ? ka : kb;
+        if (d + (uint32_t)e < a + b) out(o + (uint32_t)e, key);
+        ai += take_a ? 1u : 0u;
+        bi += take_a ? 0u : 1u;
+        const bool more = take_a ? ai < a : bi < b;
+        const uint64_t nxt = A[take_a ? min(ai, a - 1u) : width + min(bi, max(b, 1u) - 1u)];
+        if (take_a) ka = more ? nxt : kInf; else kb = more ? nxt : kInf;
+    }
+}
+
+template <int E, typename Out>
+__device__ __forceinline__ void merge_run_pairs(const uint64_t* src, uint32_t n, uint32_t width, Out&& out) {
+    merge_run_pairs_at<E>(src, n, width, threadIdx.x * (uint32_t)E, out);
+}
+
+template <int CAP, int THREADS, typename Emit>
+__device__ __forceinline__ void sort_block_lds(const Binning& b, uint32_t first, uint32_t n, uint64_t* run_key, Emit&& emit) {
+    constexpr int GROUPS = THREADS / 256;
+    const uint32_t group = threadIdx.x >> 8, tid = threadIdx.x & 255u;
+    const uint32_t n_runs = (n + 1023u) / 1024u;
+    for (uint32_t r0 = 0; r0 < n_runs; r0 += GROUPS) {
+        const uint32_t r = r0 + group;
+        const uint32_t m = r < n_runs ? min(1024u, n - r * 1024u) : 0u;
+        __syncthreads();
+        uint64_t* rk = run_key + r * 1024u;
+        uint64_t k[4];
+        if (m <= 256u) {
+            uint64_t k1[1];
+            load_sort_chunk<256, 1>(b, first + r * 1024u, m, k1, rk, tid);
+            k[0] = k1[0];
+        } else if (m <= 512u) {
+            uint64_t k2[2];
+            load_sort_chunk<512, 2>(b, first + r * 1024u, m, k2, rk, tid);
+            k[0] = k2[0]; k[1] = k2[1];
+        } else {
+            load_sort_chunk<1024, 4>(b, first + r * 1024u, m, k, rk, tid);
+        }
+        __syncthreads();
+        const uint32_t per = m <= 256u ? 1u : (m <= 512u ? 2u : 4u);
+#pragma unroll
+        for (int e = 0; e < 4; ++e) {
+            const uint32_t i = tid * per + e;
+            if ((uint32_t)e < per && i < m) rk[i] = k[e];
+        }
+    }
+    __syncthreads();
+    uint64_t* src = run_key;
+    uint64_t* dst = run_key + CAP;
+    for (uint32_t width = 1024u;; width <<= 1) {
+        if (2u * width >= n) {
+            merge_run_pairs<CAP / THREADS>(src, n, width, emit);
+            break;
+        }
+        merge_run_pairs<CAP / THREADS>(src, n, width, [&](uint32_t pos, uint64_t key) { dst[pos] = key; });
+        __syncthreads();
+        uint64_t* t = src; src = dst; dst = t;
+    }
+    __syncthreads();
+}
+
+constexpr uint32_t kSortSmallMax = 2048u;
+__device__ __forceinline__ void sort_tile_small(const Binning& b, uint32_t start, uint32_t n, uint64_t* skey) {
+    if (n <= 256u) sort_tile_regs<256, 1>(b, start, n, skey);
+    else if (n <= 512u) sort_tile_regs<512, 2>(b, start, n, skey);
+    else if (n <= 1024u) sort_tile_regs<1024, 4>(b, start, n, skey);
+    else sort_block_lds<2048, 256>(b, start, n, skey, [&](uint32_t rank, uint64_t key) { b.sorted_id[start + rank] = (uint32_t)key; });
+}
+
+constexpr uint32_t kSortInlineMax = 4096u;
+__device__ __forceinline__ void sort_tile_inline(const Binning& b, uint32_t start, uint32_t n, uint64_t* skey) {
+    if (n <= 256u) sort_tile_regs<256, 1>(b, start, n, skey);
+    else if (n <= 512u) sort_tile_regs<512, 2>(b, start, n, skey);
+    else if (n <= 1024u) sort_tile_regs<1024, 4>(b, start, n, skey);
+    else {
+        const bool halves = n > kSortSmallMax;
+        uint64_t* k0 = b.keys + start;
+#pragma unroll 1
+        for (uint32_t off = 0; off < n; off += kSortSmallMax) {
+            uint32_t* ids = b.sorted_id + start;
+            asm volatile("" : "+s"(ids));
+            sort_block_lds<2048, 256>(b, start + off, min(kSortSmallMax, n - off), skey, [&](uint32_t rank, uint64_t key) {
+                if (halves) k0[off + rank] = key; else ids[rank] = (uint32_t)key;
+            });
+        }
+        if (halves) {
+            __builtin_amdgcn_fence(__ATOMIC_RELEASE, "workgroup");
+            __syncthreads();
+            __builtin_amdgcn_fence(__ATOMIC_ACQUIRE, "workgroup");
+#pragma unroll 1
+            for (uint32_t o = threadIdx.x * 8u; o < n; o += 256u * 8u)
+                merge_run_pairs_at<8>(k0, n, kSortSmallMax, o, [&](uint32_t pos, uint64_t key) { b.sorted_id[start + pos] = (uint32_t)key; });
+        }
+    }
+}
+
+constexpr uint32_t kInlineLongTiles = 8u;
+__device__ __forceinline__ bool few_long_tiles(uint32_t long_slots, uint32_t longest) { return long_slots <= kInlineLongTiles && longest <= kSortInlineMax; }
+
+}
diff --git a/splatfields_amd/rasterizer.py b/splatfields_amd/rasterizer.py
--- a/splatfields_amd/rasterizer.py
+++ b/splatfields_amd/rasterizer.py
@@ -103,6 +103,14 @@
     return {0: "auto", 1: "wave", 2: "quads"}[prev]
 
 
+_SORT_KERNELS = {None: 0, "auto": 0, "inline": 0, "standalone": 1, "short": 2}
+
+
+def set_sort_kernel(which) -> str:
+    prev = _lib.load().sr_set_sort_kernel(_SORT_KERNELS[which])
+    return {0: "inline", 1: "standalone", 2: "short"}[prev]
+
+
 def _round_capacity(instances: int) -> int:
     c = max(int(instances * _HEADROOM) + 1024, 1 << 16)
     step = 1 << (c.bit_length() - 4)
@@ -119,6 +127,7 @@
     hint: Optional[int] = None
     expected: int = -1
     covered: int = 0
+    long_tiles: int = -1
 
 
 class _Estimates:
@@ -129,6 +138,7 @@
     def __init__(self):
         self.capacity = {}
         self.per_splat = {}
+        self.long_tiles = {}
         self.lock = threading.Lock()
 
     def plan(self, device_index: int, n: int, H: int, W: int, view, may_async: bool) -> _Promise:
@@ -137,12 +147,13 @@
             ratio = self.per_splat.get((device_index, H, W))
             capacity = self.capacity.get(key) or (max(4 * n, 1 << 16) if ratio is None else _round_capacity(int(ratio * n)))
             before = view.seen.get(n) if may_async else None
+            long_tiles = int(self.long_tiles.get((id(view.seen), n), -1))
         if before is None or _round_capacity(before[0]) > capacity:
             return _Promise(key, capacity)
         hint = int(before[1] * _HEADROOM) + 1
-        return _Promise(key, capacity, hint, int(before[1]), _covered_by_hint(hint))
-
-    def record(self, promise: _Promise, view, instances: int, longest: int) -> None:
+        return _Promise(key, capacity, hint, int(before[1]), _covered_by_hint(hint), long_tiles)
+
+    def record(self, promise: _Promise, view, instances: int, longest: int, long_tiles: int = -1) -> None:
         global LAST_INSTANCES
         dev, n, H, W = key = promise.key
         rkey = (dev, H, W)
@@ -155,6 +166,9 @@
                 if len(view.seen) > self.SEEN_ROWS:
                     view.seen.clear()
                 view.seen[n] = (int(instances), int(longest))
+                if len(self.long_tiles) > self.CAPACITY_ROWS:
+                    self.long_tiles.clear()
+                self.long_tiles[(id(view.seen), n)] = int(long_tiles)
             LAST_INSTANCES = instances
 
 
@@ -191,11 +205,12 @@
     def _redeem(self, ticket):
         inst, longest = C.c_longlong(0), C.c_longlong(0)
         rc = self.lib.sr_ticket_wait(ticket, C.byref(inst), C.byref(longest))
+        long_tiles = int(_lib.load().sr_last_long_tiles()) if rc == 0 else -1
         with _PENDING_LOCK:
             self._list[:] = [r for r in self._list if r() is not None and r() is not self]
         _lib.check(rc)
         instances, longest, promise = int(inst.value), int(longest.value), self.promise
-        _ESTIMATES.record(promise, self.view, instances, longest)
+        _ESTIMATES.record(promise, self.view, instances, longest, long_tiles)
         covered = max(promise.covered, 2048)
         if instances > promise.capacity or longest > covered:
             return RasterizerOverflow(
@@ -367,6 +382,7 @@
         state, outs = (C.byref(view.struct), C.byref(splats), _ptr(geom)), (_ptr(image), _ptr(color), _ptr(depth), _ptr(alpha))
         if promise.hint is not None:
             ticket = C.c_void_p()
+            lib.sr_expect_long_tiles(promise.long_tiles)
             _lib.check(lib.sr_forward_async(*state, _ptr(radii), _ptr(binning), capacity, promise.hint, promise.expected, *outs,
                                             C.byref(ticket), stream))
             return geom, binning, image, capacity, None, _Pending(lib, ticket, promise, view)
@@ -375,7 +391,7 @@
         if status != _lib.SR_NEED_CAPACITY:
             _lib.check(status)
         instances = int(inst.value)
-        _ESTIMATES.record(promise, view, instances, int(lib.sr_last_longest_list()))
+        _ESTIMATES.record(promise, view, instances, int(lib.sr_last_longest_list()), int(lib.sr_last_long_tiles()))
         if status == _lib.SR_NEED_CAPACITY:
             capacity = _round_capacity(instances)
             binning = torch.empty(lib.sr_binning_bytes(capacity, H, W), dtype=torch.uint8, device=dev)
```

Result: faster. 1341000 billion (median of 6 runs) (+2.9%).
